# giesselmann/STRique

Measured on AMD Instinct MI355X. Metric: reads/s for STRique 'count' on 50 kb r9.4 signals, higher is better.
Workload: dtype f32

## Files before the change

### include/strique_hip.h

```cpp
#ifndef STRIQUE_HIP_H
#define STRIQUE_HIP_H

#include <stdint.h>

#ifdef __cplusplus
extern "C" {
#endif

#define STRQ_OK 0
#define STRQ_ERR_ARG 1
#define STRQ_ERR_DEVICE 2
#define STRQ_ERR_UNSUPPORTED 3
#define STRQ_ERR_NOMEM 4

typedef struct strq_ctx strq_ctx;

int strq_abi_version(void);

int strq_ctx_create(int device_id, strq_ctx** out);
void strq_ctx_destroy(strq_ctx* ctx);
const char* strq_last_error(const strq_ctx* ctx);
int strq_device_synchronize(strq_ctx* ctx);

int strq_set_option(strq_ctx* ctx, const char* key, const char* value);
// ... 12 lines not shown
                     int32_t samples,
                     float* score, int64_t* j_end, int64_t* j0, int32_t* rec);

int strq_model_create(strq_ctx* ctx, int32_t n_states, int32_t silent_start, int32_t start, int32_t end,
                      const int32_t* in_ptr, const int32_t* in_src, const double* in_logp,
                      const int32_t* emis_kind, const double* emis_a, const double* emis_b,
                      const double* emis_c, const int32_t* count_inc, const int32_t* state_tag,
                      const int32_t* hint_slot, const int32_t* hint_lane, int32_t* model_id);

int strq_model_set_positions(strq_ctx* ctx, int32_t model_id, const int32_t* kind, const int32_t* pos);

int strq_viterbi(strq_ctx* ctx, int32_t model_id, const double* x, int64_t T,
                 double* logp, int64_t* counted, int32_t* status, int32_t* path);
int strq_viterbi_batch(strq_ctx* ctx, int32_t model_id, int64_t n_seq, const double* x,
                       const int64_t* x_off, double* logp, int64_t* counted, int32_t* status,
                       int32_t* paths);

int strq_forward_batch(strq_ctx* ctx, int32_t model_id, int64_t n_seq, const double* x, const int64_t* x_off,
                       const int64_t* c0, double* log_lik, double* visits_mean, double* visits_var, int32_t* status);
int strq_model_set_forward_logp(strq_ctx* ctx, int32_t model_id, const double* in_logp_sum);

typedef struct strq_result {
    int32_t count;
    int32_t status;
    double score_prefix, score_suffix, log_p;
    int64_t offset, ticks;
    int64_t prefix_begin, prefix_end, suffix_begin, suffix_end;
} strq_result;

int strq_set_pore_stats(strq_ctx* ctx, double tail_lo, double tail_hi, double model_min, double model_max);
int strq_target_add(strq_ctx* ctx, const float* prefix_ext, int64_t m_prefix, const float* suffix_ext,
                    int64_t m_suffix, int32_t trim_prefix, int32_t trim_suffix, int32_t samples,
                    int32_t hmm_model_id, int32_t count_bias, int32_t* target_id);
int strq_target_set_mod(strq_ctx* ctx, int32_t target_id, int32_t mod_model_id, double mod_min, double mod_max);
int strq_batch_fetch_mod(strq_ctx* ctx, char* pool, int64_t pool_cap, int64_t* off);
int strq_set_units(strq_ctx* ctx, int32_t on);
int strq_batch_fetch_units(strq_ctx* ctx, int64_t* pool, int64_t pool_cap, int64_t* off, int32_t* decoded);
int strq_last_units(strq_ctx* ctx, double* out4);
int strq_set_mod_llr(strq_ctx* ctx, int32_t on);
int strq_batch_fetch_mod_llr(strq_ctx* ctx, double* pool, int64_t pool_cap, int64_t* off);
int strq_last_mod_llr(strq_ctx* ctx, double* out4);
int strq_target_set_variants(strq_ctx* ctx, int32_t target_id, int32_t model_id, double lo, double hi, int32_t n_alt, int32_t context_units);
int strq_set_variants(strq_ctx* ctx, int32_t on);
int strq_batch_fetch_variants(strq_ctx* ctx, int32_t* count_v, int32_t* decoded, int64_t* off, int8_t* branch, int64_t* end, int64_t pass_cap,
                              double* vpool, int64_t* voff, int64_t v_cap, int64_t* v_total);
int strq_last_variants(strq_ctx* ctx, double* out4);
int strq_set_confidence(strq_ctx* ctx, int32_t on);
int strq_batch_fetch_confidence(strq_ctx* ctx, double* out3, int32_t* decoded);
int strq_last_confidence(strq_ctx* ctx, double* out4);
int strq_detect_batch(strq_ctx* ctx, int64_t n_reads, const void* signals, int32_t dtype,
                      const int64_t* offsets, const int32_t* target_id, const double* host_stats,
                      strq_result* out);
int strq_detect_batch_reads(strq_ctx* ctx, int64_t n_reads, const void* const* reads, const int64_t* lengths, int32_t dtype,
                            const int32_t* target_id, const double* host_stats, strq_result* out);
int strq_batch_upload(strq_ctx* ctx, int64_t n_reads, const void* signals, int32_t dtype,
                      const int64_t* offsets, const int32_t* target_id, const double* host_stats);
int strq_batch_upload_part(strq_ctx* ctx, int64_t total_reads, int64_t total_samples, int64_t first_read, int64_t n_reads,
                           const void* signals, int32_t dtype, const int64_t* offsets, const int32_t* target_id);
int strq_batch_run(strq_ctx* ctx);
int strq_batch_run_range(strq_ctx* ctx, int64_t first, int64_t last);
int strq_batch_fetch(strq_ctx* ctx, strq_result* out);
int strq_batch_fetch_range(strq_ctx* ctx, int64_t first, int64_t last, strq_result* out);
int strq_scan_batch_reads(strq_ctx* ctx, int64_t n_reads, const void* const* reads, const int64_t* lengths, int32_t dtype,
                          int32_t n_cand, const int32_t* cand_target_id, double min_score,
                          strq_result* out_rows, int32_t* out_cand, double* out_scores);
int strq_scan_set(strq_ctx* ctx, int32_t n_cand, const int32_t* cand_target_id, double min_score);
int strq_scan_clear(strq_ctx* ctx);
int strq_batch_fetch_scan(strq_ctx* ctx, int32_t* out_cand, double* out_scores);
typedef struct strq_anchored {
    int32_t kind;
    int32_t status;
    int32_t count, pad_;
    double log_p;
    int64_t begin, end;
    int64_t free_samples;
} strq_anchored;
int strq_target_set_anchored(strq_ctx* ctx, int32_t target_id, int32_t end_model_id, int32_t end_bias, int32_t start_model_id, int32_t start_bias);
int strq_set_anchored(strq_ctx* ctx, int32_t on, double min_score);
int strq_batch_fetch_anchored(strq_ctx* ctx, strq_anchored* out, int64_t n);
int strq_last_anchored(strq_ctx* ctx, double* out8);
typedef struct strq_renorm_fit {
    int32_t a, b, w;
    int32_t fitted;
    int64_t score;
} strq_renorm_fit;
typedef struct strq_renorm {
    int32_t applied, pad_;
    strq_renorm_fit fit[3];
} strq_renorm;
int strq_target_set_renorm(strq_ctx* ctx, int32_t target_id, const int16_t* Q, int32_t q_out, const int32_t* A, const double* W,
                           double grid_lo, double grid_d, double grid_p);
int strq_set_renorm(strq_ctx* ctx, int32_t on, double min_share);
int strq_batch_fetch_renorm(strq_ctx* ctx, strq_renorm* out, int64_t n);
int strq_last_renorm(strq_ctx* ctx, double* out4);
int strq_debug_renorm_fit(strq_ctx* ctx, int32_t target_id, const uint32_t* h3, strq_renorm* out);
int strq_host_stats(const double* signals, const int64_t* offsets, int64_t n_reads, int32_t want_raw, double* out);
int64_t strq_svb_decode(const uint8_t* stream, int64_t stream_len, int64_t n, int32_t key_bits, int32_t zigzag,
                        int32_t isize, void* out);
int64_t strq_inflate_chunks(const uint8_t* base, int64_t base_len, int64_t n_chunks, const int64_t* addr,
                            const int32_t* csize, const int64_t* elem_off, int32_t elem_size, int32_t shuffle,
                            int64_t chunk_elems, int64_t n_total, void* out);
#define STRQ_H5_UNHANDLED (-100)
#define STRQ_H5_MORE_CHUNKS (-101)
int64_t strq_h5_locate(const uint8_t* base, int64_t base_len, int64_t group_ohdr, const char* path, int64_t meta[16],
                       int64_t* chunk_addr, int32_t* chunk_size, int64_t* chunk_off, int64_t max_chunks);
int64_t strq_inflate_many(int64_t n_ds, const uint8_t* const* base, const int64_t* base_len, const int64_t* chunk_first,
                          const int64_t* addr, const int32_t* csize, const int64_t* elem_off, const int32_t* elem_size,
                          const int32_t* shuffle, const int64_t* chunk_elems, const int64_t* n_total, void* const* out,
                          int64_t* status);
int64_t strq_vbz_chunks(const uint8_t* base, int64_t base_len, int64_t n_chunks, const int64_t* addr, const int32_t* csize,
                        const int64_t* elem_off, int32_t elem_size, int32_t version, int32_t isize, int32_t zigzag, int32_t level,
                        int64_t chunk_elems, int64_t n_total, void* out);
void strq_inflate_stats(int64_t out[3], int32_t reset);
int strq_inflate_backend(void);
int strq_debug_conditioning(strq_ctx* ctx, int64_t read, uint8_t* levels, int64_t n, float* level_val,
                            double* scalars10);
int strq_debug_filtered(strq_ctx* ctx, int64_t read, void* out, int64_t n);
int strq_debug_live_allocations(int64_t out[2]);
int strq_debug_g2_layout(int32_t n_states, int32_t silent_start, int32_t start, int32_t end,
                         const int32_t* in_ptr, const int32_t* in_src, const double* in_logp,
                         const int32_t* emis_kind, const int32_t* count_inc, const int32_t* kind, const int32_t* pos,
                         double* out_lp, int32_t* out_own, int32_t* out_meta, char* why, int32_t why_len);

int strq_debug_screen_plan(const float params[6], int32_t samples, int32_t max_n, int32_t out[6]);

int strq_debug_score_tables(strq_ctx* ctx, int32_t n_jobs, const float* level_val, const float* cls_val, const int64_t* cls_off,
                            int32_t* info, int32_t* band_lo, float* table, uint8_t* planes,
                            int32_t* handed, int32_t handed_cap, int32_t* n_handed);

int strq_debug_variant_image(int32_t n_states, int32_t silent_start, int32_t start, int32_t end,
                             const int32_t* in_ptr, const int32_t* in_src, const double* in_logp,
                             const int32_t* emis_kind, const double* emis_a, const double* emis_b, const double* emis_c,
                             const int32_t* state_tag, int32_t n_alt, int32_t* build_rc, int32_t* head, int64_t* offsets,
                             void* image, int64_t image_cap, int64_t* image_bytes, char* why, int32_t why_len);
int strq_debug_mod_llr_image(int32_t n_states, int32_t silent_start, int32_t start, int32_t end,
                             const int32_t* in_ptr, const int32_t* in_src, const double* in_logp,
                             const int32_t* emis_kind, const double* emis_a, const double* emis_b, const double* emis_c,
                             const int32_t* state_tag, int32_t* build_rc, int32_t* head, int64_t* offsets,
                             void* image, int64_t image_cap, int64_t* image_bytes, char* why, int32_t why_len);
int strq_debug_variant_scores(strq_ctx* ctx, int32_t n_reads, const int32_t* model_id, int32_t n_alt, const double* x,
                              const int64_t* x_off, const int32_t* w, const int64_t* w_off, double* out, int32_t* launched);
int strq_debug_mod_llr_scores(strq_ctx* ctx, int32_t n_reads, const int32_t* model_id, const double* x, const int64_t* x_off,
                              const int32_t* w, const int64_t* w_off, double* out, int32_t* launched);
int strq_debug_variant_bounds(strq_ctx* ctx, int32_t model_id, int32_t n_alt, int32_t n_reads, const int64_t* off,
                              const int32_t* path, const uint64_t* rec, const uint32_t* last, const int32_t* status,
                              const int32_t* cap, int32_t stride, int32_t guard, int32_t* n, int32_t* bad, int32_t* w,
                              int32_t* branch, int32_t* untouched);

int strq_last_timing(const strq_ctx* ctx, float ms[8]);
int strq_last_counters(const strq_ctx* ctx, double out[8]);
int strq_last_geometry(const strq_ctx* ctx, int32_t out[8]);
int strq_last_viterbi_launches(const strq_ctx* ctx, int32_t out[4]);
int strq_last_second_round(const strq_ctx* ctx, int64_t out[2]);
int strq_last_screen(const strq_ctx* ctx, double out[8]);
int strq_last_screen_mode(const strq_ctx* ctx, int32_t out[8]);
int strq_last_overlap(const strq_ctx* ctx, double out[4]);

#ifdef __cplusplus
}
#endif
#endif
```

### strique_amd/csrc/align_kernels.h

```cpp
#pragma once
#include <hip/hip_runtime.h>
#include <stdint.h>

#define STRQ_CKPT_STEPS 256
#define STRQ_COLS_PER_STEP 2
#define STRQ_CKPT_FIELDS(R) (2 * (R) + 6)
#define STRQ_TRACE_WORDS(R) (((R) + 15) / 16)

namespace strq {

struct AlignParams {
    float open_h, ext_h, open_v, ext_v, dist_offset, dist_min;
};

struct AlignTask {
    const uint8_t* levels;
    const float* table;
    const uint8_t* table3;
    const int32_t* band_lo;
    const float* col0;
    float* ckpt;
    int32_t* rec;
    const float* bnd_in;
    float* bnd_out;
    const AlignTask* up;
    int32_t n, m, k, tsize;
    int32_t row0, m_total;
    int32_t col_off, n_full;
};

struct AlignResult {
    float best;
    int32_t j_end;
    int32_t j0;
    int32_t status;
};

static inline int align_num_steps(int n) { return (n + 1) / 2 + 63; }
static inline int align_num_ckpts(int n) { return (align_num_steps(n) - 1) / STRQ_CKPT_STEPS; }

#define STRQ_MAX_STRIPS 64
int align_plan(int m, int samples, int* rows_per_lane, int* n_strips);
int align_effective_samples(int samples);
int align_segment_overlap(const AlignParams& p, int m);
int launch_align_segments(hipStream_t stream, int R, int S, const AlignTask* tasks, AlignResult* seg_results,
                          int n_groups, int segs, int* queue, const AlignParams& p, int lds_dwords,
                          int tables_per_cu, int n_cu, int packed, const int* group_list = nullptr, const int* n_list = nullptr,
                          bool known_last_row = false);
int align_segments_wpe(int segs, int tables_per_cu);
int launch_align_combine(hipStream_t stream, const AlignTask* tasks, const AlignResult* seg_results, int n_align,
                         int segs, AlignResult* results, int32_t* pick, int pick_base = 0, const int* list = nullptr,
                         const int* n_list = nullptr, const float* min_score = nullptr, int* redo = nullptr, int* redo_count = nullptr,
                         unsigned int* redo_total = nullptr);
int launch_align_scatter(hipStream_t stream, const AlignResult* src, const int32_t* pick_src, const int32_t* first, const int32_t* pos, int n,
                         AlignResult* dst, int32_t* pick_dst);
float align_segment_min_score(const AlignParams& p, int m, int overlap_used);
int align_overlap_for_score(const AlignParams& p, int m, float score);
int launch_align(hipStream_t stream, int R, int S, const AlignTask* tasks, AlignResult* results,
                 int n_tasks, int* queue, const AlignParams& p, int lds_floats_per_wave,
                 int waves_per_block, int n_blocks, uint64_t* scratch, int phase, int mode, int packed,
                 const int32_t* pick = nullptr);
size_t align_trace_scratch_words_per_wave(int R);

}
```

### strique_amd/csrc/align_kernels.hip

```cpp
#include "strq_opt.h"
#include <hip/hip_runtime.h>
#include <stdint.h>
#include "align_kernels.h"
#include <stdlib.h>
#include <type_traits>
#include <utility>

namespace strq {

#define STRQ_NINF (-3.4028234663852886e38f / 2)

#define STRQ_STR2(x) #x
#define STRQ_STR(x) STRQ_STR2(x)
#define STRQ_TIE_EXT(ext, opn)  ((ext) >= (opn))
#define STRQ_TIE_H_OVER_V(h, v) ((h) >= (v))
#define STRQ_TIE_D_OVER_G(d, g) ((d) >= (g))

static __device__ __forceinline__ float dpp_shr1_f(float v, float fill)
{
    return __builtin_bit_cast(float, __builtin_amdgcn_update_dpp(__builtin_bit_cast(int, fill),
                              __builtin_bit_cast(int, v), 0x138, 0xF, 0xF, false));
}
static __device__ __forceinline__ float dpp_shr1_f0(float v)
{
    return __builtin_bit_cast(float, __builtin_amdgcn_update_dpp(0, __builtin_bit_cast(int, v), 0x138, 0xF, 0xF, true));
}
static __device__ __forceinline__ int dpp_shr1_i(int v, int fill)
{
    return __builtin_amdgcn_update_dpp(fill, v, 0x138, 0xF, 0xF, false);
}
template <class T> static __device__ __forceinline__ const T* uniform_ptr(const T* p)
{
    const uint64_t u = reinterpret_cast<uint64_t>(p);
    const uint32_t lo = __builtin_amdgcn_readfirstlane((int)(uint32_t)u), hi = __builtin_amdgcn_readfirstlane((int)(uint32_t)(u >> 32));
    return reinterpret_cast<const T*>(((uint64_t)hi << 32) | lo);
}
static __device__ __forceinline__ int med3i(int a, int lo, int hi)
{
    int r;
    asm("v_med3_i32 %0, %1, %2, %3" : "=v"(r) : "v"(a), "v"(lo), "v"(hi));
    return r;
}
static __device__ __forceinline__ float sel_mask(float if0, float if1, uint64_t mask)
{
    float r;
    asm("v_cndmask_b32_e64 %0, %1, %2, %3" : "=v"(r) : "v"(if0), "v"(if1), "s"(mask));
    return r;
}

static __device__ __forceinline__ int next_task(int* queue, int lane)
{
    __builtin_amdgcn_wave_barrier();
    int ti = 0;
    if (lane == 0) ti = atomicAdd(queue, 1);
    __builtin_amdgcn_wave_barrier();
    ti = __builtin_amdgcn_readfirstlane(ti);
    __builtin_amdgcn_wave_barrier();
    return ti;
}

template <int R, int S> struct Shape {
    static constexpr int gcd_(int a, int b) { return b == 0 ? a : gcd_(b, a % b); }
    static constexpr int G = gcd_(R, S);
    static constexpr int C = (S - G + R - 1) / S + 1;
    static constexpr int NMASK = S / G;
    static_assert(C <= 6, "too many classes per lane");
};

template <int R> struct Lane {
    float S[R];
    float H[R];
    float SbotA;
    float VbotA;
    float VbotB;
    float upS;
};

struct LaneConst {
    int off[6];
    int lo4[6];
    int hi4[6];
    int off2[6];
};

#define STRQ_PK_SCALE 1048576.0f
template <int R, int S, bool PK>
static __device__ __forceinline__ void fetch_scores(const char* lds, const LaneConst& lc, int q4,
                                                    float (&sc)[Shape<R, S>::C])
{
#pragma unroll
    for (int c = 0; c < Shape<R, S>::C; ++c) {
        if constexpr (PK) {
            const int ci = med3i(q4, lc.lo4[c], lc.hi4[c]);
            const uint32_t h = *reinterpret_cast<const uint16_t*>(lds + (ci << 1) + lc.off[c]);
            const uint32_t l = *reinterpret_cast<const uint8_t*>(lds + ci + lc.off2[c]);
            sc[c] = (float)((h << 8) | l);
        } else {
            const int t = med3i(q4, lc.lo4[c], lc.hi4[c]) + lc.off[c];
            sc[c] = *reinterpret_cast<const float*>(lds + t);
        }
    }
}

template <int R, int S>
static __device__ __forceinline__ void expand_scores(const float (&sc)[Shape<R, S>::C],
                                                     const uint64_t (&pm)[Shape<R, S>::NMASK],
                                                     float (&rs)[R])
{
    constexpr int G = Shape<R, S>::G, C = Shape<R, S>::C;
#pragma unroll
    for (int r = 0; r < R; r += G) {
        const int base = r / S, x = (r % S) / G;
        float v;
        if (x == 0 || base + 1 >= C) v = sc[base < C ? base : C - 1];
        else v = sel_mask(sc[base], sc[base + 1], pm[x]);
#pragma unroll
        for (int g = 0; g < G && r + g < R; ++g) rs[r + g] = v;
    }
}

template <int R>
static __device__ __forceinline__ float pick_row(const float (&x)[R], int rM)
{
    typedef float vec_t __attribute__((ext_vector_type(R <= 16 ? 16 : 32)));
    vec_t v;
#pragma unroll
    for (int r = 0; r < R; ++r) v[r] = x[r];
    return v[rM];
}

struct TraceWords { uint64_t a[2], b[2]; };

#ifndef STRQ_TRACE_SELECT
static __device__ __forceinline__ void trace_push_ge(uint32_t& acc, float a, float b)
{
    asm("v_cmp_ge_f32 vcc, %1, %2\n\tv_addc_co_u32 %0, vcc, %0, %0, vcc" : "+v"(acc) : "v"(a), "v"(b) : "vcc");
}
#endif
template <int R> static __device__ __forceinline__ int trace_shift(int r)
{
#ifndef STRQ_TRACE_SELECT
    const int in_word = r % 16, half = in_word / 8;
    const int rows_word = R - 16 * (r / 16) < 16 ? R - 16 * (r / 16) : 16;
    const int rows_half = rows_word - 8 * half < 8 ? rows_word - 8 * half : 8;
    return 32 * half + 4 * (rows_half - 1 - (in_word % 8));
#else
    return 4 * (r % 16);
#endif
}

template <int R, bool LH, bool LV, bool KEEP, bool TRACE, int RMC = -1>
static __device__ __forceinline__ void dp_step2(Lane<R>& st, const float (&rsA)[R], const float (&rsB)[R],
                                                float upA, float upB, float upVA, float upVB,
                                                const AlignParams& p, TraceWords* tw,
                                                int rM, float* candA, float* candB)
{
    float SA[R], SB[R];
    float HA[R], HB[R];
    float vA = upVA, vB = upVB;
    if constexpr (TRACE) { tw->a[0] = tw->a[1] = tw->b[0] = tw->b[1] = 0; }
    uint32_t accA[4] = {0u, 0u, 0u, 0u}, accB[4] = {0u, 0u, 0u, 0u};
    (void)accA; (void)accB;
#pragma unroll
    for (int r = 0; r < R; ++r) {
        {
            const float diag = r == 0 ? st.upS : st.S[r - 1];
            const float up = r == 0 ? upA : SA[r > 0 ? r - 1 : 0];
            const float D = diag + rsA[r];
            if constexpr (TRACE) {
                const float hext = st.H[r] + p.ext_h, hopn = st.S[r] + p.open_h;
                const float vext = vA + p.ext_v, vopn = up + p.open_v;
#ifndef STRQ_TRACE_SELECT
                uint32_t& acc = accA[(r / 16) * 2 + (r % 16) / 8];
                trace_push_ge(acc, vext, vopn); trace_push_ge(acc, hext, hopn);
                const float Hn = __builtin_fmaxf(hext, hopn), Vn = __builtin_fmaxf(vext, vopn);
                trace_push_ge(acc, Hn, Vn);
                const float Gm = __builtin_fmaxf(Hn, Vn);
                trace_push_ge(acc, D, Gm);
                SA[r] = __builtin_fmaxf(D, Gm); HA[r] = Hn; vA = Vn;
#else
                const bool he = STRQ_TIE_EXT(hext, hopn);
                const float Hn = he ? hext : hopn;
                const bool ve = STRQ_TIE_EXT(vext, vopn);
                const float Vn = ve ? vext : vopn;
                const bool gh = STRQ_TIE_H_OVER_V(Hn, Vn);
                const float Gm = gh ? Hn : Vn;
                const bool dd = STRQ_TIE_D_OVER_G(D, Gm);
                SA[r] = dd ? D : Gm; HA[r] = Hn; vA = Vn;
                const uint64_t code = (dd ? 1u : 0u) | (gh ? 2u : 0u) | (he ? 4u : 0u) | (ve ? 8u : 0u);
                tw->a[r / 16] |= code << (4 * (r % 16));
#endif
            } else {
                float Hn, Vn;
                if constexpr (LH) Hn = st.S[r] + p.ext_h;
                else Hn = __builtin_fmaxf(st.H[r] + p.ext_h, st.S[r] + p.open_h);
                if constexpr (LV) Vn = up + p.ext_v;
                else Vn = __builtin_fmaxf(vA + p.ext_v, up + p.open_v);
                SA[r] = __builtin_fmaxf(__builtin_fmaxf(D, Hn), Vn);
                HA[r] = Hn; vA = Vn;
            }
        }
        {
            const float diag = r == 0 ? upA : SA[r > 0 ? r - 1 : 0];
            const float up = r == 0 ? upB : SB[r > 0 ? r - 1 : 0];
            const float D = diag + rsB[r];
            if constexpr (TRACE) {
                const float hext = HA[r] + p.ext_h, hopn = SA[r] + p.open_h;
                const float vext = vB + p.ext_v, vopn = up + p.open_v;
#ifndef STRQ_TRACE_SELECT
                uint32_t& acc = accB[(r / 16) * 2 + (r % 16) / 8];
                trace_push_ge(acc, vext, vopn); trace_push_ge(acc, hext, hopn);
                const float Hn = __builtin_fmaxf(hext, hopn), Vn = __builtin_fmaxf(vext, vopn);
                trace_push_ge(acc, Hn, Vn);
                const float Gm = __builtin_fmaxf(Hn, Vn);
                trace_push_ge(acc, D, Gm);
                SB[r] = __builtin_fmaxf(D, Gm); HB[r] = Hn; vB = Vn;
#else
                const bool he = STRQ_TIE_EXT(hext, hopn);
                const float Hn = he ? hext : hopn;
                const bool ve = STRQ_TIE_EXT(vext, vopn);
                const float Vn = ve ? vext : vopn;
                const bool gh = STRQ_TIE_H_OVER_V(Hn, Vn);
                const float Gm = gh ? Hn : Vn;
                const bool dd = STRQ_TIE_D_OVER_G(D, Gm);
                SB[r] = dd ? D : Gm; HB[r] = Hn; vB = Vn;
                const uint64_t code = (dd ? 1u : 0u) | (gh ? 2u : 0u) | (he ? 4u : 0u) | (ve ? 8u : 0u);
                tw->b[r / 16] |= code << (4 * (r % 16));
#endif
            } else {
                float Hn, Vn;
                if constexpr (LH) Hn = SA[r] + p.ext_h;
                else Hn = __builtin_fmaxf(HA[r] + p.ext_h, SA[r] + p.open_h);
                if constexpr (LV) Vn = up + p.ext_v;
                else Vn = __builtin_fmaxf(vB + p.ext_v, up + p.open_v);
                SB[r] = __builtin_fmaxf(__builtin_fmaxf(D, Hn), Vn);
                HB[r] = Hn; vB = Vn;
            }
        }
    }
#ifndef STRQ_TRACE_SELECT
    if constexpr (TRACE) {
#pragma unroll
        for (int x = 0; x < 2; ++x) {
            tw->a[x] = (uint64_t)accA[2 * x] | ((uint64_t)accA[2 * x + 1] << 32);
            tw->b[x] = (uint64_t)accB[2 * x] | ((uint64_t)accB[2 * x + 1] << 32);
        }
    }
#endif
#pragma unroll
    for (int r = 0; r < R; ++r) st.S[r] = SB[r];
    if constexpr (TRACE || !LH || KEEP) {
#pragma unroll
        for (int r = 0; r < R; ++r) st.H[r] = HB[r];
    }
    st.SbotA = SA[R - 1];
    if constexpr (TRACE || !LV || KEEP) { st.VbotA = vA; st.VbotB = vB; }
    st.upS = upB;
    if constexpr (RMC >= 0) { *candA = SA[RMC]; *candB = SB[RMC]; }
    else if (candA) { *candA = pick_row<R>(SA, rM); *candB = pick_row<R>(SB, rM); }
}

template <int R, int S, bool PK>
static __device__ __forceinline__ void load_lane_consts(const AlignTask& tk, int lane, int lds_base,
                                                        LaneConst& lc, uint64_t (&pm)[Shape<R, S>::NMASK])
{
    const int row0 = tk.row0 + lane * R;
    const int kbase = row0 / S - tk.row0 / S, phase = row0 % S;
    const int off0 = 0;
#pragma unroll
    for (int c = 0; c < Shape<R, S>::C; ++c) {
        int k = kbase + c; if (k > tk.k - 1) k = tk.k - 1;
        const uint32_t d = (uint32_t)tk.band_lo[k];
        const int lo = (int)(d & 255u), w1 = (int)((d >> 8) & 255u), off = (int)(d >> 16);
        if constexpr (PK) {
            lc.lo4[c] = lo; lc.hi4[c] = lo + w1;
            lc.off[c] = lds_base + (off - lo) * 2;
            lc.off2[c] = lds_base + ((2 * tk.tsize + 3) & ~3) + off - lo;
        } else {
            lc.lo4[c] = lo * 4;
            lc.hi4[c] = (lo + w1) * 4;
            lc.off[c] = lds_base + (off - off0) * 4 - lo * 4;
            lc.off2[c] = 0;
        }
    }
#pragma unroll
    for (int x = 0; x < Shape<R, S>::NMASK; ++x) {
        const uint64_t b = __ballot(phase >= S - x * Shape<R, S>::G);
        const uint32_t lo = __builtin_amdgcn_readfirstlane((int)(uint32_t)b), hi = __builtin_amdgcn_readfirstlane((int)(uint32_t)(b >> 32));
        pm[x] = ((uint64_t)hi << 32) | lo;
    }
}

template <bool PK>
static __device__ __forceinline__ void stage_table(const AlignTask& tk, float* lds, int lane)
{
    if constexpr (PK) {
        const uint32_t* src = reinterpret_cast<const uint32_t*>(tk.table3);
        uint32_t* dst = reinterpret_cast<uint32_t*>(lds);
        const int nd = (((2 * tk.tsize + 3) & ~3) + tk.tsize + 3) / 4;
        for (int i = lane; i < nd; i += 64) dst[i] = src[i];
    } else {
        for (int i = lane; i < tk.tsize; i += 64) lds[i] = tk.table[i];
    }
}

template <int R, bool PK>
static __device__ __forceinline__ void init_lane(const AlignTask& tk, int lane, Lane<R>& st)
{
    constexpr float SC = PK ? STRQ_PK_SCALE : 1.0f;
    const int row0 = lane * R;
#pragma unroll
    for (int r = 0; r < R; ++r) {
        int i = row0 + r + 1; if (i > tk.m) i = tk.m;
        st.S[r] = tk.col0[i] * SC;
        st.H[r] = STRQ_NINF;
    }
    { int i = row0 + R; if (i > tk.m) i = tk.m; st.SbotA = st.VbotA = st.VbotB = tk.col0[i] * SC; }
    { int i = row0;     if (i > tk.m) i = tk.m; st.upS = tk.col0[i] * SC; }
}

template <bool PK>
static __device__ __forceinline__ int load_chunk(const AlignTask& tk, int chunk, int lane)
{
    constexpr int U = PK ? 1 : 4;
    const int idx = (chunk * 64 + lane) * 2;
    int a = 0, b = 0;
    if (idx < tk.n) a = tk.levels[idx];
    if (idx + 1 < tk.n) b = tk.levels[idx + 1];
    return (a * U) | ((b * U) << 16);
}

struct Bnd4 { float sA, vA, sB, vB; };
static __device__ __forceinline__ Bnd4 load_bnd(const AlignTask& tk, int chunk, int lane)
{
    const int idx = (chunk * 64 + lane) * 2;
    Bnd4 b{0.0f, STRQ_NINF, 0.0f, STRQ_NINF};
    if (idx < tk.n) { b.sA = tk.bnd_in[2 * idx]; b.vA = tk.bnd_in[2 * idx + 1]; }
    if (idx + 1 < tk.n) { b.sB = tk.bnd_in[2 * idx + 2]; b.vB = tk.bnd_in[2 * idx + 3]; }
    return b;
}

template <int R>
static __device__ __forceinline__ void save_ckpt(float* c, int lane, const Lane<R>& st)
{
#pragma unroll
    for (int r = 0; r < R; ++r) c[r * 64 + lane] = st.S[r];
#pragma unroll
    for (int r = 0; r < R; ++r) c[(R + r) * 64 + lane] = st.H[r];
    c[(2 * R + 0) * 64 + lane] = st.SbotA;
    c[(2 * R + 1) * 64 + lane] = st.VbotA;
    c[(2 * R + 2) * 64 + lane] = st.VbotB;
    c[(2 * R + 3) * 64 + lane] = st.upS;
}
template <int R>
static __device__ __forceinline__ void load_ckpt(const float* c, int lane, Lane<R>& st)
{
#pragma unroll
    for (int r = 0; r < R; ++r) st.S[r] = c[r * 64 + lane];
#pragma unroll
    for (int r = 0; r < R; ++r) st.H[r] = c[(R + r) * 64 + lane];
    st.SbotA = c[(2 * R + 0) * 64 + lane];
    st.VbotA = c[(2 * R + 1) * 64 + lane];
    st.VbotB = c[(2 * R + 2) * 64 + lane];
    st.upS = c[(2 * R + 3) * 64 + lane];
}

template <int R, int S, bool LH, bool LV, int MODE, bool RM_LAST, bool PK, int RMC = -1>
struct Forward {
    static constexpr bool HAS_IN = (MODE & 1) != 0, HAS_OUT = (MODE & 2) != 0;
    const AlignTask& tk;
    const AlignParams& p;
    const char* ldsb;
    const LaneConst& lc;
    const uint64_t (&pm)[Shape<R, S>::NMASK];
    const int lane, rM;
    Lane<R> st;
    float best, bestA; int bestt;
    int qq;
    float scA[Shape<R, S>::C], scB[Shape<R, S>::C];
    Bnd4 bcur;

    __device__ __forceinline__ void advance(int qsrc, int snext, int& qn, float (&nA)[Shape<R, S>::C], float (&nB)[Shape<R, S>::C])
    {
        qn = dpp_shr1_i(qq, __builtin_amdgcn_readlane(qsrc, snext));
        fetch_scores<R, S, PK>(ldsb, lc, qn & 0xffff, nA);
        fetch_scores<R, S, PK>(ldsb, lc, (int)((unsigned)qn >> 16), nB);
    }
    __device__ __forceinline__ void prime(int qcur)
    {
        qq = 0;
        int qn; float nA[Shape<R, S>::C], nB[Shape<R, S>::C];
        advance(qcur, 0, qn, nA, nB);
        qq = qn;
#pragma unroll
        for (int c = 0; c < Shape<R, S>::C; ++c) { scA[c] = nA[c]; scB[c] = nB[c]; }
    }

    template <bool PRED, bool KEEP, int RMX = RMC>
    __device__ __forceinline__ void step(int t, int s, int qsrc, int snext)
    {
        int qn; float nA[Shape<R, S>::C], nB[Shape<R, S>::C];
        advance(qsrc, snext, qn, nA, nB);
        float fA = 0.0f, fB = 0.0f, fVA = STRQ_NINF, fVB = STRQ_NINF;
        if constexpr (HAS_IN) {
            fA = __builtin_bit_cast(float, __builtin_amdgcn_readlane(__builtin_bit_cast(int, bcur.sA), s));
            fB = __builtin_bit_cast(float, __builtin_amdgcn_readlane(__builtin_bit_cast(int, bcur.sB), s));
            if constexpr (!LV) {
                fVA = __builtin_bit_cast(float, __builtin_amdgcn_readlane(__builtin_bit_cast(int, bcur.vA), s));
                fVB = __builtin_bit_cast(float, __builtin_amdgcn_readlane(__builtin_bit_cast(int, bcur.vB), s));
            }
        }
#ifdef STRQ_DP_ZFILL
        const float upA = HAS_IN ? dpp_shr1_f(st.SbotA, fA) : dpp_shr1_f0(st.SbotA);
        const float upB = HAS_IN ? dpp_shr1_f(st.S[R - 1], fB) : dpp_shr1_f0(st.S[R - 1]);
#else
        const float upA = dpp_shr1_f(st.SbotA, fA);
        const float upB = dpp_shr1_f(st.S[R - 1], fB);
#endif
        float upVA = STRQ_NINF, upVB = STRQ_NINF;
        if constexpr (!LV) { upVA = dpp_shr1_f(st.VbotA, fVA); upVB = dpp_shr1_f(st.VbotB, fVB); }
        const int jB = 2 * (t - lane), jA = jB - 1;
        bool act = true;
        if constexpr (PRED) act = (jA >= 1) && (jA <= tk.n);
        if (act) {
            float rsA[R], rsB[R];
            expand_scores<R, S>(scA, pm, rsA);
            expand_scores<R, S>(scB, pm, rsB);
            bool okB = true;
            if constexpr (PRED) okB = jB <= tk.n;
            if constexpr (HAS_OUT) {
                dp_step2<R, LH, LV, true, false>(st, rsA, rsB, upA, upB, upVA, upVB, p, nullptr, 0, nullptr, nullptr);
                if (lane == 63) {
                    float* o = tk.bnd_out + 2 * (size_t)(jA - 1);
                    o[0] = st.SbotA; o[1] = st.VbotA;
                    if (okB) { o[2] = st.S[R - 1]; o[3] = st.VbotB; }
                }
            } else {
                float candA, candB;
                if constexpr (RM_LAST || RMX == R - 1) {
                    dp_step2<R, LH, LV, KEEP, false>(st, rsA, rsB, upA, upB, upVA, upVB, p, nullptr, 0, nullptr, nullptr);
                    candA = st.SbotA; candB = st.S[R - 1];
                } else if constexpr (RMX >= 0) {
                    dp_step2<R, LH, LV, KEEP, false, RMX>(st, rsA, rsB, upA, upB, upVA, upVB, p, nullptr, rM, &candA, &candB);
                } else {
                    dp_step2<R, LH, LV, KEEP, false>(st, rsA, rsB, upA, upB, upVA, upVB, p, nullptr, rM, &candA, &candB);
                }
                const float cb = okB ? candB : candA;
                const float nb = __builtin_fmaxf(__builtin_fmaxf(best, candA), cb);
                if (nb > best) { bestt = t; bestA = candA; }
                best = nb;
            }
        }
        qq = qn;
#pragma unroll
        for (int c = 0; c < Shape<R, S>::C; ++c) { scA[c] = nA[c]; scB[c] = nB[c]; }
    }
};

template <int R, int S, int X, class F>
static __device__ __forceinline__ void rm_case(int rM, bool& hit, F& f)
{
    if constexpr ((X + 1) % Shape<R, S>::G == 0) {
        if (!hit && rM == X) { f(std::integral_constant<int, X>{}); hit = true; }
    }
}
template <int R, int S, class F, int... X>
static __device__ __forceinline__ bool rm_dispatch(int rM, F& f, std::integer_sequence<int, X...>)
{
    bool hit = false;
    (rm_case<R, S, X>(rM, hit, f), ...);
    return hit;
}

template <int R, int S, bool LH, bool LV, int MODE, bool RM_LAST, bool PK, bool STAGE = true, int RMC = -1, bool RMSW = false>
static __device__ __forceinline__ void forward_one(const AlignTask& tk, AlignResult* res, const AlignParams& p,
                                                   float* lds, int lds_base, const char* ldsb, int lane)
{
    constexpr bool HAS_IN = (MODE & 1) != 0, HAS_OUT = (MODE & 2) != 0;
    if constexpr (STAGE) stage_table<PK>(tk, lds, lane);
    LaneConst lc; uint64_t pm[Shape<R, S>::NMASK];
    load_lane_consts<R, S, PK>(tk, lane, lds_base, lc, pm);
    const int lM = (tk.m - 1) / R, rM = (tk.m - 1) % R;
    Forward<R, S, LH, LV, MODE, RM_LAST, PK, RMC> f{tk, p, ldsb, lc, pm, lane, rM};
    init_lane<R, PK>(tk, lane, f.st);
    f.best = tk.col0[tk.m] * (PK ? STRQ_PK_SCALE : 1.0f); f.bestA = 0.0f; f.bestt = -1;
    __builtin_amdgcn_s_waitcnt(0);

    const int nsteps = (tk.n + 1) / 2 + 63;
    int rM_u = 0;
    if constexpr (RMSW) rM_u = __builtin_amdgcn_readfirstlane(rM);
    (void)rM_u;
    int qcur = load_chunk<PK>(tk, 0, lane);
    f.prime(qcur);
    Bnd4 bnext{0.0f, STRQ_NINF, 0.0f, STRQ_NINF};
    if constexpr (HAS_IN) f.bcur = load_bnd(tk, 0, lane); else f.bcur = bnext;
    for (int t0 = 0; t0 < nsteps; t0 += 64) {
        const int qnext = load_chunk<PK>(tk, t0 / 64 + 1, lane);
        if constexpr (HAS_IN) bnext = load_bnd(tk, t0 / 64 + 1, lane);
        const bool full = (t0 >= 63) && (2 * (t0 + 64) <= tk.n);
        const bool ckpt_here = ((t0 + 64) % STRQ_CKPT_STEPS) == 0 && (t0 + 64) < nsteps;
        const int send = nsteps - t0 < 64 ? nsteps - t0 : 64;
        if (full) {
#ifdef STRQ_DP_PAD
            asm volatile(".p2align 6\n\t.rept " STRQ_STR(STRQ_DP_PAD) "\n\ts_nop 0\n\t.endr");
#endif
            if constexpr (RMSW && !HAS_OUT && !RM_LAST) {
                auto chunk = [&](auto rmx) {
                    constexpr int X = decltype(rmx)::value;
                    for (int s = 0; s < 63; ++s) f.template step<false, false, X>(t0 + s + 1, s, qcur, s + 1);
                    if (ckpt_here) f.template step<false, true, X>(t0 + 64, 63, qnext, 0);
                    else f.template step<false, false, X>(t0 + 64, 63, qnext, 0);
                };
                if (!rm_dispatch<R, S>(rM_u, chunk, std::make_integer_sequence<int, R>{})) chunk(std::integral_constant<int, -1>{});
            } else {
                for (int s = 0; s < 63; ++s) f.template step<false, false>(t0 + s + 1, s, qcur, s + 1);
                if (ckpt_here) f.template step<false, true>(t0 + 64, 63, qnext, 0);
                else f.template step<false, false>(t0 + 64, 63, qnext, 0);
            }
        } else {
            for (int s = 0; s < send; ++s) {
                const int qsrc = s == 63 ? qnext : qcur, snext = (s + 1) & 63;
                if (ckpt_here && s == 63) f.template step<true, true>(t0 + s + 1, s, qsrc, snext);
                else f.template step<true, false>(t0 + s + 1, s, qsrc, snext);
            }
        }
        if (ckpt_here)
            save_ckpt<R>(tk.ckpt + (size_t)((t0 + 64) / STRQ_CKPT_STEPS - 1) * (STRQ_CKPT_FIELDS(R) * 64), lane, f.st);
        qcur = qnext;
        if constexpr (HAS_IN) f.bcur = bnext;
    }
    if constexpr (!HAS_OUT) {
        int bestj = 0;
        if (f.bestt >= 0) bestj = 2 * (f.bestt - lane) - (f.bestA == f.best ? 1 : 0);
        const float b = __shfl(f.best, lM, 64);
        const int bj = __shfl(bestj, lM, 64);
        res->best = b * (PK ? 1.0f / STRQ_PK_SCALE : 1.0f); res->j_end = bj;
    }
}

template <int R, int S, bool LH, bool LV, int MODE, bool PK>
__global__ void __launch_bounds__(512)
align_forward_kernel(const AlignTask* __restrict__ tasks, AlignResult* __restrict__ results, int n_tasks,
                     int* __restrict__ queue, AlignParams p, int lds_floats_per_wave)
{
    extern __shared__ float lds_all[];
    const int lane = threadIdx.x & 63, wave = threadIdx.x >> 6;
    float* lds = lds_all + (size_t)wave * lds_floats_per_wave;
    const int lds_base = wave * lds_floats_per_wave * 4;
    const char* ldsb = reinterpret_cast<const char*>(lds_all);
    for (;;) {
        const int ti = next_task(queue, lane);
        if (ti >= n_tasks) break;
        const AlignTask& tk = tasks[ti];
        if constexpr ((MODE & 2) != 0) forward_one<R, S, LH, LV, MODE, true, PK>(tk, results + ti, p, lds, lds_base, ldsb, lane);
        else {
            if ((tk.m - 1) % R == R - 1) forward_one<R, S, LH, LV, MODE, true, PK>(tk, results + ti, p, lds, lds_base, ldsb, lane);
            else forward_one<R, S, LH, LV, MODE, false, PK>(tk, results + ti, p, lds, lds_base, ldsb, lane);
        }
    }
}

template <int R, int S, bool PK, int SEG, int WPE, bool LISTED = false, bool KNOWN = false>
__global__ void __attribute__((amdgpu_flat_work_group_size(64 * SEG, 64 * SEG), amdgpu_waves_per_eu(WPE, WPE)))
align_forward_seg_kernel(const AlignTask* __restrict__ tasks, AlignResult* __restrict__ results, int n_groups,
                         int* __restrict__ queue, AlignParams p, const int* __restrict__ group_list,
                         const int* __restrict__ n_list)
{
    extern __shared__ float lds_all[];
    __shared__ int next_group;
    const int lane = threadIdx.x & 63, wave = threadIdx.x >> 6;
    const char* ldsb = reinterpret_cast<const char*>(lds_all);
    const int lds_base = 0;
    if constexpr (LISTED) n_groups = __builtin_amdgcn_readfirstlane(*n_list);
    for (;;) {
        __syncthreads();
        if (threadIdx.x == 0) next_group = atomicAdd(queue, 1);
        __syncthreads();
        int gi = __builtin_amdgcn_readfirstlane(next_group);
        if (gi >= n_groups) break;
        if constexpr (LISTED) gi = __builtin_amdgcn_readfirstlane(group_list[gi]);
        {
            const AlignTask& t0 = tasks[(size_t)gi * SEG];
            if constexpr (PK) {
                const uint32_t* src = reinterpret_cast<const uint32_t*>(t0.table3);
                uint32_t* dst = reinterpret_cast<uint32_t*>(lds_all);
                const int nd = (((2 * t0.tsize + 3) & ~3) + t0.tsize + 3) / 4;
                for (int i = threadIdx.x; i < nd; i += 64 * SEG) dst[i] = src[i];
            } else {
                for (int i = threadIdx.x; i < t0.tsize; i += 64 * SEG) lds_all[i] = t0.table[i];
            }
        }
        __syncthreads();
        const int ti = gi * SEG + wave;
        const AlignTask& tk = tasks[ti];
        if (tk.n <= 0) continue;
        if constexpr (KNOWN) {
            constexpr int RMC870 = R == 14 ? (870 - 1) % 14 : -1;
            if ((tk.m - 1) % R == R - 1) forward_one<R, S, true, true, 0, true, PK, false>(tk, results + ti, p, lds_all, lds_base, ldsb, lane);
            else if (RMC870 >= 0 && (tk.m - 1) % R == RMC870) forward_one<R, S, true, true, 0, false, PK, false, RMC870>(tk, results + ti, p, lds_all, lds_base, ldsb, lane);
            else forward_one<R, S, true, true, 0, false, PK, false>(tk, results + ti, p, lds_all, lds_base, ldsb, lane);
        } else {
            forward_one<R, S, true, true, 0, false, PK, false, -1, true>(tk, results + ti, p, lds_all, lds_base, ldsb, lane);
        }
    }
}

__global__ void align_combine_kernel(const AlignTask* __restrict__ tasks, const AlignResult* __restrict__ seg, int n_align,
                                     int segs, AlignResult* __restrict__ out, int32_t* __restrict__ pick, int pick_base,
                                     const int* __restrict__ list, const int* __restrict__ n_list,
                                     const float* __restrict__ min_score, int* __restrict__ redo, int* __restrict__ redo_count,
                                     unsigned int* __restrict__ redo_total)
{
    int a = blockIdx.x * blockDim.x + threadIdx.x;
    if (a >= (n_list ? *n_list : n_align)) return;
    if (list) a = list[a];
    int best_k = 0;
    float best = seg[(size_t)a * segs].best;
    for (int k = 1; k < segs; ++k) {
        const size_t t = (size_t)a * segs + k;
        if (tasks[t].n <= 0) continue;
        if (seg[t].best > best) { best = seg[t].best; best_k = k; }
    }
    const size_t t = (size_t)a * segs + best_k;
    AlignResult r = seg[t];
    r.j_end += tasks[t].col_off;
    out[a] = r;
    pick[a] = pick_base + (int32_t)t;
    if (min_score && !(best >= min_score[a])) {
        redo[atomicAdd(redo_count, 1)] = a;
        if (redo_total) atomicAdd(redo_total, 1u);
    }
}

template <int R, int S, bool PK>
__global__ void __launch_bounds__(512)
align_trace_kernel(const AlignTask* __restrict__ tasks, AlignResult* __restrict__ results, int n_tasks,
                   int* __restrict__ queue, AlignParams p, int lds_floats_per_wave,
                   uint64_t* __restrict__ scratch_all, const int32_t* __restrict__ pick)
{
    extern __shared__ float lds_all[];
    constexpr int W = STRQ_TRACE_WORDS(R);
    constexpr size_t STEP_WORDS = 2 * W * 64;
    const int lane = threadIdx.x & 63, wave = threadIdx.x >> 6;
    float* lds = lds_all + (size_t)wave * lds_floats_per_wave;
    const int lds_base = wave * lds_floats_per_wave * 4;
    const char* ldsb = reinterpret_cast<const char*>(lds_all);
    uint64_t* scratch = scratch_all + (size_t)(blockIdx.x * (blockDim.x >> 6) + wave) * (STRQ_CKPT_STEPS * STEP_WORDS);

    for (;;) {
        const int ti = next_task(queue, lane);
        if (ti >= n_tasks) break;
        const AlignTask* cur = &tasks[pick ? __builtin_amdgcn_readfirstlane(pick[ti]) : ti];
        const AlignTask* staged = nullptr;
        int32_t* rec = cur->rec;
        const int col_off = __builtin_amdgcn_readfirstlane(cur->col_off);
        LaneConst lc; uint64_t pm[Shape<R, S>::NMASK];

        int ci = cur->m_total, cj = __builtin_amdgcn_readfirstlane(results[ti].j_end) - col_off, state = 0;
        while (ci > 0 && cj > 0) {
            while (ci <= cur->row0) cur = uniform_ptr(cur->up);
            if (cur != staged) {
                __builtin_amdgcn_s_waitcnt(0);
                stage_table<PK>(*cur, lds, lane);
                load_lane_consts<R, S, PK>(*cur, lane, lds_base, lc, pm);
                __builtin_amdgcn_s_waitcnt(0);
                staged = cur;
            }
            const AlignTask& tk = *cur;
            const bool has_in = tk.bnd_in != nullptr;
            uint64_t pmu[Shape<R, S>::NMASK];
#pragma unroll
            for (int x = 0; x < Shape<R, S>::NMASK; ++x) {
                const uint32_t lo = __builtin_amdgcn_readfirstlane((int)(uint32_t)pm[x]), hi = __builtin_amdgcn_readfirstlane((int)(uint32_t)(pm[x] >> 32));
                pmu[x] = ((uint64_t)hi << 32) | lo;
            }
            const int tcur = (ci - tk.row0 - 1) / R + (cj + 1) / 2;
            const int blk = (tcur - 1) / STRQ_CKPT_STEPS;
            const int tb = blk * STRQ_CKPT_STEPS;
            Lane<R> st;
            if (blk == 0) init_lane<R, PK>(tk, lane, st);
            else load_ckpt<R>(tk.ckpt + (size_t)(blk - 1) * (STRQ_CKPT_FIELDS(R) * 64), lane, st);
            int qq = 0;
            {
                const int jB = 2 * (tb - lane), jA = jB - 1;
                int a = 0, b = 0;
                if (jA >= 1 && jA <= tk.n) a = tk.levels[jA - 1];
                if (jB >= 1 && jB <= tk.n) b = tk.levels[jB - 1];
                qq = (a * (PK ? 1 : 4)) | ((b * (PK ? 1 : 4)) << 16);
            }
            int qcur = load_chunk<PK>(tk, tb / 64, lane);
            Bnd4 bcur{0.0f, STRQ_NINF, 0.0f, STRQ_NINF}, bnext = bcur;
            if (has_in) bcur = load_bnd(tk, tb / 64, lane);
            for (int t0 = tb; t0 < tcur; t0 += 64) {
                const int qnext = load_chunk<PK>(tk, t0 / 64 + 1, lane);
                if (has_in) bnext = load_bnd(tk, t0 / 64 + 1, lane);
                const int send = tcur - t0 < 64 ? tcur - t0 : 64;
                for (int s = 0; s < send; ++s) {
                    const int t = t0 + s + 1;
                    qq = dpp_shr1_i(qq, __builtin_amdgcn_readlane(qcur, s));
                    const float fA = __builtin_bit_cast(float, __builtin_amdgcn_readlane(__builtin_bit_cast(int, bcur.sA), s));
                    const float fB = __builtin_bit_cast(float, __builtin_amdgcn_readlane(__builtin_bit_cast(int, bcur.sB), s));
                    const float fVA = __builtin_bit_cast(float, __builtin_amdgcn_readlane(__builtin_bit_cast(int, bcur.vA), s));
                    const float fVB = __builtin_bit_cast(float, __builtin_amdgcn_readlane(__builtin_bit_cast(int, bcur.vB), s));
                    const float upA = dpp_shr1_f(st.SbotA, fA);
                    const float upB = dpp_shr1_f(st.S[R - 1], fB);
                    const float upVA = dpp_shr1_f(st.VbotA, fVA);
                    const float upVB = dpp_shr1_f(st.VbotB, fVB);
                    const int jB = 2 * (t - lane), jA = jB - 1;
                    TraceWords w; w.a[0] = w.a[1] = w.b[0] = w.b[1] = 0;
                    if (jA >= 1 && jA <= tk.n) {
                        float scA[Shape<R, S>::C], scB[Shape<R, S>::C], rsA[R], rsB[R];
                        fetch_scores<R, S, PK>(ldsb, lc, qq & 0xffff, scA);
                        fetch_scores<R, S, PK>(ldsb, lc, (int)((unsigned)qq >> 16), scB);
                        expand_scores<R, S>(scA, pmu, rsA);
                        expand_scores<R, S>(scB, pmu, rsB);
                        dp_step2<R, false, false, true, true>(st, rsA, rsB, upA, upB, upVA, upVB, p, &w, 0, nullptr, nullptr);
                    }
                    uint64_t* dst = scratch + (size_t)(t - tb - 1) * STEP_WORDS;
#pragma unroll
                    for (int x = 0; x < W; ++x) {
                        dst[(0 * W + x) * 64 + lane] = w.a[x];
                        dst[(1 * W + x) * 64 + lane] = w.b[x];
                    }
                }
                qcur = qnext; bcur = bnext;
            }
            __threadfence();
            int pf_l = -1, pf_hi = 0, pf_lo = 0, pf_word = -1; uint64_t pf = 0;
            while (ci > tk.row0 && cj > 0) {
                const int il = ci - tk.row0;
                const int l = (il - 1) / R, r = (il - 1) % R;
                const int t = l + (cj + 1) / 2;
                if (t <= tb) break;
                const int colsel = (cj & 1) ? 0 : 1;
                if (l != pf_l || r / 16 != pf_word || t > pf_hi || t <= pf_lo) {
                    pf_l = l; pf_word = r / 16; pf_hi = t; pf_lo = t - 32 > tb ? t - 32 : tb;
                    const int st = t - (lane >> 1), cs = lane & 1;
                    pf = st > pf_lo ? scratch[(size_t)(st - tb - 1) * STEP_WORDS + (cs * W + pf_word) * 64 + l] : 0;
                }
                const int src = ((pf_hi - t) << 1) | colsel;
                const uint32_t wlo = (uint32_t)__builtin_amdgcn_readlane((int)(uint32_t)pf, src);
                const uint32_t whi = (uint32_t)__builtin_amdgcn_readlane((int)(uint32_t)(pf >> 32), src);
                const uint64_t w = ((uint64_t)whi << 32) | wlo;
                const uint32_t code = (uint32_t)(w >> trace_shift<R>(r)) & 15u;
                if (state == 0) {
                    if (code & 1u) { rec[ci - 1] = (cj + col_off) << 1; --ci; --cj; }
                    else state = (code & 2u) ? 1 : 2;
                } else if (state == 1) {
                    --cj; if (!(code & 4u)) state = 0;
                } else {
                    rec[ci - 1] = ((cj + col_off) << 1) | 1;
                    --ci; if (!(code & 8u)) state = 0;
                }
            }
        }
        for (int i = ci - lane; i > 0; i -= 64) rec[i - 1] = (col_off << 1) | 1;
        results[ti].j0 = cj + col_off;
    }
}

template <int R, int S>
static int launch_shape(hipStream_t stream, const AlignTask* tasks, AlignResult* results, int n_tasks,
                        int* queue, const AlignParams& p, int lds_floats_per_wave, int waves_per_block,
                        int n_blocks, uint64_t* scratch, int phase, int mode, int packed, const int32_t* pick)
{
    const size_t lds_bytes = (size_t)lds_floats_per_wave * 4 * waves_per_block;
    const dim3 grid(n_blocks), block(64 * waves_per_block);
    const bool lh = p.open_h == p.ext_h, lv = p.open_v == p.ext_v;
#define STRQ_FWD1(LH_, LV_, MODE_)                                                                      \
    do {                                                                                                \
        (void)hipFuncSetAttribute((const void*)align_forward_kernel<R, S, LH_, LV_, MODE_, false>,      \
                                  hipFuncAttributeMaxDynamicSharedMemorySize, (int)lds_bytes);          \
        hipLaunchKernelGGL((align_forward_kernel<R, S, LH_, LV_, MODE_, false>), grid, block, lds_bytes, stream,\
                           tasks, results, n_tasks, queue, p, lds_floats_per_wave);                     \
    } while (0)
#define STRQ_FWD(LH_, LV_)                                                                              \
    do {                                                                                                \
        if (mode == 0) STRQ_FWD1(LH_, LV_, 0); else if (mode == 1) STRQ_FWD1(LH_, LV_, 1);              \
        else if (mode == 2) STRQ_FWD1(LH_, LV_, 2); else STRQ_FWD1(LH_, LV_, 3);                        \
    } while (0)
    if (packed && !(lh && lv && mode == 0)) return 2;
    if (phase == 0 && packed) {
        AlignParams ps = p;
        ps.open_h *= STRQ_PK_SCALE; ps.ext_h *= STRQ_PK_SCALE; ps.open_v *= STRQ_PK_SCALE; ps.ext_v *= STRQ_PK_SCALE;
        (void)hipFuncSetAttribute((const void*)align_forward_kernel<R, S, true, true, 0, true>,
                                  hipFuncAttributeMaxDynamicSharedMemorySize, (int)lds_bytes);
        hipLaunchKernelGGL((align_forward_kernel<R, S, true, true, 0, true>), grid, block, lds_bytes, stream,
                           tasks, results, n_tasks, queue, ps, lds_floats_per_wave);
    } else if (phase == 0) {
        if (lh && lv) STRQ_FWD(true, true);
        else if (lh) STRQ_FWD(true, false);
        else if (lv) STRQ_FWD(false, true);
        else STRQ_FWD(false, false);
    } else if (packed) {
        AlignParams ps = p;
        ps.open_h *= STRQ_PK_SCALE; ps.ext_h *= STRQ_PK_SCALE; ps.open_v *= STRQ_PK_SCALE; ps.ext_v *= STRQ_PK_SCALE;
        (void)hipFuncSetAttribute((const void*)align_trace_kernel<R, S, true>,
                                  hipFuncAttributeMaxDynamicSharedMemorySize, (int)lds_bytes);
        hipLaunchKernelGGL((align_trace_kernel<R, S, true>), grid, block, lds_bytes, stream, tasks, results,
                           n_tasks, queue, ps, lds_floats_per_wave, scratch, pick);
    } else {
        (void)hipFuncSetAttribute((const void*)align_trace_kernel<R, S, false>,
                                  hipFuncAttributeMaxDynamicSharedMemorySize, (int)lds_bytes);
        hipLaunchKernelGGL((align_trace_kernel<R, S, false>), grid, block, lds_bytes, stream, tasks, results,
                           n_tasks, queue, p, lds_floats_per_wave, scratch, pick);
    }
#undef STRQ_FWD
#undef STRQ_FWD1
    return hipGetLastError() == hipSuccess ? 0 : 1;
}

template <int R, int S>
static int launch_shape_general(hipStream_t stream, const AlignTask* tasks, AlignResult* results, int n_tasks,
                                int* queue, const AlignParams& p, int lds_floats_per_wave, int waves_per_block,
                                int n_blocks, uint64_t* scratch, int phase, int mode, int packed, const int32_t* pick)
{
    if (packed) return 2;
    const size_t lds_bytes = (size_t)lds_floats_per_wave * 4 * waves_per_block;
    const dim3 grid(n_blocks), block(64 * waves_per_block);
#define STRQ_FWDG(MODE_)                                                                                \
    do {                                                                                                \
        (void)hipFuncSetAttribute((const void*)align_forward_kernel<R, S, false, false, MODE_, false>,  \
                                  hipFuncAttributeMaxDynamicSharedMemorySize, (int)lds_bytes);          \
        hipLaunchKernelGGL((align_forward_kernel<R, S, false, false, MODE_, false>), grid, block, lds_bytes, stream,\
                           tasks, results, n_tasks, queue, p, lds_floats_per_wave);                     \
    } while (0)
    if (phase == 0) {
        if (mode == 0) STRQ_FWDG(0); else if (mode == 1) STRQ_FWDG(1); else if (mode == 2) STRQ_FWDG(2); else STRQ_FWDG(3);
    } else {
        (void)hipFuncSetAttribute((const void*)align_trace_kernel<R, S, false>,
                                  hipFuncAttributeMaxDynamicSharedMemorySize, (int)lds_bytes);
        hipLaunchKernelGGL((align_trace_kernel<R, S, false>), grid, block, lds_bytes, stream, tasks, results,
                           n_tasks, queue, p, lds_floats_per_wave, scratch, pick);
    }
#undef STRQ_FWDG
    return hipGetLastError() == hipSuccess ? 0 : 1;
}

#define STRQ_SHAPES(X) X(6, 6) X(7, 6) X(8, 6) X(12, 6) X(14, 6) X(15, 6)
#define STRQ_GENERAL_SHAPES(X) X(2, 1) X(4, 2) X(6, 3) X(8, 4) X(10, 5) X(14, 7) X(16, 8) X(18, 9) X(20, 10) X(22, 11) X(26, 13)

int align_effective_samples(int samples)
{
    if (samples < 1) return 0;
    if (samples % 6 == 0) return 6;
    for (int d : {13, 11, 10, 9, 8, 7, 5, 4, 3, 2}) if (samples % d == 0) return d;
    return 1;
}

int align_plan(int m, int samples, int* rows_per_lane, int* n_strips)
{
    if (samples < 1 || m < 1) return 0;
    if (samples != 6) {
        if (align_effective_samples(samples) != samples) return 0;
        const int r = 2 * samples, rows = 64 * r;
        if (m > STRQ_MAX_STRIPS * rows) return 0;
        *rows_per_lane = r; *n_strips = (m + rows - 1) / rows;
        return r;
    }
    const char* e = strq::opt("STRQ_STRIPS");
    const bool force_two = e && e[0] == '2';
    const bool no14 = strq::opt("STRQ_NO_R14") != nullptr;
    const int single[] = {6, 7, 8, 12, 14, 15};
    const int two[] = {6, 7, 8, 12};
    if (!force_two)
        for (int r : single) if (64 * r >= m && !(r == 14 && no14)) { *rows_per_lane = r; *n_strips = 1; return r; }
    for (int r : two) if (64 * r < m && 128 * r >= m) { *rows_per_lane = r; *n_strips = 2; return r; }
    for (int r : single) if (64 * r >= m && !(r == 14 && no14)) { *rows_per_lane = r; *n_strips = 1; return r; }
    if (m <= STRQ_MAX_STRIPS * 64 * 12) { *rows_per_lane = 12; *n_strips = (m + 64 * 12 - 1) / (64 * 12); return 12; }
    return 0;
}

size_t align_trace_scratch_words_per_wave(int R)
{
    return (size_t)STRQ_CKPT_STEPS * 2 * STRQ_TRACE_WORDS(R) * 64;
}

int launch_align(hipStream_t stream, int R, int S, const AlignTask* tasks, AlignResult* results,
                 int n_tasks, int* queue, const AlignParams& p, int lds_floats_per_wave,
                 int waves_per_block, int n_blocks, uint64_t* scratch, int phase, int mode, int packed,
                 const int32_t* pick)
{
#define STRQ_CASE(R_, S_)                                                                               \
    if (R == R_ && S == S_)                                                                             \
        return launch_shape<R_, S_>(stream, tasks, results, n_tasks, queue, p, lds_floats_per_wave,     \
                                    waves_per_block, n_blocks, scratch, phase, mode, packed, pick);
    STRQ_SHAPES(STRQ_CASE)
#undef STRQ_CASE
#define STRQ_CASE(R_, S_)                                                                               \
    if (R == R_ && S == S_)                                                                             \
        return launch_shape_general<R_, S_>(stream, tasks, results, n_tasks, queue, p, lds_floats_per_wave, \
                                            waves_per_block, n_blocks, scratch, phase, mode, packed, pick);
    STRQ_GENERAL_SHAPES(STRQ_CASE)
#undef STRQ_CASE
    return 2;
}

int align_segment_overlap(const AlignParams& p, int m)
{
    if (!(p.dist_min >= 0.0f) || !(p.open_h < 0.0f) || !(p.ext_h < 0.0f) || !(p.dist_offset > 0.0f)) return 0;
    if (!(p.open_v <= 0.0f) || !(p.ext_v <= 0.0f)) return 0;
    const double c_h = -(double)(p.open_h > p.ext_h ? p.open_h : p.ext_h);
    const double gain = (double)(p.dist_min > p.dist_offset ? p.dist_min : p.dist_offset);
    const double h = (double)m * gain / c_h;
    const double L = (double)m + h * 1.01 + 64.0;
    if (!(L < 1e8)) return 0;
    return (int)L + 1;
}

template <int R, int S, bool PK, int SEG, int WPE, bool KNOWN>
static int launch_seg2(hipStream_t stream, const AlignTask* tasks, AlignResult* seg_results, int n_groups, int* queue,
                       const AlignParams& p, int lds_dwords, int n_blocks, const int* group_list, const int* n_list)
{
    const size_t lds_bytes = (size_t)lds_dwords * 4;
    if (group_list && n_list) {
        (void)hipFuncSetAttribute((const void*)align_forward_seg_kernel<R, S, PK, SEG, WPE, true, KNOWN>,
                                  hipFuncAttributeMaxDynamicSharedMemorySize, (int)lds_bytes);
        hipLaunchKernelGGL((align_forward_seg_kernel<R, S, PK, SEG, WPE, true, KNOWN>), dim3(n_blocks), dim3(64 * SEG), lds_bytes, stream,
                           tasks, seg_results, n_groups, queue, p, group_list, n_list);
    } else {
        (void)hipFuncSetAttribute((const void*)align_forward_seg_kernel<R, S, PK, SEG, WPE, false, KNOWN>,
                                  hipFuncAttributeMaxDynamicSharedMemorySize, (int)lds_bytes);
        hipLaunchKernelGGL((align_forward_seg_kernel<R, S, PK, SEG, WPE, false, KNOWN>), dim3(n_blocks), dim3(64 * SEG), lds_bytes, stream,
                           tasks, seg_results, n_groups, queue, p, group_list, n_list);
    }
    return hipGetLastError() == hipSuccess ? 0 : 1;
}

template <int R, int S, bool PK, int SEG, int WPE>
static int launch_seg1(hipStream_t stream, const AlignTask* tasks, AlignResult* seg_results, int n_groups, int* queue,
                       const AlignParams& p, int lds_dwords, int n_blocks, const int* group_list, const int* n_list, bool known_last_row)
{
    if constexpr (R == 14) {
        if (known_last_row) return launch_seg2<R, S, PK, SEG, WPE, true>(stream, tasks, seg_results, n_groups, queue, p, lds_dwords, n_blocks, group_list, n_list);
    }
    return launch_seg2<R, S, PK, SEG, WPE, false>(stream, tasks, seg_results, n_groups, queue, p, lds_dwords, n_blocks, group_list, n_list);
}

#define STRQ_SEG_CONFIGS(X, R_, S_, PK_) X(R_, S_, PK_, 1, 2) X(R_, S_, PK_, 2, 3) X(R_, S_, PK_, 2, 4) X(R_, S_, PK_, 3, 3) X(R_, S_, PK_, 4, 4) X(R_, S_, PK_, 3, 4) X(R_, S_, PK_, 4, 3)

int align_segments_wpe(int segs, int tables_per_cu)
{
    const int waves = tables_per_cu * segs;
    int wpe = (waves + 3) / 4; if (wpe < 2) wpe = 2;
    if (segs == 1) wpe = 2;
    else if (wpe < 3) wpe = 3;
    if (wpe > 4) wpe = 4;
    return wpe;
}

int launch_align_segments(hipStream_t stream, int R, int S, const AlignTask* tasks, AlignResult* seg_results,
                          int n_groups, int segs, int* queue, const AlignParams& p, int lds_dwords,
                          int tables_per_cu, int n_cu, int packed, const int* group_list, const int* n_list, bool known_last_row)
{
    if (!(p.open_h == p.ext_h && p.open_v == p.ext_v)) return 2;
    AlignParams ps = p;
    if (packed) { ps.open_h *= STRQ_PK_SCALE; ps.ext_h *= STRQ_PK_SCALE; ps.open_v *= STRQ_PK_SCALE; ps.ext_v *= STRQ_PK_SCALE; }
    const int wpe = align_segments_wpe(segs, tables_per_cu);
    const int n_blocks = tables_per_cu * n_cu;
#define STRQ_SEGCASE(R_, S_, PK_, SEG_, WPE_)                                                             \
    if (R == R_ && S == S_ && (packed != 0) == PK_ && segs == SEG_ && wpe == WPE_)                        \
        return launch_seg1<R_, S_, PK_, SEG_, WPE_>(stream, tasks, seg_results, n_groups, queue, ps, lds_dwords, n_blocks, group_list, n_list, known_last_row);
#define STRQ_SEGSHAPE(R_, S_) STRQ_SEG_CONFIGS(STRQ_SEGCASE, R_, S_, true) STRQ_SEG_CONFIGS(STRQ_SEGCASE, R_, S_, false)
    STRQ_SHAPES(STRQ_SEGSHAPE)
#undef STRQ_SEGSHAPE
#undef STRQ_SEGCASE
    return 2;
}

int launch_align_combine(hipStream_t stream, const AlignTask* tasks, const AlignResult* seg_results, int n_align,
                         int segs, AlignResult* results, int32_t* pick, int pick_base, const int* list, const int* n_list,
                         const float* min_score, int* redo, int* redo_count, unsigned int* redo_total)
{
    if (n_align <= 0) return 0;
    hipLaunchKernelGGL(align_combine_kernel, dim3((n_align + 255) / 256), dim3(256), 0, stream, tasks, seg_results, n_align, segs,
                       results, pick, pick_base, list, n_list, min_score, redo, redo_count, redo_total);
    return hipGetLastError() == hipSuccess ? 0 : 1;
}

__global__ void align_scatter_kernel(const AlignResult* __restrict__ src, const int32_t* __restrict__ pick_src, const int32_t* __restrict__ first,
                                     const int32_t* __restrict__ pos, int n, AlignResult* __restrict__ dst, int32_t* __restrict__ pick_dst)
{
    const int a = blockIdx.x * blockDim.x + threadIdx.x;
    if (a >= n) return;
    int best = first[a];
    for (int g = first[a] + 1; g < first[a + 1]; ++g) if (src[g].best > src[best].best) best = g;
    dst[pos[a]] = src[best]; pick_dst[pos[a]] = pick_src[best];
}

int launch_align_scatter(hipStream_t stream, const AlignResult* src, const int32_t* pick_src, const int32_t* first, const int32_t* pos, int n,
                         AlignResult* dst, int32_t* pick_dst)
{
    if (n <= 0) return 0;
    hipLaunchKernelGGL(align_scatter_kernel, dim3((n + 255) / 256), dim3(256), 0, stream, src, pick_src, first, pos, n, dst, pick_dst);
    return hipGetLastError() == hipSuccess ? 0 : 1;
}

int align_overlap_for_score(const AlignParams& p, int m, float score)
{
    const int worst = align_segment_overlap(p, m);
    if (worst <= 0 || !(score > 0.0f)) return worst;
    const double c_h = -(double)(p.open_h > p.ext_h ? p.open_h : p.ext_h);
    const double gain = (double)(p.dist_min > p.dist_offset ? p.dist_min : p.dist_offset);
    double h = ((double)m * gain - (double)score + 1.0) / c_h;
    if (h < 0) h = 0;
    const double L = (double)m + h * 1.01 + 66.0;
    return L + 1 < (double)worst ? (int)L + 1 : worst;
}

float align_segment_min_score(const AlignParams& p, int m, int overlap_used)
{
    const double c_h = -(double)(p.open_h > p.ext_h ? p.open_h : p.ext_h);
    const double h_ok = ((double)overlap_used - (double)m - 65.0) / 1.01;
    const double gain = (double)(p.dist_min > p.dist_offset ? p.dist_min : p.dist_offset);
    const double b = (double)m * gain - h_ok * c_h;
    return (float)(b + 1.0 + 1e-6 * (b < 0 ? -b : b));
}

}
```

### strique_amd/csrc/strq_align_api.hip

```cpp
#include <hip/hip_runtime.h>
#include <algorithm>
#include <cmath>
#include <climits>
#include <cstring>
#include <cstdlib>
#include <time.h>
#include <unistd.h>
#include <map>
#include <mutex>
#include <string>
#include <tuple>
#include <numeric>
#include <vector>
#include "../../include/strique_hip.h"
#include "strq_ctx.h"
#include "align_kernels.h"
#include "lut_kernels.h"
#include "align_generic.h"

using namespace strq;

#define STRQ_DBG(...) do { if (strq::opt("STRQ_DEBUG")) { fprintf(stderr, "[strq] " __VA_ARGS__); fprintf(stderr, "\n"); fflush(stderr); } } while (0)

namespace strq {

static thread_local const strq_ctx* t_cur_ctx = nullptr;
static std::mutex g_opt_mu;
static std::map<std::string, std::string> g_opts;
CtxScope::CtxScope(const strq_ctx* c) : prev(t_cur_ctx) { t_cur_ctx = c; }
CtxScope::~CtxScope() { t_cur_ctx = prev; }
const char* opt(const char* key)
{
    static thread_local std::string ring[8];
    static thread_local unsigned ring_pos = 0;
    auto keep = [&](const std::string& v) -> const char* {
        if (v.empty()) return nullptr;
        std::string& slot = ring[ring_pos++ & 7u];
        slot = v;
        return slot.c_str();
    };
    if (t_cur_ctx) {
        std::lock_guard<std::mutex> lk(t_cur_ctx->options_mu);
        auto it = t_cur_ctx->options.find(key);
        if (it != t_cur_ctx->options.end()) return keep(it->second);
    }
    {
        std::lock_guard<std::mutex> lk(g_opt_mu);
        auto it = g_opts.find(key);
        if (it != g_opts.end()) return keep(it->second);
    }
    return getenv(key);
}

float host_cell_score(const AlignParams& p, float h, float v)
{
    const float d = h > v ? h - v : v - h;
    const float s = p.dist_offset - (float)std::pow((double)d, 1.2);
    return s > p.dist_min ? s : p.dist_min;
}

void host_col0(const AlignParams& p, int m, float* out)
{
    const float NINF = -3.4028234663852886e38f / 2;
    out[0] = 0.0f;
    float vprev = NINF, sprev = 0.0f;
    for (int i = 1; i <= m; ++i) {
        const float ext = vprev + p.ext_v, opn = sprev + p.open_v;
        const float v = ext >= opn ? ext : opn;
        out[i] = v; vprev = v; sprev = v;
    }
}

struct BatchIn {
    int64_t n_align, n_reads;
    const uint8_t* levels; const int64_t* read_off; const float* level_val;
    const int32_t* align_read; const float* flank; const int64_t* flank_off; int32_t samples;
};
struct BatchOut { float* score; int64_t* j_end; int64_t* j0; int32_t* rec; };


static const int hard_cap = 1 << 16;
static const int trace_wpb = 8;

struct Piece { int col_off, n; size_t ck; };

static int cut(int n, int segs, int ov, Piece* out)
{
    int use = segs;
    while (use > 1 && (ov <= 0 || (long)n < (long)(use + 1) * ov)) --use;
    const long len = use > 1 ? ((long)n + (long)(use - 1) * ov + use - 1) / use : n;
    long o = 0;
    for (int k = 0; k < segs; ++k) {
        if (k >= use) { out[k].col_off = 0; out[k].n = 0; continue; }
        const long start = k == 0 ? 0 : o - ov;
        long end = k == use - 1 ? n : start + len; if (end > n) end = n;
        out[k].col_off = (int)start; out[k].n = (int)(end - start);
        o = end;
    }
    return use;
}

static int packed_dwords(int entries) { return (((2 * entries + 3) & ~3) + entries + 3) / 4; }

struct Launch { int R, NS, tables, first, count, first_task, first_up, lds_floats, packed, segs; bool known_last_row; };

struct CorePlan {
    CorePlan(strq_ctx* c_, const AlignCoreIn& in_, AlignCoreOut& out_) : c(c_), in(in_), out(out_), nb(in_.nb), S(in_.samples), st(c_->stream) {}
    strq_ctx* c;
    const AlignCoreIn& in;
    AlignCoreOut& out;
    const int nb, S;
    const hipStream_t st;

    bool collapsed = false, allow_pack = false, ov_fixed = false, scr_forced = false, mode_fine = false, mode_coarse = false;
    int seg_want = 0, max_tables = 8, max_waves = 16, ov_cap = 8192;
    std::map<std::pair<int, int>, int> ov_of_m;

    std::vector<size_t> cls_off, col0_off, bnd_off;
    std::vector<int> J0, NJ;
    std::vector<int> job_align, job_k0, job_k;
    std::vector<size_t> tab_off, desc_off;
    int nj = 0, max_k = 0;
    std::vector<float> h_cls;
    std::vector<LutJob> jobs;
    std::vector<LutInfo> info;
    std::vector<int> tab_total;

    std::vector<ScreenWindows> wins;
    bool screen2_ran = false;
    std::vector<int> g2_of;
    ScreenTask* d_st2 = nullptr;
    int32_t* d_bound2 = nullptr;
    ScreenParams sp2{};
    double coarse_cols = 0, coarse_all = 0;

    std::vector<char> packed;
    std::vector<int> overlap, segs_of;
    std::vector<Launch> launches;
    int n_up = 0, max_ns = 1, r2_cap = 0, qi = STRQ_QUEUE_FIRST;
    size_t n_tasks = 0, safe0 = 0, r2_0 = 0;
    std::vector<Piece> pieces, safe;
    std::vector<float> min_score;
    std::vector<char> two_round;
    bool any_two_round = false;
    std::vector<size_t> ck_up;
    std::vector<AlignTask> tasks;
    AlignTask *d_tasks = nullptr, *d_heads = nullptr;
    AlignResult *d_seg = nullptr, *d_res = nullptr, *d_seg_safe = nullptr;
    int32_t* d_pick = nullptr;
    float* d_min_score = nullptr;
    int *d_redo = nullptr, *d_redo_count = nullptr;
};

static int overlap_for(CorePlan& p, int m, int ov_worst, int redo_weight = 1)
{
    strq_ctx* c = p.c;
    if (p.ov_fixed || c->score_fracs.size() < 64 || c->mean_n <= 0) return std::min(ov_worst, p.ov_cap);
    auto it = p.ov_of_m.find(std::make_pair(m, redo_weight));
    if (it != p.ov_of_m.end()) return it->second;
    const std::vector<float>& f = c->score_fracs;
    double best_cost = 0; int best_ov = std::min(ov_worst, p.ov_cap);
    for (int ov = 1024; ; ov += 512) {
        if (ov > ov_worst) ov = ov_worst;
        const float need = align_segment_min_score(c->ap, m, ov) / ((float)m * c->ap.dist_offset) + 0.01f;
        const double redo = (double)(std::lower_bound(f.begin(), f.end(), need) - f.begin()) / (double)f.size();
        const double cost = 3.0 * ov / c->mean_n + redo_weight * redo * (1.0 + 3.0 * ov_worst / c->mean_n);
        if (best_cost == 0 || cost < best_cost) { best_cost = cost; best_ov = ov; }
        if (ov >= ov_worst) break;
    }
    p.ov_of_m[std::make_pair(m, redo_weight)] = best_ov;
    STRQ_DBG("overlap for %d-row flanks: %d columns (worst case %d; previous sub-batch: median score fraction %.3f, mean read %.0f samples)", m, best_ov, ov_worst, f[f.size() / 2], c->mean_n);
    return best_ov;
}

static int tables_for(const CorePlan& p, int dwords, int segs)
{
    int t = std::min(p.max_tables, (160 * 1024 - 64) / (std::max(dwords, 1) * 4));
    if (segs > 1) t = std::min(t, p.max_waves / segs);
    return t;
}

static void pause_after_fail(int& pause, int& fail)
{
    pause = std::min(256, 8 << std::min(fail, 5));
    ++fail;
}

static int upload_inputs(CorePlan& p)
{
    strq_ctx* c = p.c; const AlignCoreIn& in = p.in; AlignCoreOut& out = p.out;
    const int nb = p.nb, S = p.S;
    hipStream_t st = p.st;
    size_t cls_tot = 0, col0_tot = 0, rec_tot = 0, tab_tot = 0, bnd_floats = 0, desc_tot = 0;
    p.cls_off.assign(nb, 0); p.col0_off.assign(nb, 0); p.bnd_off.assign(nb, 0);
    std::map<const float*, size_t> cls_of_flank; std::map<int, size_t> col0_of_m;
    std::vector<int> cls_first, col0_first;
    out.rec_off.assign(nb, 0);
    p.J0.assign(nb, 0); p.NJ.assign(nb, 0);
    for (int i = 0; i < nb; ++i) {
        auto fc = cls_of_flank.find(in.flank[i]);
        if (fc == cls_of_flank.end()) { fc = cls_of_flank.emplace(in.flank[i], cls_tot).first; cls_tot += in.k[i]; cls_first.push_back(i); }
        p.cls_off[i] = fc->second;
        auto f0 = col0_of_m.find(in.m[i]);
        if (f0 == col0_of_m.end()) { f0 = col0_of_m.emplace(in.m[i], col0_tot).first; col0_tot += in.m[i] + 1; col0_first.push_back(i); }
        p.col0_off[i] = f0->second;
        p.J0[i] = (int)p.job_align.size();
        p.NJ[i] = in.k[i] > STRQ_LUT_MAX_K ? in.NS[i] : 1;
        for (int sidx = 0; sidx < p.NJ[i]; ++sidx) {
            int k0 = 0, kn = in.k[i];
            if (p.NJ[i] > 1) {
                const int row0 = sidx * 64 * in.R[i], rows = std::min(64 * in.R[i], in.m[i] - row0);
                k0 = row0 / S; kn = (row0 + rows - 1) / S - k0 + 1;
            }
            p.job_align.push_back(i); p.job_k0.push_back(k0); p.job_k.push_back(kn);
            p.desc_off.push_back(desc_tot); desc_tot += kn;
            p.tab_off.push_back(tab_tot); tab_tot += STRQ_TABLE_SLOT_FLOATS(kn);
            p.max_k = std::max(p.max_k, kn);
        }
        out.rec_off[i] = rec_tot; rec_tot += in.m[i];
        p.bnd_off[i] = bnd_floats; if (in.NS[i] > 1) bnd_floats += (size_t)(in.NS[i] - 1) * 2 * ((size_t)in.n[i] + 2);
    }
    const int nj = p.nj = (int)p.job_align.size();
    out.rec_total = rec_tot;
    p.h_cls.assign(cls_tot, 0.0f);
    std::vector<float> h_col0(col0_tot);
    for (int i : cls_first) {
        const float* f = in.flank[i];
        for (int kk = 0; kk < in.k[i]; ++kk) p.h_cls[p.cls_off[i] + kk] = f[(size_t)kk * S];
    }
    for (int i : col0_first) host_col0(c->ap, in.m[i], &h_col0[p.col0_off[i]]);
    STRQ_HIP(c, c->flank_cls.reserve(cls_tot * 4));
    STRQ_HIP(c, c->col0.reserve(col0_tot * 4));
    STRQ_HIP(c, c->band_lo.reserve(desc_tot * 4));
    STRQ_HIP(c, c->tables.reserve(tab_tot * 4));
    STRQ_HIP(c, c->tables3.reserve(tab_tot * 3 + (size_t)nj * 8 + 64));
    STRQ_HIP(c, c->bnd.reserve(bnd_floats * 4 + 256));
    STRQ_HIP(c, c->rec.reserve(rec_tot * 4 + 256));
    STRQ_HIP(c, c->lutinfo.reserve((size_t)nj * (sizeof(LutJob) + sizeof(LutInfo))));
    STRQ_HIP(c, c->hard.reserve((size_t)hard_cap * (sizeof(HardEntry) + 4) + 64));
    STRQ_HIP(c, c->queue.reserve(STRQ_QUEUE_BYTES));
    STRQ_HIP(c, hipMemcpyAsync(c->flank_cls.p, p.h_cls.data(), cls_tot * 4, hipMemcpyHostToDevice, st));
    STRQ_HIP(c, hipMemcpyAsync(c->col0.p, h_col0.data(), col0_tot * 4, hipMemcpyHostToDevice, st));
    STRQ_HIP(c, hipMemsetAsync(c->queue.p, 0, STRQ_QUEUE_BYTES, st));
    return STRQ_OK;
}

struct TableBuild {
    int nj = 0, max_k = 0;
    std::vector<LutJob>* jobs = nullptr;
    const float* d_level_val = nullptr;
    std::vector<int> job_read;
    std::vector<const float*> job_cls;
    std::function<int()> after_tables;
    std::vector<LutInfo>* info = nullptr;
    std::vector<LutInfo>* reported = nullptr;
    std::vector<HardEntry>* handed = nullptr;
    int hard_count = 0;
};

static int run_table_build(strq_ctx* c, hipStream_t st, TableBuild& b)
{
    const int nj = b.nj;
    std::vector<LutJob>& jobs = *b.jobs;
    std::vector<LutInfo>& info = *b.info;
    LutJob* d_jobs = c->lutinfo.as<LutJob>();
    LutInfo* d_info = reinterpret_cast<LutInfo*>(d_jobs + nj);
    STRQ_HIP(c, hipMemcpyAsync(d_jobs, jobs.data(), (size_t)nj * sizeof(LutJob), hipMemcpyHostToDevice, st));
    HardEntry* d_hard = c->hard.as<HardEntry>();
    float* d_hard_vals = reinterpret_cast<float*>(d_hard + hard_cap);
    int* d_hard_count = c->queue.as<int>();
    STRQ_HIP(c, hipEventRecord(c->ev[0], st));
    if (launch_lut_build(st, d_jobs, d_info, nj, b.max_k, d_hard, d_hard_count, hard_cap, c->ap)) { c->err = "lut launch failed"; return STRQ_ERR_DEVICE; }
    STRQ_HIP(c, hipEventRecord(c->ev[1], st));
    if (b.after_tables) { const int arc = b.after_tables(); if (arc) return arc; }
    info.resize(nj);
    int hard_count = 0;
    STRQ_HIP(c, hipMemcpyAsync(info.data(), d_info, (size_t)nj * sizeof(LutInfo), hipMemcpyDeviceToHost, st));
    STRQ_HIP(c, hipMemcpyAsync(&hard_count, d_hard_count, 4, hipMemcpyDeviceToHost, st));
    STRQ_HIP(c, hipStreamSynchronize(st));
    if (b.reported) *b.reported = info;
    STRQ_DBG("lut done jobs=%d hard=%d floats0=%d", nj, hard_count, info[0].total);
    if (strq::opt("STRQ_DEBUG")) { int hist[9] = {0}; for (int i = 0; i < nj; ++i) hist[std::min(8, info[i].need / 8)]++; STRQ_DBG("band need histogram (x8 levels): %d %d %d %d %d %d %d %d %d", hist[0], hist[1], hist[2], hist[3], hist[4], hist[5], hist[6], hist[7], hist[8]); }
    if (strq::opt("STRQ_DEBUG")) { long tot = 0; int mx = 0; for (int i = 0; i < nj; ++i) { tot += info[i].total; mx = std::max(mx, info[i].total); } STRQ_DBG("table floats: mean %.0f max %d (k=%d)", (double)tot / nj, mx, jobs[0].k); }
    if (hard_count > hard_cap) { c->err = "too many borderline table entries"; return STRQ_ERR_DEVICE; }
    bool any_rebuild = false;
    for (int j = 0; j < nj; ++j) any_rebuild |= info[j].n_hard < 0;
    auto level_vals_of = [&](int read, float* dst) -> int {
        STRQ_HIP(c, hipMemcpy(dst, b.d_level_val + (size_t)read * 256, 256 * 4, hipMemcpyDeviceToHost));
        return STRQ_OK;
    };
    if (hard_count > 0) {
        std::vector<HardEntry> he(hard_count); std::vector<float> hv(hard_count);
        STRQ_HIP(c, hipMemcpy(he.data(), d_hard, (size_t)hard_count * sizeof(HardEntry), hipMemcpyDeviceToHost));
        float lv[256]; int last_read = -1;
        for (int i = 0; i < hard_count; ++i) {
            const int rd = b.job_read[he[i].job];
            if (rd != last_read) { const int rc = level_vals_of(rd, lv); if (rc) return rc; last_read = rd; }
            hv[i] = host_cell_score(c->ap, lv[he[i].level], b.job_cls[he[i].job][he[i].k]);
        }
        STRQ_HIP(c, hipMemcpyAsync(d_hard_vals, hv.data(), (size_t)hard_count * 4, hipMemcpyHostToDevice, st));
        if (launch_lut_patch(st, d_jobs, d_hard, d_hard_vals, hard_count)) { c->err = "patch launch failed"; return STRQ_ERR_DEVICE; }
        STRQ_HIP(c, hipStreamSynchronize(st));
        if (b.handed) *b.handed = he;
    } else if (b.handed) b.handed->clear();
    if (any_rebuild) for (int j = 0; j < nj; ++j) if (info[j].n_hard < 0) {
        const int kk = jobs[j].k;
        std::vector<float> tab((size_t)kk * 256); std::vector<int32_t> blo(kk);
        float lv[256];
        { const int rc = level_vals_of(b.job_read[j], lv); if (rc) return rc; }
        for (int x = 0; x < kk; ++x) {
            float* row = &tab[(size_t)x * 256];
            for (int q = 0; q < 256; ++q) row[q] = host_cell_score(c->ap, lv[q], b.job_cls[j][x]);
            blo[x] = (int32_t)((255u << 8) | ((uint32_t)(x * 256) << 16));
        }
        STRQ_HIP(c, hipMemcpy(jobs[j].table, tab.data(), tab.size() * 4, hipMemcpyHostToDevice));
        STRQ_HIP(c, hipMemcpy(jobs[j].band_lo, blo.data(), (size_t)kk * 4, hipMemcpyHostToDevice));
        info[j].total = kk * 256; info[j].need = 256;
    }
    b.hard_count = hard_count;
    return STRQ_OK;
}

static uint8_t* table3_slot(strq_ctx* c, size_t tab_off, int j)
{
    const size_t o = tab_off * 3 + (size_t)j * 8;
    return c->tables3.as<uint8_t>() + o - o % 4;
}

static int build_tables(CorePlan& p)
{
    strq_ctx* c = p.c; const AlignCoreIn& in = p.in;
    const int nb = p.nb, nj = p.nj;
    std::vector<LutJob>& jobs = p.jobs;
    jobs.resize(nj);
    TableBuild b;
    b.nj = nj; b.max_k = p.max_k; b.jobs = &jobs; b.d_level_val = in.d_level_val; b.after_tables = in.after_tables; b.info = &p.info;
    b.job_read.resize(nj); b.job_cls.resize(nj);
    for (int j = 0; j < nj; ++j) {
        const int i = p.job_align[j];
        jobs[j].level_val = in.d_level_val + (size_t)in.read[i] * 256;
        jobs[j].cls_val = c->flank_cls.as<float>() + p.cls_off[i] + p.job_k0[j];
        jobs[j].table = c->tables.as<float>() + p.tab_off[j];
        jobs[j].table3 = table3_slot(c, p.tab_off[j], j);
        jobs[j].band_lo = c->band_lo.as<int32_t>() + p.desc_off[j];
        jobs[j].k = p.job_k[j]; jobs[j].pad_ = 0;
        b.job_read[j] = in.read[i];
        b.job_cls[j] = &p.h_cls[p.cls_off[i] + p.job_k0[j]];
    }
    const int rc = run_table_build(c, p.st, b);
    if (rc) return rc;
    p.tab_total.assign(nb, 0);
    for (int j = 0; j < nj; ++j) p.tab_total[p.job_align[j]] = std::max(p.tab_total[p.job_align[j]], p.info[j].total);
    p.out.n_hard = b.hard_count;
    return STRQ_OK;
}

static void read_switches(CorePlan& p)
{
    const strq_ctx* c = p.c;
    p.collapsed = p.S == 6 && c->ap.open_h == c->ap.ext_h && c->ap.open_v == c->ap.ext_v;
    if (const char* e = strq::opt("STRQ_SEG")) { const int v = atoi(e); if (v >= 1 && v <= 4) p.seg_want = v; }
    if (const char* e = strq::opt("STRQ_TABLES")) { const int v = atoi(e); if (v >= 1 && v <= 8) p.max_tables = v; }
    if (const char* e = strq::opt("STRQ_MAX_WAVES")) { const int v = atoi(e); if (v >= 4 && v <= 16) p.max_waves = v; }
    p.allow_pack = p.collapsed && !strq::opt("STRQ_NO_PACK");
    if (const char* e = strq::opt("STRQ_OVERLAP")) { const int v = atoi(e); p.ov_cap = v > 0 ? v : (1 << 30); p.ov_fixed = true; }
    p.scr_forced = strq::opt("STRQ_SCREEN_ALWAYS") != nullptr;
    const char* mode_opt = strq::opt("STRQ_SCREEN_MODE");
    p.mode_fine = mode_opt && std::strcmp(mode_opt, "fine") == 0;
    p.mode_coarse = mode_opt && std::strcmp(mode_opt, "coarse") == 0;
}


struct ScreenJob {
    int flanks = 1;
    std::vector<int> al;
    std::vector<ScreenTask> views;
    std::vector<Screen2Task> t2;
    std::vector<int32_t> bound;
    std::vector<size_t> out_off;
    size_t out_words = 0, lds_bytes = 0;
    int lanes_rows = 0;
    double steps = 0;
};

struct ScreenRules {
    int merge;
    int groups_per_cu;
    const char* lds_err;
    bool below_bound_free;
    bool count_untaken;
    bool judge;
    double max_cols;
    int* pause; int* fail;
};

static void screen_tasks(CorePlan& p, const ScreenParams& sp, ScreenJob& j)
{
    constexpr int SSEG = STRQ_SCREEN_SEG;
    const AlignCoreIn& in = p.in;
    const int F = j.flanks, ng = (int)j.al.size() / F;
    if (F == 2) j.t2.resize((size_t)ng * SSEG);
    j.views.resize(j.al.size() * SSEG);
    j.bound.resize(j.al.size());
    j.out_off.assign(j.al.size() * SSEG, 0);
    for (int g = 0; g < ng; ++g) {
        const int* a = &j.al[(size_t)g * F];
        const int n = in.n[a[0]];
        const int m_big = F == 2 ? std::max(in.m[a[0]], in.m[a[1]]) : in.m[a[0]];
        const int ov_worst = align_segment_overlap(p.c->ap, m_big), ov_s = overlap_for(p, m_big, ov_worst, 16);
        Piece pc[SSEG];
        const int used = cut(n, SSEG, ov_s, pc);
        j.lds_bytes = std::max(j.lds_bytes, F == 2 ? screen2_lds_bytes(p.info[p.J0[a[0]]].total, p.info[p.J0[a[1]]].total) : screen_lds_bytes(p.info[p.J0[a[0]]].total));
        if (F == 2) j.lanes_rows = std::max(j.lanes_rows, screen2_lanes_rows(p.info[p.J0[a[0]]].need, p.info[p.J0[a[1]]].need));
        for (int f = 0; f < F; ++f)
            j.bound[(size_t)g * F + f] = used <= 1 ? INT32_MIN / 2 : (ov_s >= ov_worst ? 0 : (int32_t)std::ceil((double)align_segment_min_score(p.c->ap, in.m[a[f]], ov_s) * sp.sc));
        for (int w = 0; w < SSEG; ++w) {
            Screen2Task t; std::memset(&t, 0, sizeof(t));
            t.levels = in.d_levels + in.read_off[in.read[a[0]]] + pc[w].col_off;
            t.n = pc[w].n; t.col_off = pc[w].col_off;
            t.n_chunks = pc[w].n > 0 ? (align_num_steps(pc[w].n) + 63) / 64 : 0;
            for (int f = 0; f < F; ++f) {
                const LutJob& job = p.jobs[p.J0[a[f]]];
                t.table[f] = job.table; t.band_lo[f] = job.band_lo; t.tsize[f] = p.info[p.J0[a[f]]].total; t.k[f] = in.k[a[f]];
                ScreenTask v; std::memset(&v, 0, sizeof(v));
                v.n = pc[w].n; v.m = in.m[a[f]]; v.k = in.k[a[f]]; v.col_off = pc[w].col_off; v.n_chunks = t.n_chunks;
                if (F == 2) v.lane_last = f * STRQ_SCREEN2_LANE_B + (in.k[a[f]] - 1) / STRQ_SCREEN2_CPL;
                else { v.levels = t.levels; v.table = t.table[0]; v.band_lo = t.band_lo[0]; v.tsize = t.tsize[0]; v.lane_last = (v.m - 1) / STRQ_SCREEN_R; }
                j.out_off[((size_t)g * F + f) * SSEG + w] = j.out_words; j.out_words += (size_t)t.n_chunks;
                j.views[((size_t)g * F + f) * SSEG + w] = v;
            }
            if (pc[w].n > 0) j.steps += align_num_steps(pc[w].n);
            if (F == 2) j.t2[(size_t)g * SSEG + w] = t;
        }
    }
}

static int run_screen(CorePlan& p, ScreenJob& j, const ScreenParams& sp, const ScreenRules& r)
{
    constexpr int SSEG = STRQ_SCREEN_SEG;
    strq_ctx* c = p.c; const AlignCoreIn& in = p.in;
    hipStream_t st = p.st;
    const int nv = (int)j.al.size();
    int lanes_rows = 0;
    if (j.flanks == 2) {
        const char* e = strq::opt("STRQ_SCREEN_LDS");
        if (!(e && std::strcmp(e, "rows") == 0) && screen2_lanes_fit(j.lanes_rows)) { lanes_rows = j.lanes_rows; j.lds_bytes = screen2_lanes_lds_bytes(lanes_rows); }
    }
    if (j.lds_bytes > 160 * 1024 - 64) { c->err = r.lds_err; return STRQ_ERR_UNSUPPORTED; }
    const int groups = std::max(1, std::min(r.groups_per_cu, (int)((160 * 1024 - 64) / j.lds_bytes)));
    auto aligned = [](size_t bytes) { return (bytes + 255) & ~(size_t)255; };
    const size_t t2_bytes = aligned(j.t2.size() * sizeof(Screen2Task)), task_bytes = aligned(j.views.size() * sizeof(ScreenTask));
    const size_t bound_bytes = aligned((size_t)nv * 4), win_bytes = aligned((size_t)nv * sizeof(ScreenWindows));
    STRQ_HIP(c, c->screen.reserve(t2_bytes + task_bytes + bound_bytes + win_bytes + j.out_words * 4 + 256));
    char* base = c->screen.as<char>();
    Screen2Task* d_t2 = reinterpret_cast<Screen2Task*>(base);
    ScreenTask* d_st = reinterpret_cast<ScreenTask*>(base + t2_bytes);
    int32_t* d_bound = reinterpret_cast<int32_t*>(base + t2_bytes + task_bytes);
    ScreenWindows* d_win = reinterpret_cast<ScreenWindows*>(base + t2_bytes + task_bytes + bound_bytes);
    int32_t* d_out = reinterpret_cast<int32_t*>(base + t2_bytes + task_bytes + bound_bytes + win_bytes);
    for (size_t x = 0; x < j.views.size(); ++x) j.views[x].out = d_out + j.out_off[x];
    if (j.flanks == 2)
        for (int v = 0; v < nv; ++v) for (int w = 0; w < SSEG; ++w) j.t2[(size_t)(v / 2) * SSEG + w].out[v % 2] = j.views[(size_t)v * SSEG + w].out;
    if (j.flanks == 2) STRQ_HIP(c, hipMemcpyAsync(d_t2, j.t2.data(), j.t2.size() * sizeof(Screen2Task), hipMemcpyHostToDevice, st));
    STRQ_HIP(c, hipMemcpyAsync(d_st, j.views.data(), j.views.size() * sizeof(ScreenTask), hipMemcpyHostToDevice, st));
    STRQ_HIP(c, hipMemcpyAsync(d_bound, j.bound.data(), (size_t)nv * 4, hipMemcpyHostToDevice, st));
    STRQ_HIP(c, hipEventRecord(c->ev[5], st));
    int* queue = c->queue.as<int>() + STRQ_QUEUE_FIRST - 1;
    if (j.flanks == 2) {
        if (launch_screen2(st, d_t2, nv / 2, queue, sp, j.lds_bytes, groups, c->n_cu, r.merge, lanes_rows)) { c->err = "coarse screen launch failed"; return STRQ_ERR_DEVICE; }
    } else {
        if (launch_screen(st, d_st, nv, queue, sp, j.lds_bytes, groups, c->n_cu)) { c->err = "screen launch failed"; return STRQ_ERR_DEVICE; }
    }
    STRQ_HIP(c, hipEventRecord(c->ev[6], st));
    if (launch_screen_windows(st, d_st, nv, sp, d_bound, d_win)) { c->err = "screen windows launch failed"; return STRQ_ERR_DEVICE; }
    std::vector<ScreenWindows> hw((size_t)nv);
    STRQ_HIP(c, hipMemcpyAsync(hw.data(), d_win, hw.size() * sizeof(ScreenWindows), hipMemcpyDeviceToHost, st));
    STRQ_HIP(c, hipStreamSynchronize(st));
    c->screen_ran = true; c->screen_mode_last = r.merge > 1 ? 2 : 1; c->coarse_merge_last = r.merge;
    c->screen_lds_last = j.flanks == 2 ? (lanes_rows > 0 ? 1 : 2) : 0;
    if (const char* path = strq::opt("STRQ_SCREEN_DUMP")) {
        std::vector<int32_t> ho(j.out_words);
        STRQ_HIP(c, hipMemcpy(ho.data(), d_out, j.out_words * 4, hipMemcpyDeviceToHost));
        if (FILE* fp = fopen(path, "wb")) {
            const int32_t hdr[8] = {nv, sp.sc, sp.hh, sp.v, j.flanks, SSEG, sp.slack, r.merge};
            fwrite(hdr, 4, 8, fp);
            for (int v = 0; v < nv; ++v) {
                const int32_t gh[4] = {j.al[v], j.al[v], j.bound[v], j.views[(size_t)v * SSEG].lane_last};
                fwrite(gh, 4, 4, fp);
                for (int w = 0; w < SSEG; ++w) {
                    const ScreenTask& t = j.views[(size_t)v * SSEG + w];
                    const int32_t th[4] = {t.col_off, t.n, t.m, t.n_chunks};
                    fwrite(th, 4, 4, fp);
                    fwrite(ho.data() + (t.out - d_out), 4, (size_t)t.n_chunks, fp);
                }
                fwrite(&hw[(size_t)v], sizeof(ScreenWindows), 1, fp);
            }
            fclose(fp);
        }
    }
    if (const char* e = strq::opt("STRQ_SCREEN_TEST_RAISE")) {
        const float up = (float)atof(e);
        for (auto& w : hw) w.lower_bound += up;
    }
    int windowed = 0, heavy = 0, below_bound = 0; double cols = 0, all = 0;
    for (int v = 0; v < nv; ++v) {
        const int al = j.al[v];
        const ScreenWindows& w = hw[(size_t)v];
        c->screen_stats[1] += 1; c->screen_stats[7] += w.n_cand;
        double mine = in.n[al];
        if (w.n_win > 0) {
            p.wins[al] = w; c->screen_stats[2] += 1; ++windowed; mine = 0;
            for (int k = 0; k < w.n_win; ++k) { c->screen_stats[4] += w.hi[k] - w.lo[k] + 1; mine += w.hi[k] - w.lo[k] + 1 + 4096; }
        } else {
            c->screen_stats[3] += 1;
            if (w.n_cand == 0) { ++below_bound; if (r.below_bound_free) mine = 0; }
        }
        all += in.n[al]; cols += mine; heavy += mine > 4 * 32768.0;
    }
// ... 97 lines not shown
        } else {
            if (!p.collapsed || strq::opt("STRQ_NO_SCREEN") || (c->screen_pause > 0 && !p.scr_forced)) continue;
            merge = 1;
        }
        const int rc = screen_two_flank(p, merge, max_n);
        if (rc) return rc;
    }
    if (p.screen2_ran) return STRQ_OK;
    if (p.collapsed && c->screen_pause > 0 && !p.scr_forced) {
        --c->screen_pause; c->screen_stats[3] += nb;
        return STRQ_OK;
    }
    ScreenParams sp;
    if (p.collapsed && screen_plan(c->ap, p.S, max_n, &sp)) return screen_one_flank(p, sp);
    return STRQ_OK;
}

static int plan_launches(CorePlan& p)
{
    strq_ctx* c = p.c; const AlignCoreIn& in = p.in; AlignCoreOut& out = p.out;
    const int nb = p.nb;
    std::vector<ScreenWindows>& wins = p.wins;
    static const double rate[5][2] = {{0, 0}, {1.017, 0.941}, {0.79, 0.862}, {0.85, 0.85}, {0.69, 0.80}};
    p.packed.assign(nb, 0); p.overlap.assign(nb, 0); p.segs_of.assign(nb, 1);
    std::vector<char> segmentable(nb, 0);
    const bool force_pack = strq::opt("STRQ_PACK") != nullptr;
    int class_count[5] = {0, 0, 0, 0, 0};
    for (int i = 0; i < nb; ++i) {
        segmentable[i] = p.collapsed && in.NS[i] == 1;
        p.overlap[i] = segmentable[i] ? align_segment_overlap(c->ap, in.m[i]) : 0;
        const bool can_pack = p.allow_pack && in.NS[i] == 1 && p.info[p.J0[i]].packed && p.info[p.J0[i]].n_hard == 0;
        int best_s = 1, best_p = can_pack ? 1 : 0;
        if (segmentable[i]) {
            const double l = overlap_for(p, in.m[i], p.overlap[i]);
            double best_cost = 0;
            for (int sgs : {1, 2, 3, 4}) {
                if (p.seg_want ? sgs != p.seg_want : sgs == 3) continue;
                if (sgs > 1 && !p.seg_want && (l <= 0 || in.n[i] < (sgs + 1) * l)) continue;
                for (int pk = 0; pk < 2; ++pk) {
                    if ((pk && !can_pack) || (force_pack && can_pack && !pk)) continue;
                    const double cost = (in.n[i] + (sgs - 1) * l) * rate[sgs][pk];
                    if (best_cost == 0 || cost < best_cost) { best_cost = cost; best_s = sgs; best_p = pk; }
                }
            }
        }
        if (wins[i].n_win > 0) {
            ScreenWindows& w = wins[i];
            while (w.n_win < STRQ_SCREEN_MAX_WINDOWS) {
                int widest = 0;
                for (int k2 = 1; k2 < w.n_win; ++k2) if (w.hi[k2] - w.lo[k2] > w.hi[widest] - w.lo[widest]) widest = k2;
                if (w.hi[widest] - w.lo[widest] < 16384) break;
                const int mid = w.lo[widest] + (w.hi[widest] - w.lo[widest]) / 2;
                for (int k2 = w.n_win; k2 > widest + 1; --k2) { w.lo[k2] = w.lo[k2 - 1]; w.hi[k2] = w.hi[k2 - 1]; }
                w.lo[widest + 1] = mid + 1; w.hi[widest + 1] = w.hi[widest]; w.hi[widest] = mid;
                ++w.n_win;
            }
            const int nw = w.n_win;
            best_s = p.seg_want >= nw ? p.seg_want : (nw <= 2 ? nw : 4); best_p = 0;
        }
        p.segs_of[i] = best_s; p.packed[i] = (char)best_p;
        ++class_count[best_s];
    }
    std::vector<int>& segs_of = p.segs_of;
    if (!p.seg_want && !c->screen_ran) {
        int few = 2 * c->n_cu;
        if (const char* e = strq::opt("STRQ_CLASS_MIN")) few = atoi(e);
        if (class_count[4] && class_count[4] < few) { for (int i = 0; i < nb; ++i) if (segs_of[i] == 4) { segs_of[i] = 2; if (wins[i].n_win > 2) wins[i].n_win = 0; } class_count[2] += class_count[4]; class_count[4] = 0; }
        if (class_count[2] && class_count[2] < few && class_count[1]) { for (int i = 0; i < nb; ++i) if (segs_of[i] == 2) { segs_of[i] = 1; if (wins[i].n_win > 1) wins[i].n_win = 0; } class_count[1] += class_count[2]; class_count[2] = 0; }
    }
    std::map<std::tuple<int, int, int, int, int>, std::vector<int>> groups;
    for (int i = 0; i < nb; ++i) {
        const int w = tables_for(p, p.packed[i] ? packed_dwords(p.tab_total[i]) : p.tab_total[i], segs_of[i]);
        if (w < 1) { c->err = "score table does not fit LDS"; return STRQ_ERR_UNSUPPORTED; }
        groups[std::make_tuple(in.R[i], in.NS[i], -segs_of[i], -w, p.packed[i] ? 0 : 1)].push_back(i);
    }
    const int min_rounds = 4;
    for (auto it = groups.begin(); it != groups.end();) {
        auto nx = std::next(it);
        const int w = -std::get<3>(it->first);
        const bool same_kind = nx != groups.end() && std::get<0>(nx->first) == std::get<0>(it->first) && std::get<1>(nx->first) == std::get<1>(it->first)
                               && std::get<2>(nx->first) == std::get<2>(it->first)
                               && !(std::get<4>(it->first) == 1 && std::get<4>(nx->first) == 0);
        if (same_kind && (long)it->second.size() < (long)min_rounds * w * c->n_cu) {
            nx->second.insert(nx->second.end(), it->second.begin(), it->second.end());
            it = groups.erase(it);
        } else ++it;
    }
    out.order.clear(); out.order.reserve(nb);
    for (auto& g : groups) {
        auto& v = g.second;
        auto work = [&](int x) {
            if (wins[x].n_win <= 0) return (long)in.n[x];
            long w = 0;
            for (int k = 0; k < wins[x].n_win; ++k) w += wins[x].hi[k] - wins[x].lo[k] + 1 + 4096;
            return w;
        };
        std::stable_sort(v.begin(), v.end(), [&](int x, int y) { return work(x) > work(y); });
        const int NS = std::get<1>(g.first);
        const int pk = std::get<4>(g.first) == 0;
        int lds_floats = 0;
        for (int i : v) lds_floats = std::max(lds_floats, pk ? packed_dwords(p.tab_total[i]) : p.tab_total[i]);
        const int segs = -std::get<2>(g.first);
        const int tables = std::min(-std::get<3>(g.first), tables_for(p, lds_floats, segs));
        if (tables < 1) { c->err = "score table does not fit LDS"; return STRQ_ERR_UNSUPPORTED; }
        bool known = std::get<0>(g.first) == 14;
        for (int i : v) known = known && in.m[i] == 870;
        p.launches.push_back({std::get<0>(g.first), NS, tables, (int)out.order.size(), (int)v.size(), (int)p.n_tasks, 0, lds_floats, pk, segs, known});
        out.order.insert(out.order.end(), v.begin(), v.end());
        p.n_tasks += (size_t)v.size() * segs;
        if (NS > 1) p.n_up += (int)v.size() * (NS - 1);
    }
    { size_t up = p.n_tasks; for (auto& L : p.launches) if (L.NS > 1) { L.first_up = (int)up; up += (size_t)L.count * (L.NS - 1); } }
    return STRQ_OK;
}

static int cut_pieces(CorePlan& p)
{
    strq_ctx* c = p.c; const AlignCoreIn& in = p.in; const AlignCoreOut& out = p.out;
    const int nb = p.nb;
    const size_t n_tasks = p.n_tasks;
    p.safe0 = n_tasks + p.n_up + (size_t)nb;
    p.pieces.resize(n_tasks); p.safe.resize(n_tasks);
    p.min_score.assign(nb, -INFINITY);
    p.two_round.assign(p.launches.size(), 0);
    p.ck_up.assign(nb, 0);
    size_t ck_floats = 0;
    for (size_t li = 0; li < p.launches.size(); ++li) {
        auto& L = p.launches[li];
        for (int x = 0; x < L.count; ++x) {
            const int pos = L.first + x, i = out.order[pos];
            const int n = in.n[i], R = in.R[i], ov = p.overlap[i];
            const size_t per_ckpt = (size_t)STRQ_CKPT_FIELDS(R) * 64;
            Piece* pf = &p.pieces[(size_t)L.first_task + (size_t)x * L.segs];
            Piece* ps = &p.safe[(size_t)L.first_task + (size_t)x * L.segs];
            cut(n, L.segs, ov, ps);
            const int ov_fast = overlap_for(p, in.m[i], ov);
            if (p.wins[i].n_win > 0) {
                const ScreenWindows& w = p.wins[i];
                const int ov_w = std::min(ov > 0 ? ov : (1 << 30), align_overlap_for_score(c->ap, in.m[i], w.lower_bound));
                for (int k = 0; k < L.segs; ++k) {
                    if (k < w.n_win) { const int start = std::max(0, w.lo[k] - 1 - ov_w); pf[k].col_off = start; pf[k].n = w.hi[k] - start; }
                    else { pf[k].col_off = 0; pf[k].n = 0; }
                }
                p.min_score[pos] = std::max(w.lower_bound, align_segment_min_score(c->ap, in.m[i], ov_w));
                p.two_round[li] = 1;
            } else if (L.segs > 1 && ov_fast < ov && cut(n, L.segs, ov_fast, pf) > 1) {
                p.min_score[pos] = align_segment_min_score(c->ap, in.m[i], ov_fast);
                p.two_round[li] = 1;
            } else {
                for (int k = 0; k < L.segs; ++k) pf[k] = ps[k];
            }
            for (int k = 0; k < L.segs; ++k) {
                pf[k].ck = ps[k].ck = ck_floats;
                ck_floats += (size_t)align_num_ckpts(std::max(pf[k].n, ps[k].n)) * per_ckpt;
            }
            if (L.NS > 1) { p.ck_up[i] = ck_floats; ck_floats += (size_t)(L.NS - 1) * align_num_ckpts(n) * per_ckpt; }
        }
    }
    for (char t : p.two_round) p.any_two_round |= t != 0;
    const size_t n_all_tasks = p.safe0 + (p.any_two_round ? n_tasks : 0);
    STRQ_HIP(c, c->ckpt.reserve(ck_floats * 4 + 256));
    p.r2_cap = p.screen2_ran ? std::max(1024, std::min(nb, 8192)) : 0;
    p.r2_0 = n_all_tasks;
    STRQ_HIP(c, c->tasks.reserve((n_all_tasks + (size_t)p.r2_cap * 4) * sizeof(AlignTask)));
    STRQ_HIP(c, c->results.reserve((2 * n_tasks + nb) * sizeof(AlignResult) + (size_t)nb * 12 + p.launches.size() * 4 + 256));
    p.tasks.resize(n_all_tasks);
    p.d_tasks = c->tasks.as<AlignTask>();
    p.d_heads = p.d_tasks + n_tasks + p.n_up;
    p.d_seg = c->results.as<AlignResult>();
    p.d_res = p.d_seg + n_tasks;
    p.d_seg_safe = p.d_res + nb;
    p.d_pick = reinterpret_cast<int32_t*>(p.d_seg_safe + n_tasks);
    p.d_min_score = reinterpret_cast<float*>(p.d_pick + nb);
    p.d_redo = reinterpret_cast<int*>(p.d_min_score + nb);
    p.d_redo_count = p.d_redo + nb;
    return STRQ_OK;
}

static int write_tasks(CorePlan& p)
{
    strq_ctx* c = p.c; const AlignCoreIn& in = p.in; AlignCoreOut& out = p.out;
    const int nb = p.nb, S = p.S;
    hipStream_t st = p.st;
    const size_t n_tasks = p.n_tasks, n_up = p.n_up, safe0 = p.safe0;
    std::vector<AlignTask>& tasks = p.tasks;
    for (auto& L : p.launches) {
        for (int x = 0; x < L.count; ++x) {
            const int pos = L.first + x, i = out.order[pos];
            const int R = in.R[i], M = in.m[i];
            AlignTask base; std::memset(&base, 0, sizeof(base));
            base.levels = in.d_levels + in.read_off[in.read[i]];
            base.rec = c->rec.as<int32_t>() + out.rec_off[i];
            base.n = in.n[i]; base.n_full = in.n[i]; base.m_total = M;
            auto strip = [&](int row0, int rows, size_t ck, int sidx) {
                AlignTask t = base;
                const int j = p.NJ[i] > 1 ? p.J0[i] + sidx : p.J0[i];
                const int k0 = row0 / S, k1 = (row0 + rows - 1) / S;
                t.row0 = row0; t.m = rows; t.k = k1 - k0 + 1; t.tsize = p.info[j].total;
                t.table = p.jobs[j].table; t.table3 = p.jobs[j].table3; t.band_lo = p.jobs[j].band_lo + (k0 - p.job_k0[j]);
                t.col0 = c->col0.as<float>() + p.col0_off[i] + row0;
                t.ckpt = c->ckpt.as<float>() + ck;
                return t;
            };
            tasks[n_tasks + n_up + pos] = strip(0, M, 0, 0);
            if (L.NS == 1) {
                for (int k = 0; k < L.segs; ++k) {
                    const size_t ti = (size_t)L.first_task + (size_t)x * L.segs + k;
                    AlignTask t = strip(0, M, p.pieces[ti].ck, 0);
                    t.levels += p.pieces[ti].col_off; t.n = p.pieces[ti].n; t.col_off = p.pieces[ti].col_off;
                    tasks[ti] = t;
                    if (p.any_two_round) {
                        AlignTask u = strip(0, M, p.safe[ti].ck, 0);
                        u.levels += p.safe[ti].col_off; u.n = p.safe[ti].n; u.col_off = p.safe[ti].col_off;
                        tasks[safe0 + ti] = u;
                    }
                }
            } else {
                const int rows_s = 64 * R;
                const size_t ck_strip = (size_t)align_num_ckpts(in.n[i]) * STRQ_CKPT_FIELDS(R) * 64;
                float* bnd = c->bnd.as<float>() + p.bnd_off[i];
                const size_t bnd_stride = 2 * ((size_t)in.n[i] + 2);
                for (int sidx = 0; sidx < L.NS; ++sidx) {
                    const bool last = sidx == L.NS - 1;
                    const int row0 = sidx * rows_s, rows = last ? M - row0 : rows_s;
                    const size_t slot = last ? (size_t)L.first_task + x : (size_t)L.first_up + (size_t)sidx * L.count + x;
                    AlignTask t = strip(row0, rows, last ? p.pieces[(size_t)L.first_task + x].ck : p.ck_up[i] + (size_t)sidx * ck_strip, sidx);
                    if (sidx > 0) { t.bnd_in = bnd + (size_t)(sidx - 1) * bnd_stride; t.up = p.d_tasks + L.first_up + (size_t)(sidx - 1) * L.count + x; }
                    if (!last) t.bnd_out = bnd + (size_t)sidx * bnd_stride;
                    tasks[slot] = t;
                    if (last && p.any_two_round) tasks[safe0 + slot] = t;
                }
            }
        }
    }
    STRQ_HIP(c, hipMemcpyAsync(p.d_tasks, tasks.data(), tasks.size() * sizeof(AlignTask), hipMemcpyHostToDevice, st));
    STRQ_HIP(c, hipMemsetAsync(p.d_seg, 0, (2 * n_tasks + nb) * sizeof(AlignResult), st));
    if (p.any_two_round) {
        STRQ_HIP(c, hipMemcpyAsync(p.d_min_score, p.min_score.data(), (size_t)nb * 4, hipMemcpyHostToDevice, st));
        STRQ_HIP(c, hipMemsetAsync(p.d_redo_count, 0, p.launches.size() * 4, st));
    }
    size_t scratch_words = 0;
    for (auto& L : p.launches) scratch_words = std::max(scratch_words, align_trace_scratch_words_per_wave(L.R));
    STRQ_HIP(c, c->scratch.reserve(scratch_words * 8 * (size_t)c->n_cu * trace_wpb));
    out.n_launches = 0; out.wave_steps = 0; out.columns = 0;
    for (size_t t = 0; t < n_tasks + n_up; ++t) if (tasks[t].n > 0) { out.wave_steps += align_num_steps(tasks[t].n); out.columns += tasks[t].n; }
    if (!p.launches.empty()) {
        const Launch& L = p.launches.back(); out.segs = L.segs; out.tables = L.tables; out.packed = L.packed; out.rows_per_lane = L.R;
        const int i = out.order[L.first];
        out.overlap_worst = p.overlap[i]; out.overlap_first = L.segs > 1 ? overlap_for(p, in.m[i], p.overlap[i]) : 0;
        const bool seg_kernel = L.NS == 1 && p.collapsed;
        const int32_t g[8] = {L.segs, L.tables, seg_kernel ? align_segments_wpe(L.segs, L.tables) : 0, L.R, L.packed, out.overlap_first, out.overlap_worst, (int32_t)p.launches.size()};
        std::memcpy(c->geometry, g, sizeof(g));
    }
    return STRQ_OK;
}

static int run_forward(CorePlan& p)
{
    strq_ctx* c = p.c; AlignCoreOut& out = p.out;
    const int S = p.S;
    hipStream_t st = p.st;
    const std::vector<Launch>& launches = p.launches;
    for (auto& L : launches) p.max_ns = std::max(p.max_ns, L.NS);
    if ((size_t)STRQ_QUEUE_FIRST + launches.size() * ((size_t)p.max_ns + 2) + 16 > (size_t)STRQ_QUEUE_SLOTS) {
        c->err = "too many distinct (flank shape, table size) groups in one batch"; return STRQ_ERR_UNSUPPORTED;
    }
    bool side = false;
    std::vector<hipStream_t> lstream(launches.size(), st);
    if (c->screen_ran && launches.size() > 1 && p.max_ns == 1 && p.collapsed) {
        side = true;
        if (!c->ev_fork) STRQ_HIP(c, hipEventCreateWithFlags(&c->ev_fork, hipEventDisableTiming));
        STRQ_HIP(c, hipEventRecord(c->ev_fork, st));
        size_t biggest = 0;
        for (size_t li = 1; li < launches.size(); ++li) if (launches[li].count > launches[biggest].count) biggest = li;
        if (!c->side_stream) { STRQ_HIP(c, hipStreamCreateWithFlags(&c->side_stream, hipStreamNonBlocking)); STRQ_HIP(c, hipEventCreateWithFlags(&c->side_join, hipEventDisableTiming)); }
        STRQ_HIP(c, hipStreamWaitEvent(c->side_stream, c->ev_fork, 0));
        lstream[biggest] = c->side_stream;
    }
    for (int level = 0; level < p.max_ns; ++level) {
        for (size_t lidx = 0; lidx < launches.size(); ++lidx) {
            const Launch& L = launches[lidx];
            hipStream_t lst = lstream[lidx];
            if (level >= L.NS) continue;
            STRQ_DBG("forward launch R=%d strips=%d slice dwords=%d packed=%d level=%d count=%d tables/CU=%d segments=%d", L.R, L.NS, L.lds_floats, L.packed, level, L.count, L.tables, L.segs);
            int rc;
            if (L.NS == 1 && p.collapsed) {
                rc = launch_align_segments(lst, L.R, S, p.d_tasks + L.first_task, p.d_seg + L.first_task, L.count, L.segs, c->queue.as<int>() + p.qi,
                                           c->ap, L.lds_floats, L.tables, c->n_cu, L.packed, nullptr, nullptr, L.known_last_row);
            } else {
                const bool last = level == L.NS - 1;
                const AlignTask* dt = last ? p.d_tasks + L.first_task : p.d_tasks + L.first_up + (size_t)level * L.count;
                const int mode = (level > 0 ? 1 : 0) | (last ? 0 : 2);
                rc = launch_align(st, L.R, S, dt, p.d_seg + L.first_task, L.count, c->queue.as<int>() + p.qi, c->ap, L.lds_floats, L.tables, c->n_cu,
                                  c->scratch.as<uint64_t>(), 0, mode, L.packed);
            }
            if (rc) { c->err = "align launch failed"; return STRQ_ERR_DEVICE; }
            ++p.qi; ++out.n_launches;
        }
    }
    if (side) {
        STRQ_HIP(c, hipEventRecord(c->side_join, c->side_stream));
        STRQ_HIP(c, hipStreamWaitEvent(st, c->side_join, 0));
    }
    for (size_t li = 0; li < launches.size(); ++li) {
        const Launch& L = launches[li];
        int* redo = p.d_redo + L.first; int* cnt = p.d_redo_count + li;
        if (launch_align_combine(st, p.d_tasks + L.first_task, p.d_seg + L.first_task, L.count, L.segs, p.d_res + L.first, p.d_pick + L.first, L.first_task,
                                 nullptr, nullptr, p.two_round[li] ? p.d_min_score + L.first : nullptr, redo, cnt,
                                 c->redo_total.p ? c->redo_total.as<unsigned int>() : nullptr)) { c->err = "combine launch failed"; return STRQ_ERR_DEVICE; }
    }
    return STRQ_OK;
}

struct Look2 { int pos, i, g2; float b1; };

static void keep_whole_read(const CorePlan& p, std::vector<std::vector<int>>& redo_keep, int pos)
{
    for (size_t li = 0; li < p.launches.size(); ++li) {
        const Launch& L = p.launches[li];
        if (pos >= L.first && pos < L.first + L.count) redo_keep[li].push_back(pos - L.first);
    }
}

static int look2_run(CorePlan& p, const std::vector<Look2>& l2, std::vector<std::vector<int>>& redo_keep)
{
    strq_ctx* c = p.c; const AlignCoreIn& in = p.in; AlignCoreOut& out = p.out;
    const int nb = p.nb, S = p.S;
    hipStream_t st = p.st;
    const ScreenParams& sp2 = p.sp2;
    const int n2 = (int)l2.size();
    const size_t o_list = 0, o_theta = o_list + (size_t)n2 * 4, o_win = (o_theta + (size_t)n2 * 4 + 15) & ~(size_t)15,
                 o_pos = o_win + (size_t)n2 * sizeof(ScreenWindows), o_seg = (o_pos + (size_t)n2 * 4 + 15) & ~(size_t)15,
                 o_res = o_seg + (size_t)n2 * 4 * sizeof(AlignResult), o_pick = o_res + (size_t)n2 * sizeof(AlignResult), o_end = o_pick + (size_t)n2 * 4;
    STRQ_HIP(c, c->misc.reserve(o_end + 256));
    char* mb = c->misc.as<char>();
    std::vector<int32_t> h_list((size_t)n2), h_theta((size_t)n2), h_pos((size_t)n2);
    for (int k2 = 0; k2 < n2; ++k2) {
        const Look2& e = l2[(size_t)k2];
        h_list[(size_t)k2] = e.g2; h_pos[(size_t)k2] = e.pos;
        const double b1s = std::floor((double)e.b1 * sp2.sc);
        h_theta[(size_t)k2] = (int32_t)std::max(-2.0e9, std::min(2.0e9, b1s + (double)in.m[e.i] * sp2.v - (double)sp2.slack));
    }
    STRQ_HIP(c, hipMemcpyAsync(mb + o_list, h_list.data(), (size_t)n2 * 4, hipMemcpyHostToDevice, st));
    STRQ_HIP(c, hipMemcpyAsync(mb + o_theta, h_theta.data(), (size_t)n2 * 4, hipMemcpyHostToDevice, st));
    STRQ_HIP(c, hipMemcpyAsync(mb + o_pos, h_pos.data(), (size_t)n2 * 4, hipMemcpyHostToDevice, st));
    if (launch_screen_windows(st, p.d_st2, n2, sp2, p.d_bound2, reinterpret_cast<ScreenWindows*>(mb + o_win),
                              reinterpret_cast<const int32_t*>(mb + o_list), reinterpret_cast<const int32_t*>(mb + o_theta))) { c->err = "screen windows launch failed"; return STRQ_ERR_DEVICE; }
    std::vector<ScreenWindows> w2((size_t)n2);
    STRQ_HIP(c, hipMemcpyAsync(w2.data(), mb + o_win, (size_t)n2 * sizeof(ScreenWindows), hipMemcpyDeviceToHost, st));
    STRQ_HIP(c, hipStreamSynchronize(st));
    std::map<int, std::vector<int>> by_R;
    for (int k2 = 0; k2 < n2; ++k2) {
        if (w2[(size_t)k2].n_win > 0) by_R[in.R[l2[(size_t)k2].i]].push_back(k2);
        else keep_whole_read(p, redo_keep, l2[(size_t)k2].pos);
    }
    const int piece_cols = 8192;
    std::vector<AlignTask> t2; t2.reserve((size_t)n2 * 4);
    std::vector<int32_t> pos_sorted, grp_first;
    size_t ck2 = 0; int slot = 0, n_grp = 0; double cols2 = 0;
    struct G2 { int R, first_grp, n_grp, lds, tables; bool known; };
    std::vector<G2> groups2;
    const size_t r2_task_cap = (size_t)p.r2_cap * 4;
    for (auto& kv : by_R) {
        G2 g{kv.first, n_grp, 0, 0, 0, kv.first == 14};
        for (int k2 : kv.second) {
            const Look2& e = l2[(size_t)k2];
            const ScreenWindows& w = w2[(size_t)k2];
            const int ov = p.overlap[e.i];
            const int ov_w = std::min(ov > 0 ? ov : (1 << 30), align_overlap_for_score(c->ap, in.m[e.i], w.lower_bound));
            int need = 0;
            for (int q = 0; q < w.n_win; ++q) need += (w.hi[q] - w.lo[q] + piece_cols) / piece_cols;
            need = (need + 3) & ~3;
            if (t2.size() + (size_t)need > r2_task_cap) { keep_whole_read(p, redo_keep, e.pos); continue; }
            const AlignTask& head = p.tasks[p.n_tasks + p.n_up + (size_t)e.pos];
            const size_t per_ckpt = (size_t)STRQ_CKPT_FIELDS(in.R[e.i]) * 64;
            int made = 0;
            for (int q = 0; q < w.n_win; ++q) {
                const int len = w.hi[q] - w.lo[q] + 1, np = (len + piece_cols - 1) / piece_cols;
                for (int j = 0; j < np; ++j) {
                    const int own_lo = w.lo[q] + (int)((long)len * j / np), own_hi = w.lo[q] + (int)((long)len * (j + 1) / np) - 1;
                    AlignTask t = head;
                    const int start = std::max(0, own_lo - 1 - ov_w);
                    t.levels = head.levels + start; t.n = own_hi - start; t.col_off = start;
                    t.ckpt = reinterpret_cast<float*>((uintptr_t)ck2 * 4);
                    ck2 += (size_t)align_num_ckpts(t.n) * per_ckpt;
                    cols2 += t.n; out.wave_steps += align_num_steps(t.n); out.columns += t.n;
                    t2.push_back(t); ++made;
                }
                c->screen_stats[4] += len;
            }
            for (; made < need; ++made) { AlignTask t = head; t.n = 0; t.col_off = 0; t2.push_back(t); }
            g.lds = std::max(g.lds, p.tab_total[e.i]); g.known = g.known && in.m[e.i] == 870;
            pos_sorted.push_back(e.pos); grp_first.push_back(n_grp); n_grp += need / 4; ++slot;
        }
        g.n_grp = n_grp - g.first_grp;
        if (g.n_grp <= 0) continue;
        g.tables = tables_for(p, g.lds, 4);
        if (g.tables < 1) { c->err = "score table does not fit LDS"; return STRQ_ERR_UNSUPPORTED; }
        groups2.push_back(g);
    }
    grp_first.push_back(n_grp);
    c->look2_served += slot;
    if (slot > 0) {
        const size_t p_seg = 0, p_res = p_seg + (size_t)n_grp * 4 * sizeof(AlignResult), p_pick = p_res + (size_t)n_grp * sizeof(AlignResult),
                     p_first = p_pick + (size_t)n_grp * 4, p_pos = p_first + ((size_t)slot + 1) * 4, p_end = p_pos + (size_t)slot * 4;
        STRQ_HIP(c, c->ckpt2.reserve(ck2 * 4 + 256 + p_end + 256));
        char* rb = c->ckpt2.as<char>() + ((ck2 * 4 + 255) & ~(size_t)255);
        for (size_t x = 0; x < t2.size(); ++x) if (t2[x].n > 0) t2[x].ckpt = c->ckpt2.as<float>() + ((uintptr_t)t2[x].ckpt / 4);
        AlignResult* d_seg2 = reinterpret_cast<AlignResult*>(rb + p_seg); AlignResult* d_res2 = reinterpret_cast<AlignResult*>(rb + p_res);
        int32_t* d_pick2 = reinterpret_cast<int32_t*>(rb + p_pick);
        AlignTask* d_tasks2 = p.d_tasks + p.r2_0;
        STRQ_HIP(c, hipMemcpyAsync(d_tasks2, t2.data(), t2.size() * sizeof(AlignTask), hipMemcpyHostToDevice, st));
        STRQ_HIP(c, hipMemcpyAsync(rb + p_first, grp_first.data(), grp_first.size() * 4, hipMemcpyHostToDevice, st));
        STRQ_HIP(c, hipMemcpyAsync(rb + p_pos, pos_sorted.data(), (size_t)slot * 4, hipMemcpyHostToDevice, st));
        STRQ_HIP(c, hipMemsetAsync(d_seg2, 0, (size_t)n_grp * 4 * sizeof(AlignResult), st));
        for (const G2& g : groups2) {
            if (launch_align_segments(st, g.R, S, d_tasks2 + (size_t)g.first_grp * 4, d_seg2 + (size_t)g.first_grp * 4, g.n_grp, 4, c->queue.as<int>() + p.qi,
                                      c->ap, g.lds, g.tables, c->n_cu, 0, nullptr, nullptr, g.known)) { c->err = "align launch failed"; return STRQ_ERR_DEVICE; }
            ++p.qi; ++out.n_launches;
            if (launch_align_combine(st, d_tasks2 + (size_t)g.first_grp * 4, d_seg2 + (size_t)g.first_grp * 4, g.n_grp, 4, d_res2 + g.first_grp, d_pick2 + g.first_grp,
                                     (int)p.r2_0 + g.first_grp * 4)) { c->err = "combine launch failed"; return STRQ_ERR_DEVICE; }
        }
        if (launch_align_scatter(st, d_res2, d_pick2, reinterpret_cast<const int32_t*>(rb + p_first), reinterpret_cast<const int32_t*>(rb + p_pos), slot, p.d_res, p.d_pick)) { c->err = "scatter launch failed"; return STRQ_ERR_DEVICE; }
    }
    const bool forced = p.scr_forced || p.mode_coarse || c->screen_mode_last == 1;
    if (p.coarse_all > 0 && (p.coarse_cols + cols2 > 0.30 * p.coarse_all || 3 * n2 > nb) && nb >= 64 && !forced && c->coarse_pause == 0) pause_after_fail(c->coarse_pause, c->coarse_fail);
    STRQ_DBG("coarse screen, second look: %d alignments, %.2f %% of the columns (first look %.2f %%) -> pause %d", slot, 100.0 * cols2 / std::max(1.0, p.coarse_all), 100.0 * p.coarse_cols / std::max(1.0, p.coarse_all), c->coarse_pause);
    return STRQ_OK;
}

static int second_look(CorePlan& p, bool allow_bail, bool* bailed)
{
    if (!p.screen2_ran || !p.any_two_round || p.r2_cap <= 0) return STRQ_OK;
    strq_ctx* c = p.c; const AlignCoreOut& out = p.out;
    const int nb = p.nb;
    hipStream_t st = p.st;
    const std::vector<Launch>& launches = p.launches;
    std::vector<std::vector<int>> redo_keep(launches.size());
    std::vector<int> cnt(launches.size()), hredo((size_t)nb);
    std::vector<AlignResult> hres((size_t)nb);
    STRQ_HIP(c, hipMemcpyAsync(cnt.data(), p.d_redo_count, launches.size() * 4, hipMemcpyDeviceToHost, st));
    STRQ_HIP(c, hipMemcpyAsync(hredo.data(), p.d_redo, (size_t)nb * 4, hipMemcpyDeviceToHost, st));
    STRQ_HIP(c, hipMemcpyAsync(hres.data(), p.d_res, (size_t)nb * sizeof(AlignResult), hipMemcpyDeviceToHost, st));
    STRQ_HIP(c, hipStreamSynchronize(st));
    std::vector<Look2> l2;
    bool any_redo = false;
    for (size_t li = 0; li < launches.size(); ++li) {
        if (!p.two_round[li]) continue;
        const Launch& L = launches[li];
        for (int x = 0; x < cnt[li]; ++x) {
            const int a = hredo[(size_t)L.first + x], pos = L.first + a, i = out.order[pos];
            any_redo = true;
            if (p.g2_of[i] >= 0 && p.wins[i].n_win > 0 && (int)l2.size() < p.r2_cap && L.NS == 1) l2.push_back({pos, i, p.g2_of[i], hres[(size_t)pos].best});
            else redo_keep[li].push_back(a);
        }
    }
    size_t n_redo = l2.size();
    for (auto& v : redo_keep) n_redo += v.size();
    const bool forced = p.scr_forced || p.mode_coarse || c->screen_mode_last == 1;
    if (allow_bail && !forced && nb >= 64 && 3 * n_redo > (size_t)nb && !strq::opt("STRQ_SCREEN2_NO_BAIL")) {
        pause_after_fail(c->coarse_pause, c->coarse_fail);
        float ms = 0;
        STRQ_HIP(c, hipEventRecord(c->ev[3], st));
        STRQ_HIP(c, hipStreamSynchronize(st));
        STRQ_HIP(c, hipEventElapsedTime(&ms, c->ev[2], c->ev[3])); c->aborted_fwd_ms += ms;
        STRQ_HIP(c, hipEventElapsedTime(&ms, c->ev[5], c->ev[6])); c->aborted_screen_ms += ms;
        c->look2_served += (int64_t)n_redo;
        STRQ_DBG("coarse screen: %zu of %d alignments missed the first look's certificate -> the sub-batch starts over with the fine screen, pause %d", n_redo, nb, c->coarse_pause);
        *bailed = true;
        return STRQ_OK;
    }
    if (!l2.empty()) {
        const int rc = look2_run(p, l2, redo_keep);
        if (rc) return rc;
    }
    if (any_redo) {
        std::vector<int> redo_keep_n(launches.size(), 0);
        for (size_t li = 0; li < launches.size(); ++li) {
            if (!p.two_round[li]) continue;
            redo_keep_n[li] = (int)redo_keep[li].size();
            if (!redo_keep[li].empty()) STRQ_HIP(c, hipMemcpyAsync(p.d_redo + launches[li].first, redo_keep[li].data(), redo_keep[li].size() * 4, hipMemcpyHostToDevice, st));
        }
        STRQ_HIP(c, hipMemcpyAsync(p.d_redo_count, redo_keep_n.data(), launches.size() * 4, hipMemcpyHostToDevice, st));
    }
    return STRQ_OK;
}

static int second_round_and_trace(CorePlan& p)
{
    strq_ctx* c = p.c; AlignCoreOut& out = p.out;
    const int S = p.S;
    hipStream_t st = p.st;
    const std::vector<Launch>& launches = p.launches;
    for (size_t li = 0; li < launches.size(); ++li) {
        const Launch& L = launches[li];
        int* redo = p.d_redo + L.first; int* cnt = p.d_redo_count + li;
        if (!p.two_round[li]) continue;
        if (launch_align_segments(st, L.R, S, p.d_tasks + p.safe0 + L.first_task, p.d_seg_safe + L.first_task, L.count, L.segs, c->queue.as<int>() + p.qi,
                                  c->ap, L.lds_floats, L.tables, c->n_cu, L.packed, redo, cnt, L.known_last_row)) { c->err = "align launch failed"; return STRQ_ERR_DEVICE; }
        ++p.qi;
        if (launch_align_combine(st, p.d_tasks + p.safe0 + L.first_task, p.d_seg_safe + L.first_task, L.count, L.segs, p.d_res + L.first, p.d_pick + L.first,
                                 (int)p.safe0 + L.first_task, redo, cnt, nullptr, nullptr, nullptr)) { c->err = "combine launch failed"; return STRQ_ERR_DEVICE; }
    }
    STRQ_HIP(c, hipEventRecord(c->ev[3], st));
    for (size_t li = 0; li < launches.size();) {
        const Launch& L = launches[li];
        int count = L.count, lds_floats = L.lds_floats;
        size_t lj = li + 1;
        for (; lj < launches.size(); ++lj) {
            const Launch& M = launches[lj];
            if (M.R != L.R || M.NS != L.NS || M.packed != L.packed || L.NS != 1 || M.first != L.first + count) break;
            count += M.count; lds_floats = std::max(lds_floats, M.lds_floats);
        }
        const int wpb = std::min(trace_wpb, (160 * 1024) / (std::max(lds_floats, 1) * 4));
        if (launch_align(st, L.R, S, p.d_tasks, p.d_res + L.first, count, c->queue.as<int>() + p.qi, c->ap, lds_floats, wpb, c->n_cu,
                         c->scratch.as<uint64_t>(), 1, 0, L.packed, p.d_pick + L.first)) { c->err = "trace launch failed"; return STRQ_ERR_DEVICE; }
        ++p.qi; li = lj;
    }
    STRQ_HIP(c, hipEventRecord(c->ev[4], st));
    out.d_tasks = p.d_heads; out.d_results = p.d_res; out.d_rec = c->rec.as<int32_t>();
    return STRQ_OK;
}

static int align_core_once(strq_ctx* c, const AlignCoreIn& in, AlignCoreOut& out, bool allow_bail, bool* bailed)
{
    CorePlan p(c, in, out);
    int rc;
    if ((rc = upload_inputs(p))) return rc;
    if ((rc = build_tables(p))) return rc;
    read_switches(p);
    if ((rc = run_screens(p))) return rc;
    if ((rc = plan_launches(p))) return rc;
    if ((rc = cut_pieces(p))) return rc;
    if ((rc = write_tasks(p))) return rc;
    if ((rc = run_forward(p))) return rc;
    bool bail = false;
    if ((rc = second_look(p, allow_bail, &bail))) return rc;
    if (bail) { *bailed = true; return STRQ_OK; }
    return second_round_and_trace(p);
}

int align_core(strq_ctx* c, const AlignCoreIn& in, AlignCoreOut& out)
{
    double saved[8];
    std::memcpy(saved, c->screen_stats, sizeof(saved));
    bool bailed = false;
    const int rc = align_core_once(c, in, out, true, &bailed);
    if (rc || !bailed) return rc;
    std::memcpy(c->screen_stats, saved, sizeof(saved));
    return align_core_once(c, in, out, false, &bailed);
}

int align_core_times(strq_ctx* c, float* t_lut, float* t_fwd, float* t_tr)
{
    float ms;
    STRQ_HIP(c, hipEventElapsedTime(&ms, c->ev[0], c->ev[1])); *t_lut += ms;
    STRQ_HIP(c, hipEventElapsedTime(&ms, c->ev[2], c->ev[3])); *t_fwd += ms + c->aborted_fwd_ms;
    c->screen_stats[0] += c->aborted_screen_ms;
    c->aborted_fwd_ms = c->aborted_screen_ms = 0;
    STRQ_HIP(c, hipEventElapsedTime(&ms, c->ev[3], c->ev[4])); *t_tr += ms;
    if (c->screen_ran) { STRQ_HIP(c, hipEventElapsedTime(&ms, c->ev[5], c->ev[6])); c->screen_stats[0] += ms; }
    return STRQ_OK;
}

size_t align_workspace_bytes(int n, int m, int R, int NS)
{
    size_t b = (size_t)NS * (align_num_ckpts(n) + align_num_ckpts(n) / 4 + 300) * STRQ_CKPT_FIELDS(R) * 64 * 4;
    if (NS > 1) b += (size_t)(NS - 1) * ((size_t)n + 2) * 8;
    (void)m;
    return b;
}

int align_validate_flank(strq_ctx* c, const float* f, int64_t mm, int samples, int* k_out, int* R_out, int* NS_out)
{
    if (mm < 1 || samples < 1 || mm % samples != 0) { c->err = "flank length must be a positive multiple of `samples`"; return STRQ_ERR_UNSUPPORTED; }
    for (int64_t i = 0; i < mm; ++i)
        if (std::memcmp(&f[i], &f[i - i % samples], 4) != 0) { c->err = "flank is not made of runs of `samples` equal values"; return STRQ_ERR_UNSUPPORTED; }
    const int S = align_effective_samples(samples);
    int R = 0, NS = 0;
    if (mm > (1 << 20) || !align_plan((int)mm, S, &R, &NS)) { c->err = "flank shape not covered by the compiled kernels"; return STRQ_ERR_UNSUPPORTED; }
    if (S == 6 && mm / S > STRQ_LUT_MAX_K && NS == 1) { R = 12; NS = (int)((mm + 64 * 12 - 1) / (64 * 12)); }
    *k_out = (int)(mm / S); *R_out = R; *NS_out = NS;
    return STRQ_OK;
}

static int run_align_batch(strq_ctx* c, const BatchIn& in, const BatchOut& out)
{
    const int S = align_effective_samples(in.samples);
    const int64_t NA = in.n_align;
    std::fill(c->timing, c->timing + 8, 0.0f);
    for (double& v : c->screen_stats) v = 0;
    if (NA == 0) return STRQ_OK;
    std::vector<int> m(NA), k(NA), R(NA), n(NA), NS(NA);
    for (int64_t a = 0; a < NA; ++a) {
        const int64_t mm = in.flank_off[a + 1] - in.flank_off[a];
        const int rd = in.align_read[a];
        if (rd < 0 || rd >= in.n_reads) { c->err = "align_read out of range"; return STRQ_ERR_ARG; }
        const int64_t nn = in.read_off[rd + 1] - in.read_off[rd];
        if (nn < 0 || nn > (int64_t)1 << 30) { c->err = "bad read length"; return STRQ_ERR_ARG; }
        const int rc = align_validate_flank(c, in.flank + in.flank_off[a], mm, in.samples, &k[a], &R[a], &NS[a]);
        if (rc) return rc;
        m[a] = (int)mm; n[a] = (int)nn;
    }
    hipStream_t st = c->stream;
    c->second_round[0] = 0; c->second_round[1] = NA; c->look2_served = 0;
    STRQ_HIP(c, c->redo_total.reserve(64));
    STRQ_HIP(c, hipMemsetAsync(c->redo_total.p, 0, 64, st));
    const int64_t tot_levels = in.read_off[in.n_reads];
    STRQ_HIP(c, c->levels.reserve((size_t)tot_levels + 64));
    STRQ_HIP(c, c->level_val.reserve((size_t)in.n_reads * 256 * 4));
    STRQ_HIP(c, hipMemcpyAsync(c->levels.p, in.levels, (size_t)tot_levels, hipMemcpyHostToDevice, st));
    STRQ_HIP(c, hipMemcpyAsync(c->level_val.p, in.level_val, (size_t)in.n_reads * 256 * 4, hipMemcpyHostToDevice, st));
    int64_t a0 = 0;
    float t_lut = 0, t_fwd = 0, t_tr = 0, n_hard = 0, n_launch = 0;
    std::fill(c->counters, c->counters + 8, 0.0);
    while (a0 < NA) {
        int64_t a1 = a0; size_t ck_bytes = 0;
        while (a1 < NA) {
            const size_t need = align_workspace_bytes(n[a1], m[a1], R[a1], NS[a1]);
            if (a1 > a0 && ck_bytes + need > c->max_ws_bytes) break;
            ck_bytes += need; ++a1;
        }
        const int nb = (int)(a1 - a0);
        AlignCoreIn ci; AlignCoreOut co;
        ci.nb = nb; ci.samples = S; ci.d_levels = c->levels.as<uint8_t>(); ci.read_off = in.read_off;
        ci.d_level_val = c->level_val.as<float>();
        std::vector<const float*> fl(nb);
        for (int i = 0; i < nb; ++i) fl[i] = in.flank + in.flank_off[a0 + i];
        ci.read = in.align_read + a0; ci.n = &n[a0]; ci.m = &m[a0]; ci.k = &k[a0]; ci.R = &R[a0]; ci.NS = &NS[a0]; ci.flank = fl.data();
        int rc = align_core(c, ci, co);
        if (rc) return rc;
        std::vector<AlignResult> res(nb);
        std::vector<int32_t> h_rec(co.rec_total);
        STRQ_HIP(c, hipMemcpyAsync(res.data(), co.d_results, (size_t)nb * sizeof(AlignResult), hipMemcpyDeviceToHost, st));
        if (out.rec) STRQ_HIP(c, hipMemcpyAsync(h_rec.data(), co.d_rec, co.rec_total * 4, hipMemcpyDeviceToHost, st));
        STRQ_HIP(c, hipStreamSynchronize(st));
        for (int pos = 0; pos < nb; ++pos) {
            const int i = co.order[pos]; const int64_t a = a0 + i;
            if (out.score) out.score[a] = res[pos].best;
            if (out.j_end) out.j_end[a] = res[pos].j_end;
            if (out.j0) out.j0[a] = res[pos].j0;
            if (out.rec) std::memcpy(out.rec + in.flank_off[a], &h_rec[co.rec_off[i]], (size_t)m[a] * 4);
        }
        rc = align_core_times(c, &t_lut, &t_fwd, &t_tr);
        if (rc) return rc;
        n_hard += co.n_hard; n_launch += co.n_launches;
        c->counters[0] += co.wave_steps; c->counters[1] += co.columns; c->counters[2] += nb;
        c->counters[3] = co.segs; c->counters[4] = co.tables; c->counters[5] = co.packed; c->counters[6] = co.rows_per_lane;
        a0 = a1;
    }
    c->timing[0] = t_lut; c->timing[1] = t_fwd; c->timing[2] = t_tr; c->timing[3] = t_lut + t_fwd + t_tr; c->timing[4] = n_hard; c->timing[7] = n_launch;
    {
        unsigned int redo = 0;
        STRQ_HIP(c, hipMemcpy(&redo, c->redo_total.p, 4, hipMemcpyDeviceToHost));
        c->second_round[0] = (int64_t)redo - c->look2_served;
    }
    return STRQ_OK;
}

}

extern "C" {

int strq_abi_version(void) { return 13; }

int strq_set_option(strq_ctx* c, const char* key, const char* value)
{
    if (!key || std::strncmp(key, "STRQ_", 5) != 0) { if (c) c->err = "option keys start with STRQ_"; return STRQ_ERR_ARG; }
    if (c) { std::lock_guard<std::mutex> lk(c->options_mu); if (value) c->options[key] = value; else c->options.erase(key); return STRQ_OK; }
    std::lock_guard<std::mutex> lk(g_opt_mu);
    if (value) g_opts[key] = value; else g_opts.erase(key);
    return STRQ_OK;
}

int strq_get_option(const strq_ctx* c, const char* key, char* out, int32_t cap)
{
    if (!key || !out || cap < 1) return STRQ_ERR_ARG;
    CtxScope scope(c);
    const char* v = opt(key);
    out[0] = 0;
    if (!v) return STRQ_OK;
    std::strncpy(out, v, (size_t)cap - 1); out[cap - 1] = 0;
    return STRQ_OK;
}

int strq_ctx_create(int device_id, strq_ctx** out)
{
    if (!out) return STRQ_ERR_ARG;
    *out = nullptr;
    int ndev = 0;
    if (hipGetDeviceCount(&ndev) != hipSuccess || ndev <= 0 || device_id < 0 || device_id >= ndev) return STRQ_ERR_DEVICE;
    if (hipSetDevice(device_id) != hipSuccess) return STRQ_ERR_DEVICE;
    strq_ctx* c = new strq_ctx();
    c->device = device_id;
    hipDeviceProp_t prop;
    if (hipGetDeviceProperties(&prop, device_id) != hipSuccess) { delete c; return STRQ_ERR_DEVICE; }
    c->n_cu = prop.multiProcessorCount;
    if (hipStreamCreateWithFlags(&c->stream, hipStreamNonBlocking) != hipSuccess) { delete c; return STRQ_ERR_DEVICE; }
    for (auto& e : c->ev) if (hipEventCreate(&e) != hipSuccess) { delete c; return STRQ_ERR_DEVICE; }
    *out = c;
    return STRQ_OK;
}

void strq_ctx_destroy(strq_ctx* c)
{
    if (!c) return;
    (void)hipSetDevice(c->device);
    if (c->stream) (void)hipStreamSynchronize(c->stream);
    detect_state_free(c);
    for (HostModel* m : c->models) delete m;
    for (auto& e : c->ev) if (e) (void)hipEventDestroy(e);
    if (c->ev_fork) (void)hipEventDestroy(c->ev_fork);
    if (c->side_join) (void)hipEventDestroy(c->side_join);
    if (c->side_stream) (void)hipStreamDestroy(c->side_stream);
    if (c->stream) (void)hipStreamDestroy(c->stream);
    delete c;
}

int strq_debug_live_allocations(int64_t out[2])
{
    if (!out) return STRQ_ERR_ARG;
    out[0] = live_allocations[0].load(); out[1] = live_allocations[1].load();
    return STRQ_OK;
}

const char* strq_last_error(const strq_ctx* c) { return c ? c->err.c_str() : "null context"; }

int strq_set_align_params(strq_ctx* c, const float p[6])
{
    if (!c || !p) return STRQ_ERR_ARG;
    c->ap = AlignParams{p[0], p[1], p[2], p[3], p[4], p[5]};
    return STRQ_OK;
}
int strq_get_align_params(const strq_ctx* c, float p[6])
{
    if (!c || !p) return STRQ_ERR_ARG;
    p[0] = c->ap.open_h; p[1] = c->ap.ext_h; p[2] = c->ap.open_v; p[3] = c->ap.ext_v;
    p[4] = c->ap.dist_offset; p[5] = c->ap.dist_min;
    return STRQ_OK;
}

int strq_device_synchronize(strq_ctx* c)
{
    if (!c) return STRQ_ERR_ARG;
    STRQ_HIP(c, hipSetDevice(c->device));
    STRQ_HIP(c, hipDeviceSynchronize());
    return STRQ_OK;
}

int strq_last_timing(const strq_ctx* c, float ms[8])
{
    if (!c || !ms) return STRQ_ERR_ARG;
    std::memcpy(ms, c->timing, sizeof(c->timing));
    return STRQ_OK;
}

int strq_last_counters(const strq_ctx* c, double out[8])
{
    if (!c || !out) return STRQ_ERR_ARG;
    std::memcpy(out, c->counters, sizeof(c->counters));
    return STRQ_OK;
}

int strq_debug_screen_plan(const float params[6], int32_t samples, int32_t max_n, int32_t out[6])
{
    if (!params || !out) return 0;
    const AlignParams p{params[0], params[1], params[2], params[3], params[4], params[5]};
    ScreenParams sp;
    if (!screen_plan(p, samples, max_n, &sp)) return 0;
    out[0] = sp.sc; out[1] = sp.hh; out[2] = sp.v; out[3] = sp.cadd; out[4] = sp.slack; out[5] = sp.merge_gap;
    return 1;
}

int strq_debug_score_tables(strq_ctx* c, int32_t n_jobs, const float* level_val, const float* cls_val, const int64_t* cls_off,
                            int32_t* info_out, int32_t* band_lo, float* table, uint8_t* planes,
                            int32_t* handed, int32_t handed_cap, int32_t* n_handed)
{
    strq::CtxScope scope_(c);
    if (!c) return STRQ_ERR_ARG;
    if (n_jobs < 1 || n_jobs > 4096 || !level_val || !cls_val || !cls_off || !info_out || !band_lo || !table || !planes || !n_handed ||
        handed_cap < 0 || (handed_cap > 0 && !handed) || cls_off[0] != 0) { c->err = "bad argument"; return STRQ_ERR_ARG; }
    int max_k = 0;
    for (int j = 0; j < n_jobs; ++j) {
        const int64_t k = cls_off[j + 1] - cls_off[j];
        if (k < 1 || k > STRQ_LUT_MAX_K) { c->err = "a score table has 1 to 158 classes"; return STRQ_ERR_ARG; }
        max_k = std::max(max_k, (int)k);
    }
    STRQ_HIP(c, hipSetDevice(c->device));
    hipStream_t st = c->stream;
    const size_t cls_tot = (size_t)cls_off[n_jobs], tab_tot = STRQ_TABLE_SLOT_FLOATS(cls_tot);
    STRQ_HIP(c, c->level_val.reserve((size_t)n_jobs * 256 * 4));
    STRQ_HIP(c, c->flank_cls.reserve(cls_tot * 4));
    STRQ_HIP(c, c->band_lo.reserve(cls_tot * 4));
    STRQ_HIP(c, c->tables.reserve(tab_tot * 4));
    STRQ_HIP(c, c->tables3.reserve(tab_tot * 3 + (size_t)n_jobs * 8 + 64));
    STRQ_HIP(c, c->lutinfo.reserve((size_t)n_jobs * (sizeof(LutJob) + sizeof(LutInfo))));
    STRQ_HIP(c, c->hard.reserve((size_t)hard_cap * (sizeof(HardEntry) + 4) + 64));
    STRQ_HIP(c, c->queue.reserve(STRQ_QUEUE_BYTES));
    STRQ_HIP(c, hipMemcpyAsync(c->level_val.p, level_val, (size_t)n_jobs * 256 * 4, hipMemcpyHostToDevice, st));
    STRQ_HIP(c, hipMemcpyAsync(c->flank_cls.p, cls_val, cls_tot * 4, hipMemcpyHostToDevice, st));
    STRQ_HIP(c, hipMemsetAsync(c->queue.p, 0, STRQ_QUEUE_BYTES, st));
    STRQ_HIP(c, hipMemsetAsync(c->tables3.p, 0, tab_tot * 3 + (size_t)n_jobs * 8, st));
    std::vector<LutJob> jobs(n_jobs);
    std::vector<LutInfo> info, reported;
    std::vector<HardEntry> he;
    TableBuild b;
    b.nj = n_jobs; b.max_k = max_k; b.jobs = &jobs; b.d_level_val = c->level_val.as<float>(); b.info = &info; b.reported = &reported; b.handed = &he;
    b.job_read.resize(n_jobs); b.job_cls.resize(n_jobs);
    for (int j = 0; j < n_jobs; ++j) {
        const size_t tab_off = STRQ_TABLE_SLOT_FLOATS(cls_off[j]);
        jobs[j].level_val = c->level_val.as<float>() + (size_t)j * 256;
        jobs[j].cls_val = c->flank_cls.as<float>() + cls_off[j];
        jobs[j].table = c->tables.as<float>() + tab_off;
        jobs[j].table3 = table3_slot(c, tab_off, j);
        jobs[j].band_lo = c->band_lo.as<int32_t>() + cls_off[j];
        jobs[j].k = (int32_t)(cls_off[j + 1] - cls_off[j]); jobs[j].pad_ = 0;
        b.job_read[j] = j;
        b.job_cls[j] = cls_val + cls_off[j];
    }
    const int rc = run_table_build(c, st, b);
    if (rc) return rc;
    for (int j = 0; j < n_jobs; ++j) {
        info_out[5 * j] = reported[j].total; info_out[5 * j + 1] = reported[j].need; info_out[5 * j + 2] = reported[j].packed;
        info_out[5 * j + 3] = reported[j].n_hard; info_out[5 * j + 4] = info[j].total;
    }
    STRQ_HIP(c, hipMemcpy(band_lo, c->band_lo.p, cls_tot * 4, hipMemcpyDeviceToHost));
    STRQ_HIP(c, hipMemcpy(table, c->tables.p, tab_tot * 4, hipMemcpyDeviceToHost));
    for (int j = 0; j < n_jobs; ++j)
        STRQ_HIP(c, hipMemcpy(planes + (size_t)cls_off[j] * 768 + (size_t)j * 8, jobs[j].table3, (size_t)jobs[j].k * 768 + 8, hipMemcpyDeviceToHost));
    *n_handed = (int32_t)he.size();
    for (size_t i = 0; i < he.size() && (int64_t)i < handed_cap; ++i) {
        handed[4 * i] = he[i].job; handed[4 * i + 1] = he[i].k; handed[4 * i + 2] = he[i].level; handed[4 * i + 3] = he[i].index;
    }
    return STRQ_OK;
}

int strq_last_overlap(const strq_ctx* c, double out[4])
{
    if (!c || !out) return STRQ_ERR_ARG;
    for (int i = 0; i < 4; ++i) out[i] = c->overlap[i];
    return STRQ_OK;
}
int strq_last_screen(const strq_ctx* c, double out[8])
{
    if (!c || !out) return STRQ_ERR_ARG;
    for (int i = 0; i < 8; ++i) out[i] = c->screen_stats[i];
    return STRQ_OK;
}

int strq_last_screen_mode(const strq_ctx* c, int32_t out[8])
{
    if (!c || !out) return STRQ_ERR_ARG;
    for (int i = 0; i < 8; ++i) out[i] = 0;
    out[0] = c->screen_mode_last; out[1] = c->coarse_pause; out[2] = c->screen_pause; out[3] = (int32_t)c->coarse_margin;
    out[5] = (int32_t)std::min<int64_t>(c->look2_served, INT32_MAX);
    out[4] = c->screen_mode_last ? c->coarse_merge_last : 0;
    out[6] = c->screen_mode_last ? c->screen_lds_last : 0;
    return STRQ_OK;
}

int strq_last_second_round(const strq_ctx* c, int64_t out[2])
{
    if (!c || !out) return STRQ_ERR_ARG;
    out[0] = c->second_round[0]; out[1] = c->second_round[1];
    return STRQ_OK;
}

int strq_last_viterbi_launches(const strq_ctx* c, int32_t out[4])
{
    if (!c || !out) return STRQ_ERR_ARG;
    std::memcpy(out, c->vit_launches, sizeof(c->vit_launches));
    return STRQ_OK;
}

int strq_last_geometry(const strq_ctx* c, int32_t out[8])
{
    if (!c || !out) return STRQ_ERR_ARG;
    std::memcpy(out, c->geometry, sizeof(c->geometry));
    return STRQ_OK;
}

int strq_align_batch(strq_ctx* c, int64_t n_align, int64_t n_reads, const uint8_t* levels,
                     const int64_t* read_off, const float* level_val, const int32_t* align_read,
                     const float* flank, const int64_t* flank_off, int32_t samples,
                     float* score, int64_t* j_end, int64_t* j0, int32_t* rec)
{
    strq::CtxScope scope_(c);
    if (!c) return STRQ_ERR_ARG;
    if (n_align < 0 || n_reads < 0 || (n_align > 0 && (!levels || !read_off || !level_val || !align_read || !flank || !flank_off)) || samples < 1) {
        c->err = "bad argument"; return STRQ_ERR_ARG;
    }
    STRQ_HIP(c, hipSetDevice(c->device));
    BatchIn in{n_align, n_reads, levels, read_off, level_val, align_read, flank, flank_off, samples};
    BatchOut out{score, j_end, j0, rec};
    return run_align_batch(c, in, out);
}

static int align_overlap_generic(strq_ctx* c, const float* a, int64_t n, const float* b, int64_t m, float* score,
                                 std::vector<int32_t>& rec, int64_t* je, int64_t* j0)
{
    if (n > ((int64_t)1 << 30) || m > ((int64_t)1 << 24) || (double)(n + 1) * (double)(m + 1) > 1.7e10) {
        c->err = "align_overlap: (n + 1) x (m + 1) exceeds the 16 GiB trace limit of the generic path"; return STRQ_ERR_UNSUPPORTED;
    }
    hipStream_t st = c->stream;
    auto encode = [](const float* x, int64_t len, std::vector<float>& vals, std::vector<uint32_t>& code) {
        std::vector<uint32_t> bits((size_t)len);
        std::memcpy(bits.data(), x, (size_t)len * 4);
        std::vector<uint32_t> uniq(bits);
        std::sort(uniq.begin(), uniq.end());
        uniq.erase(std::unique(uniq.begin(), uniq.end()), uniq.end());
        code.resize((size_t)len);
        for (int64_t i = 0; i < len; ++i) code[(size_t)i] = (uint32_t)(std::lower_bound(uniq.begin(), uniq.end(), bits[(size_t)i]) - uniq.begin());
        vals.resize(uniq.size());
        std::memcpy(vals.data(), uniq.data(), uniq.size() * 4);
    };
    std::vector<float> va, vb; std::vector<uint32_t> ca, cb;
    encode(a, n, va, ca); encode(b, m, vb, cb);
    const size_t na = va.size(), nbv = vb.size();
    if ((double)na * (double)nbv > 2.0e9) { c->err = "align_overlap: more than 2e9 distinct (a, b) value pairs"; return STRQ_ERR_UNSUPPORTED; }
    const size_t tab = std::max<size_t>(1, na * nbv);
    const int hard_cap = 1 << 20;
    STRQ_HIP(c, c->gen_codes.reserve(((size_t)n + (size_t)m + na + nbv) * 4 + 64));
    STRQ_HIP(c, c->gen_table.reserve(tab * 4 + 64));
    STRQ_HIP(c, c->gen_bnd.reserve(((size_t)n + 1) * 16 + ((size_t)m + 1) * 4 + 256));
    STRQ_HIP(c, c->gen_trace.reserve(((size_t)n + 1) * ((size_t)m + 1) + 64));
    STRQ_HIP(c, c->gen_hard.reserve((size_t)hard_cap * (sizeof(GenericHard) + 4) + 64));
    STRQ_HIP(c, c->results.reserve(sizeof(AlignResult) + 64));
    STRQ_HIP(c, c->queue.reserve(STRQ_QUEUE_BYTES));
    uint32_t* d_ca = c->gen_codes.as<uint32_t>(); uint32_t* d_cb = d_ca + n;
    float* d_va = reinterpret_cast<float*>(d_cb + m); float* d_vb = d_va + na;
    float* d_tab = c->gen_table.as<float>();
    float* d_bnd = c->gen_bnd.as<float>();
    GenericHard* d_hard = c->gen_hard.as<GenericHard>(); float* d_hvals = reinterpret_cast<float*>(d_hard + hard_cap);
    int* d_count = c->queue.as<int>();
    if (n) STRQ_HIP(c, hipMemcpyAsync(d_ca, ca.data(), (size_t)n * 4, hipMemcpyHostToDevice, st));
    STRQ_HIP(c, hipMemcpyAsync(d_cb, cb.data(), (size_t)m * 4, hipMemcpyHostToDevice, st));
    if (na) STRQ_HIP(c, hipMemcpyAsync(d_va, va.data(), na * 4, hipMemcpyHostToDevice, st));
    STRQ_HIP(c, hipMemcpyAsync(d_vb, vb.data(), nbv * 4, hipMemcpyHostToDevice, st));
    STRQ_HIP(c, hipMemsetAsync(d_count, 0, 4, st));
    int hard_count = 0;
    if (na) {
        if (launch_generic_table(st, d_va, (int)na, d_vb, (int)nbv, d_tab, d_hard, d_count, hard_cap, c->ap)) { c->err = "table launch failed"; return STRQ_ERR_DEVICE; }
        STRQ_HIP(c, hipMemcpyAsync(&hard_count, d_count, 4, hipMemcpyDeviceToHost, st));
        STRQ_HIP(c, hipStreamSynchronize(st));
        if (hard_count > hard_cap) {
            std::vector<float> full(tab);
            for (size_t y = 0; y < nbv; ++y) for (size_t x = 0; x < na; ++x) full[y * na + x] = host_cell_score(c->ap, va[x], vb[y]);
            STRQ_HIP(c, hipMemcpy(d_tab, full.data(), tab * 4, hipMemcpyHostToDevice));
        } else if (hard_count > 0) {
            std::vector<GenericHard> he((size_t)hard_count); std::vector<float> hv((size_t)hard_count);
            STRQ_HIP(c, hipMemcpy(he.data(), d_hard, (size_t)hard_count * sizeof(GenericHard), hipMemcpyDeviceToHost));
            for (int i = 0; i < hard_count; ++i) hv[(size_t)i] = host_cell_score(c->ap, va[(size_t)he[(size_t)i].ia], vb[(size_t)he[(size_t)i].ib]);
            STRQ_HIP(c, hipMemcpyAsync(d_hvals, hv.data(), (size_t)hard_count * 4, hipMemcpyHostToDevice, st));
            if (launch_generic_patch(st, d_tab, (int)na, d_hard, d_hvals, hard_count)) { c->err = "patch launch failed"; return STRQ_ERR_DEVICE; }
        }
    }
    c->timing[4] = (float)hard_count;
    std::vector<float> col0((size_t)m + 1);
    host_col0(c->ap, (int)m, col0.data());
    GenericAlignArgs ga;
    ga.code_a = d_ca; ga.code_b = d_cb; ga.table = d_tab;
    ga.bnd_S[0] = d_bnd; ga.bnd_V[0] = d_bnd + (n + 1); ga.bnd_S[1] = d_bnd + 2 * (n + 1); ga.bnd_V[1] = d_bnd + 3 * (n + 1);
    float* d_col0 = d_bnd + 4 * (n + 1);
    STRQ_HIP(c, hipMemcpyAsync(d_col0, col0.data(), ((size_t)m + 1) * 4, hipMemcpyHostToDevice, st));
    ga.col0 = d_col0; ga.trace = c->gen_trace.as<uint8_t>(); ga.result = c->results.as<AlignResult>();
    ga.p = c->ap; ga.n = (int32_t)n; ga.m = (int32_t)m; ga.na = (int32_t)na; ga.nb = (int32_t)nbv;
    if (launch_generic_align(st, ga)) { c->err = "generic align launch failed"; return STRQ_ERR_DEVICE; }
    AlignResult res;
    std::vector<uint8_t> trace(((size_t)n + 1) * ((size_t)m + 1));
    STRQ_HIP(c, hipMemcpyAsync(&res, ga.result, sizeof(res), hipMemcpyDeviceToHost, st));
    STRQ_HIP(c, hipMemcpyAsync(trace.data(), ga.trace, trace.size(), hipMemcpyDeviceToHost, st));
    STRQ_HIP(c, hipStreamSynchronize(st));
    rec.assign((size_t)m, 0);
    int64_t i = m, j = res.j_end; int state = 0;
    const size_t W = (size_t)n + 1;
    while (i > 0 && j > 0) {
        const uint8_t tr = trace[(size_t)i * W + (size_t)j];
        if (state == 0) {
            const unsigned dsel = tr & 3u;
            if (dsel == 0) { rec[(size_t)i - 1] = (int32_t)(j << 1); --i; --j; }
            else state = (int)dsel;
        } else if (state == 1) { --j; if (!(tr & 4u)) state = 0; }
        else { rec[(size_t)i - 1] = (int32_t)((j << 1) | 1); --i; if (!(tr & 8u)) state = 0; }
    }
    for (; i > 0; --i) rec[(size_t)i - 1] = (int32_t)((j << 1) | 1);
    *score = res.best; *je = res.j_end; *j0 = j;
    return STRQ_OK;
}

int strq_align_overlap(strq_ctx* c, const float* a, int64_t n, const float* b, int64_t m, float* score,
                       uint64_t* a_idx, uint64_t* b_idx, int32_t* rec_out, int64_t* j_end_out, int64_t* j0_out)
{
    strq::CtxScope scope_(c);
    if (!c) return STRQ_ERR_ARG;
    if ((!a && n > 0) || !b || n < 0 || m < 1 || !score) { c->err = "bad argument"; return STRQ_ERR_ARG; }
    STRQ_HIP(c, hipSetDevice(c->device));
    std::fill(c->timing, c->timing + 8, 0.0f);
    std::vector<int32_t> rec((size_t)m);
    int64_t je = 0, j0 = 0;
    std::vector<float> vals(a, a + n);
    std::sort(vals.begin(), vals.end(), [](float x, float y) { return __builtin_bit_cast(uint32_t, x) < __builtin_bit_cast(uint32_t, y); });
    vals.erase(std::unique(vals.begin(), vals.end(), [](float x, float y) { return std::memcmp(&x, &y, 4) == 0; }), vals.end());
    int run = 0;
    { int64_t start = 0;
      for (int64_t i = 1; i <= m; ++i)
          if (i == m || std::memcmp(&b[i], &b[start], 4) != 0) { int len = (int)std::min<int64_t>(i - start, 1 << 20); run = run ? std::__gcd(run, len) : len; start = i; } }
    bool fast = vals.size() <= 256 && run >= 1 && !strq::opt("STRQ_GENERIC_ALIGN");
    for (float v : vals) if (v != v) fast = false;
    if (fast) {
        std::sort(vals.begin(), vals.end());
        for (size_t x = 1; x < vals.size(); ++x) if (vals[x] == vals[x - 1]) fast = false;
        int kk, RR, NN;
        if (fast && align_validate_flank(c, b, m, run, &kk, &RR, &NN) != STRQ_OK) fast = false;
    }
    if (fast) {
        std::vector<uint8_t> lv((size_t)n);
        for (int64_t i = 0; i < n; ++i) lv[(size_t)i] = (uint8_t)(std::lower_bound(vals.begin(), vals.end(), a[i]) - vals.begin());
// ... 33 lines not shown
```

### strique_amd/ffi.py

```python
import ctypes
import os

import numpy as np

_HERE = os.path.dirname(os.path.abspath(__file__))
LIB_PATH = os.environ.get("STRQ_LIB") or os.path.join(_HERE, "lib", "libstrique_hip.so")

STRQ_OK, STRQ_ERR_ARG, STRQ_ERR_DEVICE, STRQ_ERR_UNSUPPORTED, STRQ_ERR_NOMEM = 0, 1, 2, 3, 4

SCAN_SYMBOLS = ("strq_scan_batch_reads", "strq_scan_set", "strq_scan_clear", "strq_batch_fetch_scan")

_lib = None


class StriqueHipError(RuntimeError):
    def __init__(self, code, message):
        RuntimeError.__init__(self, "libstrique_hip error %d: %s" % (code, message))
        self.code = code


def _torch_hip_runtime():
    import importlib.util
    try:
        spec = importlib.util.find_spec("torch")
# ... 64 lines not shown
    out = np.zeros((len(offsets) - 1, 6), np.float64)
    rc = lib.strq_host_stats(_ptr(signals), _ptr(offsets), ctypes.c_int64(len(offsets) - 1), ctypes.c_int32(1 if want_raw else 0), _ptr(out))
    if rc != STRQ_OK:
        raise StriqueHipError(rc, "strq_host_stats: bad argument")
    return out


def live_allocations():
    out = np.zeros(2, np.int64)
    rc = load_library().strq_debug_live_allocations(_ptr(out))
    if rc != STRQ_OK:
        raise StriqueHipError(rc, "strq_debug_live_allocations: bad argument")
    return int(out[0]), int(out[1])


def _offsets(arrays, dtype):
    off = np.zeros(len(arrays) + 1, np.int64)
    for i, a in enumerate(arrays):
        off[i + 1] = off[i] + len(a)
    flat = np.concatenate([_c(a, dtype).ravel() for a in arrays] + [np.zeros(1, dtype)])
    return flat, off


_IMAGE_ORDER = ("src", "lp", "src2", "lp2", "start_lp", "kind", "hub", "ea", "eb", "ec", "end_src", "end_lp")
VARIANT_IMAGE_SHAPES = {"src": (np.int32, (2, 8, 64)), "lp": (np.float64, (2, 8, 64)), "src2": (np.int32, (3, 2, 4, 64)), "lp2": (np.float64, (3, 2, 4, 64)),
                        "start_lp": (np.float64, (2, 64)), "kind": (np.int32, (2, 64)), "hub": (np.int32, (2, 64)), "ea": (np.float64, (2, 64)),
                        "eb": (np.float64, (2, 64)), "ec": (np.float64, (2, 64)), "end_src": (np.int32, (4, 8)), "end_lp": (np.float64, (4, 8))}
MOD_LLR_IMAGE_SHAPES = dict(VARIANT_IMAGE_SHAPES, src2=(np.int32, (2, 4, 64)), lp2=(np.float64, (2, 4, 64)), start_lp=(np.float64, (2, 2, 64)),
                            end_src=(np.int32, (2, 8)), end_lp=(np.float64, (2, 8)))


def _debug_image(entry, shapes, baked, extra):
    lib = load_library()
    arrs = [_c(baked.in_ptr, np.int32), _c(baked.in_src, np.int32), _c(baked.in_logp, np.float64), _c(baked.emis_kind, np.int32),
            _c(baked.emis_a, np.float64), _c(baked.emis_b, np.float64), _c(baked.emis_c, np.float64),
            None if baked.tag is None else _c(baked.tag, np.int32)]
    brc = ctypes.c_int32(-1); head = np.zeros(10, np.int32); offs = np.zeros(12, np.int64); nbytes = ctypes.c_int64(0)
    image = np.zeros(1 << 16, np.uint8); why = ctypes.create_string_buffer(512)
    rc = getattr(lib, entry)(ctypes.c_int32(baked.n_states), ctypes.c_int32(baked.silent_start), ctypes.c_int32(baked.start), ctypes.c_int32(baked.end),
                             *([_ptr(a) for a in arrs] + extra + [ctypes.byref(brc), _ptr(head), _ptr(offs), _ptr(image), ctypes.c_int64(len(image)),
                                                                ctypes.byref(nbytes), why, ctypes.c_int32(512)]))
    if rc != STRQ_OK:
        raise StriqueHipError(rc, "%s: bad argument" % entry)
    out = {"rc": int(brc.value), "why": why.value.decode()}
    if brc.value:
        return out
    if nbytes.value > len(image):
        raise StriqueHipError(STRQ_ERR_NOMEM, "%s: an image of %d bytes" % (entry, nbytes.value))
    out.update(n_emit=int(head[0]), n_branch=int(head[1]), mode=int(head[2]), deg=int(head[3]), deg2=int(head[4]),
               end_deg=[int(v) for v in head[5:5 + int(head[1])]])
    for name, at in zip(_IMAGE_ORDER, offs):
        dtype, shape = shapes[name]
        count = int(np.prod(shape))
        out[name] = np.frombuffer(image.tobytes(), dtype, count, int(at)).reshape(shape).copy()
    return out


def debug_variant_image(baked, n_alt):
    return _debug_image("strq_debug_variant_image", VARIANT_IMAGE_SHAPES, baked, [ctypes.c_int32(n_alt)])


def debug_mod_llr_image(baked):
    return _debug_image("strq_debug_mod_llr_image", MOD_LLR_IMAGE_SHAPES, baked, [])


class Context(object):

    def __init__(self, device=0):
        self._lib = load_library()
        self._h = ctypes.c_void_p()
        rc = self._lib.strq_ctx_create(ctypes.c_int(device), ctypes.byref(self._h))
        if rc != STRQ_OK:
            self._h = None
            raise StriqueHipError(rc, "cannot create a context on HIP device %d (no GPU?)" % device)
        self.device = device

    def close(self):
        if getattr(self, "_h", None):
            self._lib.strq_ctx_destroy(self._h)
            self._h = None

    def __del__(self):
        try:
            self.close()
        except Exception:
            pass

    def _check(self, rc):
        if rc != STRQ_OK:
            raise StriqueHipError(rc, self._lib.strq_last_error(self._h).decode())

    def device_synchronize(self):
        self._check(self._lib.strq_device_synchronize(self._h))

    def set_option(self, key, value):
        v = None if value is None else str(value).encode()
        self._check(self._lib.strq_set_option(self._h, key.encode(), v))

    def get_option(self, key):
        buf = ctypes.create_string_buffer(256)
        self._check(self._lib.strq_get_option(self._h, key.encode(), buf, ctypes.c_int32(256)))
        return buf.value.decode()

    def set_align_params(self, open_h, ext_h, open_v, ext_v, dist_offset, dist_min):
        p = np.array([open_h, ext_h, open_v, ext_v, dist_offset, dist_min], dtype=np.float32)
        self._check(self._lib.strq_set_align_params(self._h, _ptr(p)))

    def get_align_params(self):
        p = np.zeros(6, np.float32)
        self._check(self._lib.strq_get_align_params(self._h, _ptr(p)))
        return p

    def align_overlap(self, a, b, want_idx=True):
        a = _c(a, np.float32); b = _c(b, np.float32)
        n, m = len(a), len(b)
        score = ctypes.c_float(); j_end = ctypes.c_int64(); j0 = ctypes.c_int64()
        rec = np.zeros(m, np.int32)
        a_idx = np.zeros(n, np.uint64) if want_idx else None
        b_idx = np.zeros(m, np.uint64) if want_idx else None
        self._check(self._lib.strq_align_overlap(self._h, _ptr(a), ctypes.c_int64(n), _ptr(b), ctypes.c_int64(m),
                                                 ctypes.byref(score), _ptr(a_idx), _ptr(b_idx), _ptr(rec),
                                                 ctypes.byref(j_end), ctypes.byref(j0)))
        return score.value, a_idx, b_idx, rec, j_end.value, j0.value

    def align_batch(self, levels, read_off, level_val, align_read, flank, flank_off, samples=6, want_rec=True):
        levels = _c(levels, np.uint8); read_off = _c(read_off, np.int64); level_val = _c(level_val, np.float32)
        align_read = _c(align_read, np.int32); flank = _c(flank, np.float32); flank_off = _c(flank_off, np.int64)
        na, nr = len(align_read), len(read_off) - 1
        score = np.zeros(na, np.float32); j_end = np.zeros(na, np.int64); j0 = np.zeros(na, np.int64)
        rec = np.zeros(len(flank), np.int32) if want_rec else None
        self._check(self._lib.strq_align_batch(self._h, ctypes.c_int64(na), ctypes.c_int64(nr), _ptr(levels), _ptr(read_off),
                                               _ptr(level_val), _ptr(align_read), _ptr(flank), _ptr(flank_off),
                                               ctypes.c_int32(samples), _ptr(score), _ptr(j_end), _ptr(j0), _ptr(rec)))
        return score, j_end, j0, rec

    def last_timing(self):
        t = np.zeros(8, np.float32)
        self._check(self._lib.strq_last_timing(self._h, _ptr(t)))
        return t

    def last_counters(self):
        t = np.zeros(8, np.float64)
        self._check(self._lib.strq_last_counters(self._h, _ptr(t)))
        return t

    def last_viterbi_launches(self):
        g = np.zeros(4, np.int32)
        self._check(self._lib.strq_last_viterbi_launches(self._h, _ptr(g)))
        return dict(zip(("launches", "register_resident", "lane_layout", "general"), (int(v) for v in g)))

    def last_second_round(self):
        g = np.zeros(2, np.int64)
        self._check(self._lib.strq_last_second_round(self._h, _ptr(g)))
        return int(g[0]), int(g[1])

    def last_screen(self):
        g = np.zeros(8, np.float64)
        self._check(self._lib.strq_last_screen(self._h, _ptr(g)))
        keys = ("ms", "screened", "windowed", "whole_read", "window_columns", "wave_steps", "scale", "candidate_chunks")
        out = dict(zip(keys, (float(v) for v in g)))
        m = np.zeros(8, np.int32)
        self._check(self._lib.strq_last_screen_mode(self._h, _ptr(m)))
        out["mode"] = {0: None, 1: "fine", 2: "coarse"}.get(int(m[0]))
        out["coarse_pause"], out["fine_pause"], out["coarse_margin"], out["merge"] = int(m[1]), int(m[2]), int(m[3]), int(m[4])
        out["second_look"] = int(m[5])
        out["lds_layout"] = {0: None, 1: "lanes", 2: "rows"}.get(int(m[6]))
        return out

    def last_overlap(self):
        g = np.zeros(4, np.float64)
        self._check(self._lib.strq_last_overlap(self._h, _ptr(g)))
        return dict(zip(("viterbi_ms", "under_screen_ms", "under_alignment_stage_ms", "sub_batches"), (float(v) for v in g)))

    def last_geometry(self):
        g = np.zeros(8, np.int32)
        self._check(self._lib.strq_last_geometry(self._h, _ptr(g)))
        keys = ("waves_per_alignment", "tables_per_cu", "wpe", "rows_per_lane", "packed", "overlap_first", "overlap_worst", "launch_groups")
        return dict(zip(keys, (int(v) for v in g)))

    def model_create(self, baked):
        mid = ctypes.c_int32(-1)
        arrs = [_c(baked.in_ptr, np.int32), _c(baked.in_src, np.int32), _c(baked.in_logp, np.float64),
                _c(baked.emis_kind, np.int32), _c(baked.emis_a, np.float64), _c(baked.emis_b, np.float64),
                _c(baked.emis_c, np.float64), _c(baked.count_inc, np.int32), _c(baked.tag, np.int32)]
        hints = getattr(baked, 'hint_slot', None) is not None and (np.asarray(baked.hint_slot)[:baked.silent_start] >= 0).all()
        arrs += [_c(baked.hint_slot, np.int32) if hints else None, _c(baked.hint_lane, np.int32) if hints else None]
        self._check(self._lib.strq_model_create(self._h, ctypes.c_int32(baked.n_states), ctypes.c_int32(baked.silent_start),
                                                ctypes.c_int32(baked.start), ctypes.c_int32(baked.end),
                                                *[_ptr(a) for a in arrs], ctypes.byref(mid)))
        psum = getattr(baked, 'in_logp_sum', None)
        if psum is not None and len(psum) == len(baked.in_logp) and np.all(psum >= baked.in_logp) and not np.array_equal(psum, baked.in_logp):
            self._check(self._lib.strq_model_set_forward_logp(self._h, mid, _ptr(_c(baked.in_logp_sum, np.float64))))
        self.last_positions_rc = self.last_positions_error = None
        if getattr(baked, 'pos_kind', None) is not None:
            rc = self._lib.strq_model_set_positions(self._h, mid, _ptr(_c(baked.pos_kind, np.int32)), _ptr(_c(baked.pos_index, np.int32)))
            self.last_positions_rc = rc
            self.last_positions_error = self._lib.strq_last_error(self._h).decode() if rc == STRQ_ERR_UNSUPPORTED else None
            if rc not in (STRQ_OK, STRQ_ERR_UNSUPPORTED):
                self._check(rc)
        return mid.value

    def viterbi_batch(self, model_id, seqs, want_path=False):
        off = np.zeros(len(seqs) + 1, np.int64)
        for i, s in enumerate(seqs):
            off[i + 1] = off[i] + len(s)
        x = np.concatenate([_c(s, np.float64) for s in seqs]) if len(seqs) else np.zeros(0)
        n = len(seqs)
        logp = np.zeros(n); counted = np.zeros(n, np.int64); status = np.zeros(n, np.int32)
        paths = np.zeros(len(x), np.int32) if want_path else None
        self._check(self._lib.strq_viterbi_batch(self._h, ctypes.c_int32(model_id), ctypes.c_int64(n), _ptr(x), _ptr(off),
                                                 _ptr(logp), _ptr(counted), _ptr(status), _ptr(paths)))
        if want_path:
            paths = [paths[off[i]:off[i + 1]] for i in range(n)]
        return logp, counted, status, paths

    def forward_batch(self, model_id, xs, c0=None):
        n = len(xs)
        off = np.zeros(n + 1, np.int64)
        for i, s in enumerate(xs):
            off[i + 1] = off[i] + len(s)
        x = np.concatenate([_c(s, np.float64) for s in xs]) if n else np.zeros(0)
        if len(x) == 0:
            x = np.zeros(1)
        ll = np.zeros(n); mean = np.zeros(n); var = np.zeros(n); status = np.zeros(n, np.int32)
        c0a = None if c0 is None else _c(c0, np.int64)
        if c0a is not None and len(c0a) != n:
            raise ValueError("c0 must have one entry per window")
        self._check(self._lib.strq_forward_batch(self._h, ctypes.c_int32(model_id), ctypes.c_int64(n), _ptr(x), _ptr(off), _ptr(c0a),
                                                 _ptr(ll), _ptr(mean), _ptr(var), _ptr(status)))
        return ll, mean, var, status

    def viterbi(self, model_id, x, want_path=True):
        logp, counted, status, paths = self.viterbi_batch(model_id, [x], want_path)
        return logp[0], int(counted[0]), int(status[0]), (paths[0] if want_path else None)

    def set_pore_stats(self, tail_lo, tail_hi, model_min, model_max):
        self._check(self._lib.strq_set_pore_stats(self._h, ctypes.c_double(tail_lo), ctypes.c_double(tail_hi),
                                                  ctypes.c_double(model_min), ctypes.c_double(model_max)))

    def target_add(self, prefix_ext, suffix_ext, trim_prefix, trim_suffix, samples, model_id, count_bias):
        pe = _c(prefix_ext, np.float32); se = _c(suffix_ext, np.float32)
        tid = ctypes.c_int32(-1)
        self._check(self._lib.strq_target_add(self._h, _ptr(pe), ctypes.c_int64(len(pe)), _ptr(se), ctypes.c_int64(len(se)),
                                              ctypes.c_int32(trim_prefix), ctypes.c_int32(trim_suffix), ctypes.c_int32(samples),
                                              ctypes.c_int32(model_id), ctypes.c_int32(count_bias), ctypes.byref(tid)))
        return tid.value

    def target_set_mod(self, target_id, mod_model_id, mod_min, mod_max):
        self._check(self._lib.strq_target_set_mod(self._h, ctypes.c_int32(target_id), ctypes.c_int32(mod_model_id),
                                                  ctypes.c_double(mod_min), ctypes.c_double(mod_max)))

    def batch_fetch_mod(self):
        off = np.zeros(self._n_batch + 1, np.int64)
        self._check(self._lib.strq_batch_fetch_mod(self._h, None, ctypes.c_int64(0), _ptr(off)))
        pool = np.zeros(max(1, int(off[-1])), np.uint8)
        self._check(self._lib.strq_batch_fetch_mod(self._h, _ptr(pool), ctypes.c_int64(len(pool)), _ptr(off)))
        raw = pool.tobytes()
        return [raw[off[i]:off[i + 1]].decode() for i in range(self._n_batch)]

    def set_units(self, on):
        self._check(self._lib.strq_set_units(self._h, ctypes.c_int32(1 if on else 0)))

    def batch_fetch_units(self):
        n = getattr(self, '_n_batch', 0)
        off = np.zeros(n + 1, np.int64); dec = np.zeros(max(1, n), np.int32)
        self._check(self._lib.strq_batch_fetch_units(self._h, None, ctypes.c_int64(0), _ptr(off), _ptr(dec)))
        pool = np.zeros(max(1, int(off[-1])), np.int64)
        self._check(self._lib.strq_batch_fetch_units(self._h, _ptr(pool), ctypes.c_int64(len(pool)), _ptr(off), _ptr(dec)))
        return [pool[off[i]:off[i + 1]].copy() if dec[i] else None for i in range(n)]

    def last_units(self):
        out = np.zeros(4)
        self._check(self._lib.strq_last_units(self._h, _ptr(out)))
        return {'ms': float(out[0]), 'ws_bytes': float(out[1]), 'windows': int(out[2]), 'positions': int(out[3])}

    def set_confidence(self, on):
        self._check(self._lib.strq_set_confidence(self._h, ctypes.c_int32(1 if on else 0)))

    def batch_fetch_confidence(self):
        n = getattr(self, '_n_batch', 0)
        out = np.zeros((max(1, n), 3), np.float64); dec = np.zeros(max(1, n), np.int32)
        self._check(self._lib.strq_batch_fetch_confidence(self._h, _ptr(out), _ptr(dec)))
        return [(float(out[i, 0]), float(out[i, 1]), float(out[i, 2])) if dec[i] else None for i in range(n)]

    def last_confidence(self):
        out = np.zeros(4)
        self._check(self._lib.strq_last_confidence(self._h, _ptr(out)))
        return {'ms': float(out[0]), 'windows': int(out[1]), 'no_path': int(out[2]), 'max_exponent': int(out[3])}

    def set_mod_llr(self, on):
        self._check(self._lib.strq_set_mod_llr(self._h, ctypes.c_int32(1 if on else 0)))

    def batch_fetch_mod_llr(self):
        n = getattr(self, '_n_batch', 0)
        off = np.zeros(n + 1, np.int64)
        self._check(self._lib.strq_batch_fetch_mod_llr(self._h, None, ctypes.c_int64(0), _ptr(off)))
        pool = np.zeros((max(1, int(off[-1])), 2), np.float64)
        self._check(self._lib.strq_batch_fetch_mod_llr(self._h, _ptr(pool), ctypes.c_int64(len(pool)), _ptr(off)))
        return [pool[off[i]:off[i + 1]].copy() if off[i + 1] > off[i] else None for i in range(n)]

    def last_mod_llr(self):
        out = np.zeros(4)
        self._check(self._lib.strq_last_mod_llr(self._h, _ptr(out)))
        return {'ms': float(out[0]), 'units': int(out[1]), 'reads': int(out[2]), 'launches': int(out[3])}

    def target_set_variants(self, target_id, model_id, lo, hi, n_alt, context_units):
# ... 291 lines not shown
```

Baseline: 25030.

## Use finer traceback checkpoints for short single-strip alignments and specialize trace kernel

Single-strip alignment tasks with up to 32768 columns now save forward checkpoints every 128 steps instead of 256. This shortens the recomputation window during traceback at the cost of more checkpoint stores and workspace memory. The trace kernel is also templated on linear-gap cases so it can skip the extend/open max, and its device-wide fence is relaxed to a workgroup fence. A new device counter records traceback tasks and rerun steps, which adds two atomics per task.

```diff
diff --git a/include/strique_hip.h b/include/strique_hip.h
--- a/include/strique_hip.h
+++ b/include/strique_hip.h
@@ -188,6 +188,7 @@
 int strq_last_geometry(const strq_ctx* ctx, int32_t out[8]);
 int strq_last_viterbi_launches(const strq_ctx* ctx, int32_t out[4]);
 int strq_last_second_round(const strq_ctx* ctx, int64_t out[2]);
+int strq_last_trace(const strq_ctx* ctx, uint64_t out[2]);
 int strq_last_screen(const strq_ctx* ctx, double out[8]);
 int strq_last_screen_mode(const strq_ctx* ctx, int32_t out[8]);
 int strq_last_overlap(const strq_ctx* ctx, double out[4]);
diff --git a/strique_amd/csrc/align_kernels.h b/strique_amd/csrc/align_kernels.h
--- a/strique_amd/csrc/align_kernels.h
+++ b/strique_amd/csrc/align_kernels.h
@@ -3,6 +3,8 @@
 #include <stdint.h>
 
 #define STRQ_CKPT_STEPS 256
+#define STRQ_CKPT_FINE 128
+#define STRQ_CKPT_FINE_COLS 32768
 #define STRQ_COLS_PER_STEP 2
 #define STRQ_CKPT_FIELDS(R) (2 * (R) + 6)
 #define STRQ_TRACE_WORDS(R) (((R) + 15) / 16)
@@ -27,6 +29,7 @@
     int32_t n, m, k, tsize;
     int32_t row0, m_total;
     int32_t col_off, n_full;
+    int32_t ck_steps;
 };
 
 struct AlignResult {
@@ -37,7 +40,7 @@
 };
 
 static inline int align_num_steps(int n) { return (n + 1) / 2 + 63; }
-static inline int align_num_ckpts(int n) { return (align_num_steps(n) - 1) / STRQ_CKPT_STEPS; }
+static inline int align_num_ckpts(int n, int ck_steps) { return (align_num_steps(n) - 1) / ck_steps; }
 
 #define STRQ_MAX_STRIPS 64
 int align_plan(int m, int samples, int* rows_per_lane, int* n_strips);
@@ -59,7 +62,7 @@
 int launch_align(hipStream_t stream, int R, int S, const AlignTask* tasks, AlignResult* results,
                  int n_tasks, int* queue, const AlignParams& p, int lds_floats_per_wave,
                  int waves_per_block, int n_blocks, uint64_t* scratch, int phase, int mode, int packed,
-                 const int32_t* pick = nullptr);
+                 const int32_t* pick = nullptr, unsigned long long* trace_count = nullptr);
 size_t align_trace_scratch_words_per_wave(int R);
 
 }
diff --git a/strique_amd/csrc/align_kernels.hip b/strique_amd/csrc/align_kernels.hip
--- a/strique_amd/csrc/align_kernels.hip
+++ b/strique_amd/csrc/align_kernels.hip
@@ -173,7 +173,7 @@
 #ifndef STRQ_TRACE_SELECT
                 uint32_t& acc = accA[(r / 16) * 2 + (r % 16) / 8];
                 trace_push_ge(acc, vext, vopn); trace_push_ge(acc, hext, hopn);
-                const float Hn = __builtin_fmaxf(hext, hopn), Vn = __builtin_fmaxf(vext, vopn);
+                const float Hn = LH ? hopn : __builtin_fmaxf(hext, hopn), Vn = LV ? vopn : __builtin_fmaxf(vext, vopn);
                 trace_push_ge(acc, Hn, Vn);
                 const float Gm = __builtin_fmaxf(Hn, Vn);
                 trace_push_ge(acc, D, Gm);
@@ -210,7 +210,7 @@
 #ifndef STRQ_TRACE_SELECT
                 uint32_t& acc = accB[(r / 16) * 2 + (r % 16) / 8];
                 trace_push_ge(acc, vext, vopn); trace_push_ge(acc, hext, hopn);
-                const float Hn = __builtin_fmaxf(hext, hopn), Vn = __builtin_fmaxf(vext, vopn);
+                const float Hn = LH ? hopn : __builtin_fmaxf(hext, hopn), Vn = LV ? vopn : __builtin_fmaxf(vext, vopn);
                 trace_push_ge(acc, Hn, Vn);
                 const float Gm = __builtin_fmaxf(Hn, Vn);
                 trace_push_ge(acc, D, Gm);
@@ -338,6 +338,12 @@
     if (idx < tk.n) { b.sA = tk.bnd_in[2 * idx]; b.vA = tk.bnd_in[2 * idx + 1]; }
     if (idx + 1 < tk.n) { b.sB = tk.bnd_in[2 * idx + 2]; b.vB = tk.bnd_in[2 * idx + 3]; }
     return b;
+}
+
+static __device__ __forceinline__ int task_ck_shift(const AlignTask& tk)
+{
+    const int ck = __builtin_amdgcn_readfirstlane(tk.ck_steps);
+    return ck == 64 ? 6 : ck == 128 ? 7 : 8;
 }
 
 template <int R>
@@ -487,6 +493,7 @@
     __builtin_amdgcn_s_waitcnt(0);
 
     const int nsteps = (tk.n + 1) / 2 + 63;
+    const int ck_shift = task_ck_shift(tk);
     int rM_u = 0;
     if constexpr (RMSW) rM_u = __builtin_amdgcn_readfirstlane(rM);
     (void)rM_u;
@@ -498,7 +505,7 @@
         const int qnext = load_chunk<PK>(tk, t0 / 64 + 1, lane);
         if constexpr (HAS_IN) bnext = load_bnd(tk, t0 / 64 + 1, lane);
         const bool full = (t0 >= 63) && (2 * (t0 + 64) <= tk.n);
-        const bool ckpt_here = ((t0 + 64) % STRQ_CKPT_STEPS) == 0 && (t0 + 64) < nsteps;
+        const bool ckpt_here = ((t0 + 64) & ((1 << ck_shift) - 1)) == 0 && (t0 + 64) < nsteps;
         const int send = nsteps - t0 < 64 ? nsteps - t0 : 64;
         if (full) {
 #ifdef STRQ_DP_PAD
@@ -525,7 +532,7 @@
             }
         }
         if (ckpt_here)
-            save_ckpt<R>(tk.ckpt + (size_t)((t0 + 64) / STRQ_CKPT_STEPS - 1) * (STRQ_CKPT_FIELDS(R) * 64), lane, f.st);
+            save_ckpt<R>(tk.ckpt + (size_t)(((t0 + 64) >> ck_shift) - 1) * (STRQ_CKPT_FIELDS(R) * 64), lane, f.st);
         qcur = qnext;
         if constexpr (HAS_IN) f.bcur = bnext;
     }
@@ -632,11 +639,12 @@
     }
 }
 
-template <int R, int S, bool PK>
+template <int R, int S, bool PK, bool LH = false, bool LV = false>
 __global__ void __launch_bounds__(512)
 align_trace_kernel(const AlignTask* __restrict__ tasks, AlignResult* __restrict__ results, int n_tasks,
                    int* __restrict__ queue, AlignParams p, int lds_floats_per_wave,
-                   uint64_t* __restrict__ scratch_all, const int32_t* __restrict__ pick)
+                   uint64_t* __restrict__ scratch_all, const int32_t* __restrict__ pick,
+                   unsigned long long* __restrict__ trace_count)
 {
     extern __shared__ float lds_all[];
     constexpr int W = STRQ_TRACE_WORDS(R);
@@ -655,6 +663,7 @@
         int32_t* rec = cur->rec;
         const int col_off = __builtin_amdgcn_readfirstlane(cur->col_off);
         LaneConst lc; uint64_t pm[Shape<R, S>::NMASK];
+        int rerun = 0;
 
         int ci = cur->m_total, cj = __builtin_amdgcn_readfirstlane(results[ti].j_end) - col_off, state = 0;
         while (ci > 0 && cj > 0) {
@@ -675,8 +684,10 @@
                 pmu[x] = ((uint64_t)hi << 32) | lo;
             }
             const int tcur = (ci - tk.row0 - 1) / R + (cj + 1) / 2;
-            const int blk = (tcur - 1) / STRQ_CKPT_STEPS;
-            const int tb = blk * STRQ_CKPT_STEPS;
+            const int ck_shift = task_ck_shift(tk);
+            const int blk = (tcur - 1) >> ck_shift;
+            const int tb = blk << ck_shift;
+            rerun += tcur - tb;
             Lane<R> st;
             if (blk == 0) init_lane<R, PK>(tk, lane, st);
             else load_ckpt<R>(tk.ckpt + (size_t)(blk - 1) * (STRQ_CKPT_FIELDS(R) * 64), lane, st);
@@ -714,7 +725,7 @@
                         fetch_scores<R, S, PK>(ldsb, lc, (int)((unsigned)qq >> 16), scB);
                         expand_scores<R, S>(scA, pmu, rsA);
                         expand_scores<R, S>(scB, pmu, rsB);
-                        dp_step2<R, false, false, true, true>(st, rsA, rsB, upA, upB, upVA, upVB, p, &w, 0, nullptr, nullptr);
+                        dp_step2<R, LH, LV, true, true>(st, rsA, rsB, upA, upB, upVA, upVB, p, &w, 0, nullptr, nullptr);
                     }
                     uint64_t* dst = scratch + (size_t)(t - tb - 1) * STEP_WORDS;
 #pragma unroll
@@ -725,7 +736,7 @@
                 }
                 qcur = qnext; bcur = bnext;
             }
-            __threadfence();
+            __builtin_amdgcn_fence(__ATOMIC_ACQ_REL, "workgroup");
             int pf_l = -1, pf_hi = 0, pf_lo = 0, pf_word = -1; uint64_t pf = 0;
             while (ci > tk.row0 && cj > 0) {
                 const int il = ci - tk.row0;
@@ -756,17 +767,33 @@
         }
         for (int i = ci - lane; i > 0; i -= 64) rec[i - 1] = (col_off << 1) | 1;
         results[ti].j0 = cj + col_off;
+        if (trace_count) {
+            __builtin_amdgcn_wave_barrier();
+            if (lane == 0) { atomicAdd(trace_count, 1ull); atomicAdd(trace_count + 1, (unsigned long long)rerun); }
+            __builtin_amdgcn_wave_barrier();
+        }
     }
 }
 
 template <int R, int S>
 static int launch_shape(hipStream_t stream, const AlignTask* tasks, AlignResult* results, int n_tasks,
                         int* queue, const AlignParams& p, int lds_floats_per_wave, int waves_per_block,
-                        int n_blocks, uint64_t* scratch, int phase, int mode, int packed, const int32_t* pick)
+                        int n_blocks, uint64_t* scratch, int phase, int mode, int packed, const int32_t* pick,
+                        unsigned long long* trace_count)
 {
     const size_t lds_bytes = (size_t)lds_floats_per_wave * 4 * waves_per_block;
     const dim3 grid(n_blocks), block(64 * waves_per_block);
     const bool lh = p.open_h == p.ext_h, lv = p.open_v == p.ext_v;
+    const char* tf = strq::opt("STRQ_TRACE_FULL");
+    const bool trace_full = tf && tf[0] == '1';
+    const bool tlh = lh && !trace_full, tlv = lv && !trace_full;
+#define STRQ_TRACE1(PK_, LH_, LV_, P_)                                                                  \
+    do {                                                                                                \
+        (void)hipFuncSetAttribute((const void*)align_trace_kernel<R, S, PK_, LH_, LV_>,                 \
+                                  hipFuncAttributeMaxDynamicSharedMemorySize, (int)lds_bytes);          \
+        hipLaunchKernelGGL((align_trace_kernel<R, S, PK_, LH_, LV_>), grid, block, lds_bytes, stream, tasks, results,\
+                           n_tasks, queue, P_, lds_floats_per_wave, scratch, pick, trace_count);        \
+    } while (0)
 #define STRQ_FWD1(LH_, LV_, MODE_)                                                                      \
     do {                                                                                                \
         (void)hipFuncSetAttribute((const void*)align_forward_kernel<R, S, LH_, LV_, MODE_, false>,      \
@@ -795,16 +822,15 @@
     } else if (packed) {
         AlignParams ps = p;
         ps.open_h *= STRQ_PK_SCALE; ps.ext_h *= STRQ_PK_SCALE; ps.open_v *= STRQ_PK_SCALE; ps.ext_v *= STRQ_PK_SCALE;
-        (void)hipFuncSetAttribute((const void*)align_trace_kernel<R, S, true>,
-                                  hipFuncAttributeMaxDynamicSharedMemorySize, (int)lds_bytes);
-        hipLaunchKernelGGL((align_trace_kernel<R, S, true>), grid, block, lds_bytes, stream, tasks, results,
-                           n_tasks, queue, ps, lds_floats_per_wave, scratch, pick);
+        if (tlh && tlv) STRQ_TRACE1(true, true, true, ps);
+        else STRQ_TRACE1(true, false, false, ps);
     } else {
-        (void)hipFuncSetAttribute((const void*)align_trace_kernel<R, S, false>,
-                                  hipFuncAttributeMaxDynamicSharedMemorySize, (int)lds_bytes);
-        hipLaunchKernelGGL((align_trace_kernel<R, S, false>), grid, block, lds_bytes, stream, tasks, results,
-                           n_tasks, queue, p, lds_floats_per_wave, scratch, pick);
-    }
+        if (tlh && tlv) STRQ_TRACE1(false, true, true, p);
+        else if (tlh) STRQ_TRACE1(false, true, false, p);
+        else if (tlv) STRQ_TRACE1(false, false, true, p);
+        else STRQ_TRACE1(false, false, false, p);
+    }
+#undef STRQ_TRACE1
 #undef STRQ_FWD
 #undef STRQ_FWD1
     return hipGetLastError() == hipSuccess ? 0 : 1;
@@ -813,7 +839,8 @@
 template <int R, int S>
 static int launch_shape_general(hipStream_t stream, const AlignTask* tasks, AlignResult* results, int n_tasks,
                                 int* queue, const AlignParams& p, int lds_floats_per_wave, int waves_per_block,
-                                int n_blocks, uint64_t* scratch, int phase, int mode, int packed, const int32_t* pick)
+                                int n_blocks, uint64_t* scratch, int phase, int mode, int packed, const int32_t* pick,
+                                unsigned long long* trace_count)
 {
     if (packed) return 2;
     const size_t lds_bytes = (size_t)lds_floats_per_wave * 4 * waves_per_block;
@@ -831,7 +858,7 @@
         (void)hipFuncSetAttribute((const void*)align_trace_kernel<R, S, false>,
                                   hipFuncAttributeMaxDynamicSharedMemorySize, (int)lds_bytes);
         hipLaunchKernelGGL((align_trace_kernel<R, S, false>), grid, block, lds_bytes, stream, tasks, results,
-                           n_tasks, queue, p, lds_floats_per_wave, scratch, pick);
+                           n_tasks, queue, p, lds_floats_per_wave, scratch, pick, trace_count);
     }
 #undef STRQ_FWDG
     return hipGetLastError() == hipSuccess ? 0 : 1;
@@ -879,18 +906,18 @@
 int launch_align(hipStream_t stream, int R, int S, const AlignTask* tasks, AlignResult* results,
                  int n_tasks, int* queue, const AlignParams& p, int lds_floats_per_wave,
                  int waves_per_block, int n_blocks, uint64_t* scratch, int phase, int mode, int packed,
-                 const int32_t* pick)
+                 const int32_t* pick, unsigned long long* trace_count)
 {
 #define STRQ_CASE(R_, S_)                                                                               \
     if (R == R_ && S == S_)                                                                             \
         return launch_shape<R_, S_>(stream, tasks, results, n_tasks, queue, p, lds_floats_per_wave,     \
-                                    waves_per_block, n_blocks, scratch, phase, mode, packed, pick);
+                                    waves_per_block, n_blocks, scratch, phase, mode, packed, pick, trace_count);
     STRQ_SHAPES(STRQ_CASE)
 #undef STRQ_CASE
 #define STRQ_CASE(R_, S_)                                                                               \
     if (R == R_ && S == S_)                                                                             \
         return launch_shape_general<R_, S_>(stream, tasks, results, n_tasks, queue, p, lds_floats_per_wave, \
-                                            waves_per_block, n_blocks, scratch, phase, mode, packed, pick);
+                                            waves_per_block, n_blocks, scratch, phase, mode, packed, pick, trace_count);
     STRQ_GENERAL_SHAPES(STRQ_CASE)
 #undef STRQ_CASE
     return 2;
diff --git a/strique_amd/csrc/strq_align_api.hip b/strique_amd/csrc/strq_align_api.hip
--- a/strique_amd/csrc/strq_align_api.hip
+++ b/strique_amd/csrc/strq_align_api.hip
@@ -100,6 +100,19 @@
     return use;
 }
 
+static int ck_forced()
+{
+    if (const char* e = strq::opt("STRQ_CKPT")) { const int v = atoi(e); if (v == 64 || v == 128 || v == 256) return v; }
+    return 0;
+}
+
+static int ck_steps_for(int forced, int n, bool single_strip)
+{
+    if (!single_strip) return STRQ_CKPT_STEPS;
+    if (forced) return forced;
+    return n <= STRQ_CKPT_FINE_COLS ? STRQ_CKPT_FINE : STRQ_CKPT_STEPS;
+}
+
 static int packed_dwords(int entries) { return (((2 * entries + 3) & ~3) + entries + 3) / 4; }
 
 struct Launch { int R, NS, tables, first, count, first_task, first_up, lds_floats, packed, segs; bool known_last_row; };
@@ -114,6 +127,7 @@
 
     bool collapsed = false, allow_pack = false, ov_fixed = false, scr_forced = false, mode_fine = false, mode_coarse = false;
     int seg_want = 0, max_tables = 8, max_waves = 16, ov_cap = 8192;
+    int ck_force = 0;
     std::map<std::pair<int, int>, int> ov_of_m;
 
     std::vector<size_t> cls_off, col0_off, bnd_off;
@@ -364,6 +378,7 @@
     if (const char* e = strq::opt("STRQ_MAX_WAVES")) { const int v = atoi(e); if (v >= 4 && v <= 16) p.max_waves = v; }
     p.allow_pack = p.collapsed && !strq::opt("STRQ_NO_PACK");
     if (const char* e = strq::opt("STRQ_OVERLAP")) { const int v = atoi(e); p.ov_cap = v > 0 ? v : (1 << 30); p.ov_fixed = true; }
+    p.ck_force = ck_forced();
     p.scr_forced = strq::opt("STRQ_SCREEN_ALWAYS") != nullptr;
     const char* mode_opt = strq::opt("STRQ_SCREEN_MODE");
     p.mode_fine = mode_opt && std::strcmp(mode_opt, "fine") == 0;
@@ -767,9 +782,10 @@
             }
             for (int k = 0; k < L.segs; ++k) {
                 pf[k].ck = ps[k].ck = ck_floats;
-                ck_floats += (size_t)align_num_ckpts(std::max(pf[k].n, ps[k].n)) * per_ckpt;
+                const int ck_f = ck_steps_for(p.ck_force, pf[k].n, L.NS == 1), ck_s = ck_steps_for(p.ck_force, ps[k].n, L.NS == 1);
+                ck_floats += (size_t)std::max(align_num_ckpts(pf[k].n, ck_f), align_num_ckpts(ps[k].n, ck_s)) * per_ckpt;
             }
-            if (L.NS > 1) { p.ck_up[i] = ck_floats; ck_floats += (size_t)(L.NS - 1) * align_num_ckpts(n) * per_ckpt; }
+            if (L.NS > 1) { p.ck_up[i] = ck_floats; ck_floats += (size_t)(L.NS - 1) * align_num_ckpts(n, STRQ_CKPT_STEPS) * per_ckpt; }
         }
     }
     for (char t : p.two_round) p.any_two_round |= t != 0;
@@ -807,6 +823,7 @@
             base.levels = in.d_levels + in.read_off[in.read[i]];
             base.rec = c->rec.as<int32_t>() + out.rec_off[i];
             base.n = in.n[i]; base.n_full = in.n[i]; base.m_total = M;
+            base.ck_steps = STRQ_CKPT_STEPS;
             auto strip = [&](int row0, int rows, size_t ck, int sidx) {
                 AlignTask t = base;
                 const int j = p.NJ[i] > 1 ? p.J0[i] + sidx : p.J0[i];
@@ -823,16 +840,18 @@
                     const size_t ti = (size_t)L.first_task + (size_t)x * L.segs + k;
                     AlignTask t = strip(0, M, p.pieces[ti].ck, 0);
                     t.levels += p.pieces[ti].col_off; t.n = p.pieces[ti].n; t.col_off = p.pieces[ti].col_off;
+                    t.ck_steps = ck_steps_for(p.ck_force, t.n, true);
                     tasks[ti] = t;
                     if (p.any_two_round) {
                         AlignTask u = strip(0, M, p.safe[ti].ck, 0);
                         u.levels += p.safe[ti].col_off; u.n = p.safe[ti].n; u.col_off = p.safe[ti].col_off;
+                        u.ck_steps = ck_steps_for(p.ck_force, u.n, true);
                         tasks[safe0 + ti] = u;
                     }
                 }
             } else {
                 const int rows_s = 64 * R;
-                const size_t ck_strip = (size_t)align_num_ckpts(in.n[i]) * STRQ_CKPT_FIELDS(R) * 64;
+                const size_t ck_strip = (size_t)align_num_ckpts(in.n[i], STRQ_CKPT_STEPS) * STRQ_CKPT_FIELDS(R) * 64;
                 float* bnd = c->bnd.as<float>() + p.bnd_off[i];
                 const size_t bnd_stride = 2 * ((size_t)in.n[i] + 2);
                 for (int sidx = 0; sidx < L.NS; ++sidx) {
@@ -998,7 +1017,8 @@
                     const int start = std::max(0, own_lo - 1 - ov_w);
                     t.levels = head.levels + start; t.n = own_hi - start; t.col_off = start;
                     t.ckpt = reinterpret_cast<float*>((uintptr_t)ck2 * 4);
-                    ck2 += (size_t)align_num_ckpts(t.n) * per_ckpt;
+                    t.ck_steps = ck_steps_for(p.ck_force, t.n, true);
+                    ck2 += (size_t)align_num_ckpts(t.n, t.ck_steps) * per_ckpt;
                     cols2 += t.n; out.wave_steps += align_num_steps(t.n); out.columns += t.n;
                     t2.push_back(t); ++made;
                 }
@@ -1129,7 +1149,8 @@
         }
         const int wpb = std::min(trace_wpb, (160 * 1024) / (std::max(lds_floats, 1) * 4));
         if (launch_align(st, L.R, S, p.d_tasks, p.d_res + L.first, count, c->queue.as<int>() + p.qi, c->ap, lds_floats, wpb, c->n_cu,
-                         c->scratch.as<uint64_t>(), 1, 0, L.packed, p.d_pick + L.first)) { c->err = "trace launch failed"; return STRQ_ERR_DEVICE; }
+                         c->scratch.as<uint64_t>(), 1, 0, L.packed, p.d_pick + L.first,
+                         c->redo_total.p ? c->redo_total.as<unsigned long long>() + 1 : nullptr)) { c->err = "trace launch failed"; return STRQ_ERR_DEVICE; }
         ++p.qi; li = lj;
     }
     STRQ_HIP(c, hipEventRecord(c->ev[4], st));
@@ -1180,7 +1201,15 @@
 
 size_t align_workspace_bytes(int n, int m, int R, int NS)
 {
-    size_t b = (size_t)NS * (align_num_ckpts(n) + align_num_ckpts(n) / 4 + 300) * STRQ_CKPT_FIELDS(R) * 64 * 4;
+    const int forced = ck_forced();
+    const int ck = NS == 1 && forced ? forced : STRQ_CKPT_STEPS;
+    const size_t coarse = align_num_ckpts(n, ck);
+    size_t nck = coarse + coarse / 4 + 300 * (size_t)(STRQ_CKPT_STEPS / ck);
+    if (NS == 1 && !forced) {
+        const size_t fine = align_num_ckpts(n, STRQ_CKPT_FINE);
+        nck = std::max(nck, std::min(fine + fine / 4 + 300 * (size_t)(STRQ_CKPT_STEPS / STRQ_CKPT_FINE), (size_t)4 * align_num_ckpts(STRQ_CKPT_FINE_COLS, STRQ_CKPT_FINE)));
+    }
+    size_t b = (size_t)NS * nck * STRQ_CKPT_FIELDS(R) * 64 * 4;
     if (NS > 1) b += (size_t)(NS - 1) * ((size_t)n + 2) * 8;
     (void)m;
     return b;
@@ -1478,6 +1507,18 @@
 {
     if (!c || !out) return STRQ_ERR_ARG;
     out[0] = c->second_round[0]; out[1] = c->second_round[1];
+    return STRQ_OK;
+}
+
+int strq_last_trace(const strq_ctx* c, uint64_t out[2])
+{
+    if (!c || !out) return STRQ_ERR_ARG;
+    out[0] = out[1] = 0;
+    if (!c->redo_total.p) return STRQ_OK;
+    if (hipSetDevice(c->device) != hipSuccess || hipStreamSynchronize(c->stream) != hipSuccess) return STRQ_ERR_DEVICE;
+    unsigned long long h[2] = {0, 0};
+    if (hipMemcpy(h, c->redo_total.as<unsigned long long>() + 1, sizeof(h), hipMemcpyDeviceToHost) != hipSuccess) return STRQ_ERR_DEVICE;
+    out[0] = h[0]; out[1] = h[1];
     return STRQ_OK;
 }
 
diff --git a/strique_amd/ffi.py b/strique_amd/ffi.py
--- a/strique_amd/ffi.py
+++ b/strique_amd/ffi.py
@@ -240,6 +240,11 @@
     def last_second_round(self):
         g = np.zeros(2, np.int64)
         self._check(self._lib.strq_last_second_round(self._h, _ptr(g)))
+        return int(g[0]), int(g[1])
+
+    def last_trace(self):
+        g = np.zeros(2, np.uint64)
+        self._check(self._lib.strq_last_trace(self._h, _ptr(g)))
         return int(g[0]), int(g[1])
 
     def last_screen(self):
```

Measured after the change: 24830. About the same (-0.8%).
